# haskoin/haskoin-node

Hardware: AMD Instinct MI355X
Metric: ECDSA verifies/sec (1/8 GPU) + verdict mismatches vs libsecp256k1 (higher is better)
Workload: dtype u32 (256-bit integer limbs)

## Files before the change

haskoin-node_amd/csrc/hkv_api.cpp:

```cpp
#include <hip/hip_runtime.h>

#include <algorithm>
#include <chrono>
#include <cstdio>
#include <cstdlib>
#include <cstring>
#include <memory>
#include <mutex>
#include <new>
#include <random>
#include <string>
#include <vector>

#include "../../include/hkv.h"
#include "hkv_blocktx.h"
#include "hkv_spends.h"
#include "hkv_internal.h"
#include "hkv_launch_plan.h"
#include "hkv_layout.h"
#include "hkv_plan.h"
#include "hkv_tail_plan.h"

namespace {

thread_local std::string g_last_hip;

constexpr size_t CLK_GROUPS = 4096, CLK_WORDS = 16 + 2 * CLK_GROUPS;

int hip_fail(hipError_t e, const char* what) {
  g_last_hip = std::string(what) + ": " + hipGetErrorString(e);
  return HKV_E_HIP;
}
int oom_fail(hipError_t e, const char* what) {
  g_last_hip = std::string(what) + ": " + hipGetErrorString(e);
  return HKV_E_OOM;
}
#define HKV_TRY(expr, what)                       \
  do {                                            \
    hipError_t e_ = (expr);                       \
    if (e_ != hipSuccess) return hip_fail(e_, what); \
  } while (0)
#define HKV_RC(expr)         \
  do {                       \
    const int rc_ = (expr);  \
    if (rc_) return rc_;     \
  } while (0)

struct DeviceMem {
  static hipError_t alloc(void** p, size_t bytes) { return hipMalloc(p, bytes); }
  static void release(void* p) { (void)hipFree(p); }
};
struct PinnedMem {
  static hipError_t alloc(void** p, size_t bytes) { return hipHostMalloc(p, bytes, hipHostMallocPortable); }
  static void release(void* p) { (void)hipHostFree(p); }
};
template <class T, class Mem = DeviceMem>
class DevBuf {
 public:
  DevBuf() = default;
  DevBuf(DevBuf&& o) noexcept : p_(o.p_), n_(o.n_) { o.p_ = nullptr, o.n_ = 0; }
  DevBuf& operator=(DevBuf&& o) noexcept {
    std::swap(p_, o.p_), std::swap(n_, o.n_);
    return *this;
  }
  ~DevBuf() {
    if (p_) Mem::release(p_);
  }
  int reserve(size_t count, const char* what) {
    if (p_ && n_ >= count) return HKV_OK;
    if (p_) Mem::release(p_);
    p_ = nullptr, n_ = 0;
    const hipError_t e = Mem::alloc(reinterpret_cast<void**>(&p_), std::max<size_t>(count * sizeof(T), 16));
    if (e != hipSuccess) {
      p_ = nullptr;
      return oom_fail(e, what);
    }
    n_ = count;
    return HKV_OK;
  }
  T* get() const { return p_; }
  operator T*() const { return p_; }
  size_t size() const { return n_; }

 private:
  T* p_ = nullptr;
  size_t n_ = 0;
};

struct DevCtx {
  int device = -1;
  hkv::Geometry geo;
  hipStream_t stream = nullptr;
  hipStream_t copy_stream = nullptr;
  hipStream_t hash_stream = nullptr;
  hipEvent_t ev_fork = nullptr, ev_join = nullptr;
  DevBuf<uint32_t> gtab, qs;
  DevBuf<uint32_t> im;
  DevBuf<uint32_t> bits;
  DevBuf<uint8_t> recs;
  DevBuf<uint32_t, PinnedMem> hbits;
  DevBuf<uint32_t> pool;
  uint32_t pool_n = 0;
  uint64_t pool_seed = ~0ull;
  DevBuf<uint32_t> txt;
  DevBuf<uint8_t> stage_tx_bytes, stage_scripts, stage_jobs, stage_out, stage_headers, stage_blocks;
  DevBuf<uint32_t> stage_tx_off;
  DevBuf<uint8_t> stage_prev;
  DevBuf<uint32_t> std_first, host_tx_bits;
  DevBuf<hkv_input_job> std_jobs;
  DevBuf<uint8_t> blk_txids;
  DevBuf<uint32_t> blk_table, blk_src;
  uint32_t txid_mask = 0xFFFFFFFFu;
  DevBuf<uint32_t> spd_off, spd_table, spd_spender;
  DevBuf<uint64_t> spd_sums;
  DevBuf<uint8_t> spd_flags;
  uint32_t spend_stages = hkv::SPEND_STAGE_ALL;
  DevBuf<uint32_t> ms_desc, ms_cbits, ms_kbits, host_std_bits;
  DevBuf<uint64_t> ms_off;
  DevBuf<uint8_t> ms_recs;
  uint32_t ms_win_cand = 0, ms_win_keys = 0;
  DevBuf<uint64_t> ms_ctr;
  DevBuf<unsigned int> ms_bar;
  uint32_t tail_epoch = 0;
  bool inject_tail = false;
  uint32_t* call_status = nullptr;
  bool ms_dirty = false;
  DevBuf<uint32_t> rare_ctr;
  bool rare_dirty = false;
  DevBuf<uint32_t> aux;
  bool profile = false;
  std::vector<hipEvent_t> ev;
  DevBuf<unsigned long long> clk;
  int wall_khz = 0;
  hipEvent_t last_use = nullptr;
  uint32_t inject = 0;
};

}

struct hkv_ctx {
  std::vector<DevCtx> devs;
  std::mutex mu;
  std::vector<std::unique_ptr<std::mutex>> tx_mu;
  std::vector<bool> healthy;
  std::vector<uint32_t> failures;
  uint64_t txid_salt = 0;
};
struct hkv_batch {
  hkv_ctx* ctx = nullptr;
  uint8_t* host = nullptr;
  size_t cap = 0;
};

namespace {

size_t round_up(size_t a, size_t b) { return (a + b - 1) / b * b; }

#ifndef HKV_STD_CHUNK
#define HKV_STD_CHUNK (1u << 20)
#endif
constexpr size_t MS_CAND_PER_INPUT = hkv::MS_CAND_PER_INPUT, MS_KEYS_PER_INPUT = hkv::MS_KEYS_PER_INPUT;
constexpr size_t HKV_MAX_STD_INPUTS = 0xFFFFFF00ull;
constexpr size_t MS_BAR_WORDS = 32, MS_FAULT = 16, MS_HOST_STATUS = 17;
#ifndef HKV_HOST_FIRST_DIV
#define HKV_HOST_FIRST_DIV 4
#endif
#ifndef HKV_HOST_MAX_GRIDS
#define HKV_HOST_MAX_GRIDS 8
#endif

int ensure_dev_buffers(DevCtx& d, size_t n_pad) {
  int rc = d.im.reserve(n_pad * hkv::IM_WORDS, "hipMalloc(intermediate)");
  if (!rc) rc = d.bits.reserve(n_pad / 32, "hipMalloc(bits)");
  if (!rc) rc = d.qs.reserve(hkv::plan_records(d.geo, n_pad).qs_quads * 4, "hipMalloc(qtab scratch)");
  return rc;
}

int scratch_acquire(DevCtx& d, hipStream_t st) {
  HKV_TRY(hipStreamWaitEvent(st, d.last_use, 0), "hipStreamWaitEvent(scratch)");
  return HKV_OK;
}
int scratch_release(DevCtx& d, hipStream_t st) {
  HKV_TRY(hipEventRecord(d.last_use, st), "hipEventRecord(scratch)");
  return HKV_OK;
}

int ensure_aux(DevCtx& d, size_t n_pad) { return d.aux.reserve(n_pad * hkv::AUX_WORDS, "hipMalloc(aux)"); }

int profile_mark(DevCtx& d, hipEvent_t (&e)[3], int k, hipStream_t st) {
  if (!d.profile) return HKV_OK;
  if (k == 0)
    for (auto& x : e) HKV_TRY(hipEventCreate(&x), "hipEventCreate");
  HKV_TRY(hipEventRecord(e[k], st), "hipEventRecord");
  if (k == 2) d.ev.insert(d.ev.end(), e, e + 3);
  return HKV_OK;
}

int enqueue_verify(DevCtx& d, const void* d_records, size_t n, uint32_t mode, hipStream_t st,
                   uint32_t* out_bits = nullptr, hipEvent_t late_join = nullptr,
                   const hkv::StdOps* std_pro = nullptr) {
  const hkv::RecPlan plan = hkv::plan_records(d.geo, n);
  HKV_RC(ensure_dev_buffers(d, plan.n_pad));
  hipEvent_t e[3] = {nullptr, nullptr, nullptr};
  HKV_RC(profile_mark(d, e, 0, st));
  if (std_pro != nullptr && plan.shape != hkv::Shape::Mid) return HKV_E_INTERNAL;
  if (plan.aux) HKV_RC(ensure_aux(d, plan.n_pad));
  const hkv::RecOps ops{d.im, (uint32_t)n, d.gtab, d.qs, out_bits ? out_bits : d.bits.get(),
                        (uint32_t)(out_bits ? (n + 31) / 32 : plan.n_pad / 32), d.profile ? d.clk.get() : nullptr,
                        d.aux, d_records, mode};
  if (plan.prologue && std_pro == nullptr) HKV_TRY(hkv::launch_prologue(plan, ops, st), "prologue launch");
  HKV_RC(profile_mark(d, e, 1, st));
  HKV_TRY(hkv::launch_ecmult(plan, ops, std_pro, st), "ecmult launch");
  if (plan.prologue) {
    if (late_join != nullptr) HKV_TRY(hipStreamWaitEvent(st, late_join, 0), "hipStreamWaitEvent(hash join)");
    if (d.rare_dirty) {
      HKV_TRY(hipMemsetAsync(d.rare_ctr, 0, sizeof(uint32_t), st), "hipMemset(rare counter)");
      d.rare_dirty = false;
    }
    const hipError_t e2 = hkv::launch_finish(plan, ops, d.rare_ctr, late_join != nullptr ? d_records : nullptr, st);
    if (e2 != hipSuccess) {
      d.rare_dirty = true;
      return hip_fail(e2, "finish launch");
    }
  }
  return profile_mark(d, e, 2, st);
}

int init_device(DevCtx& d, int device) {
  d.device = device;
  HKV_TRY(hipSetDevice(device), "hipSetDevice");
  hipDeviceProp_t prop;
  HKV_TRY(hipGetDeviceProperties(&prop, device), "hipGetDeviceProperties");
  if (std::strncmp(prop.gcnArchName, "gfx950", 6) != 0) {
    g_last_hip = std::string("device is ") + prop.gcnArchName + ", libhkv is built for gfx950 only";
    return HKV_E_NODEV;
  }
  hkv::Geometry& g = d.geo;
  g.n_cu = (uint32_t)prop.multiProcessorCount;
  HKV_TRY(hipStreamCreateWithFlags(&d.stream, hipStreamNonBlocking), "hipStreamCreate");
  HKV_TRY(hipStreamCreateWithFlags(&d.copy_stream, hipStreamNonBlocking), "hipStreamCreate(copy)");
  HKV_TRY(hipStreamCreateWithFlags(&d.hash_stream, hipStreamNonBlocking), "hipStreamCreate(hash)");
  HKV_TRY(hipEventCreateWithFlags(&d.ev_fork, hipEventDisableTiming), "hipEventCreate(fork)");
  HKV_TRY(hipEventCreateWithFlags(&d.ev_join, hipEventDisableTiming), "hipEventCreate(join)");
  HKV_TRY(hipEventCreateWithFlags(&d.last_use, hipEventDisableTiming), "hipEventCreate(scratch)");
  HKV_TRY(hipEventRecord(d.last_use, d.stream), "hipEventRecord(scratch)");
  HKV_RC(d.ms_ctr.reserve(4, "hipMalloc(multisig counters)"));
  HKV_TRY(hipMemsetAsync(d.ms_ctr, 0, 4 * sizeof(uint64_t), d.stream), "hipMemset(multisig counters)");
  HKV_RC(d.ms_bar.reserve(MS_BAR_WORDS, "hipMalloc(multisig barrier)"));
  HKV_TRY(hipMemsetAsync(d.ms_bar, 0, MS_BAR_WORDS * sizeof(unsigned int), d.stream), "hipMemset(multisig barrier)");
  HKV_RC(d.rare_ctr.reserve(1, "hipMalloc(rare counter)"));
  HKV_TRY(hipMemsetAsync(d.rare_ctr, 0, sizeof(uint32_t), d.stream), "hipMemset(rare counter)");
  HKV_TRY(hipStreamSynchronize(d.stream), "multisig counters sync");
  HKV_TRY(hipDeviceGetAttribute(&d.wall_khz, hipDeviceAttributeWallClockRate, device), "wall clock rate");
  HKV_RC(d.clk.reserve(CLK_WORDS, "hipMalloc(clock probe)"));
  HKV_TRY(hipMemsetAsync(d.clk, 0, CLK_WORDS * sizeof(unsigned long long), d.stream), "hipMemset(clock probe)");
  HKV_RC(d.gtab.reserve(hkv::GTAB_DWORDS, "hipMalloc(gtab)"));
  int per_cu = 0;
  HKV_TRY(hkv::ecmult_max_blocks_per_cu(&per_cu), "occupancy query");
  if (per_cu < 1) per_cu = 1;
  g.grid_max = g.n_cu * (uint32_t)per_cu;
  if (!hkv::host_chunks_ok((size_t)g.grid_max * hkv::WG, HKV_HOST_FIRST_DIV)) {
    g_last_hip = "the host-batch first chunk is not a whole number of verdict words";
    return HKV_E_INTERNAL;
  }
  g.std_chunk = HKV_STD_CHUNK;
  if (const char* e = std::getenv("HKV_STD_CHUNK")) {
    const unsigned long long c = std::strtoull(e, nullptr, 10) / 64 * 64;
    if (c >= 64 && c <= (1ull << 24)) g.std_chunk = (size_t)c;
  }
  g.rec_chunk = HKV_REC_CHUNK;
  if (const char* e = std::getenv("HKV_REC_CHUNK")) {
    const unsigned long long c = std::strtoull(e, nullptr, 10) / hkv::WG * hkv::WG;
    if (c >= (unsigned long long)hkv::WG && c <= HKV_REC_CHUNK) g.rec_chunk = (size_t)c;
  }
  HKV_RC(d.qs.reserve(hkv::plan_records(g, 1).qs_quads * 4, "hipMalloc(qtab scratch)"));
  HKV_TRY(hkv::launch_gtable(d.gtab, d.stream), "gtable launch");
  HKV_TRY(hipStreamSynchronize(d.stream), "gtable sync");
  return HKV_OK;
}

void clear_events(DevCtx& d) {
  for (auto e : d.ev) (void)hipEventDestroy(e);
  d.ev.clear();
}

void free_device(DevCtx& d) {
  if (d.device < 0) return;
  (void)hipSetDevice(d.device);
  if (d.stream) (void)hipStreamSynchronize(d.stream);
  (void)hipDeviceSynchronize();
  clear_events(d);
  for (hipEvent_t e : {d.last_use, d.ev_fork, d.ev_join})
    if (e) (void)hipEventDestroy(e);
  for (hipStream_t s : {d.stream, d.copy_stream, d.hash_stream})
    if (s) (void)hipStreamDestroy(s);
  d = DevCtx();
}

int ensure_pool(DevCtx& d, uint64_t seed, uint32_t pool_n, hipStream_t st) {
  if (d.pool_n == pool_n && d.pool_seed == seed) return HKV_OK;
  d.pool_n = 0;
  HKV_RC(d.pool.reserve((size_t)pool_n * 16, "hipMalloc(pool)"));
  HKV_TRY(hkv::launch_gen_pool(seed, pool_n, d.pool, st), "gen pool launch");
  d.pool_n = pool_n;
  d.pool_seed = seed;
  return HKV_OK;
}

int self_check(DevCtx& d) {
  const size_t n = 256;
  uint8_t* recs = nullptr;
  HKV_TRY(hipMalloc(&recs, n * hkv::REC_SIZE), "hipMalloc(selfcheck)");
  int rc = scratch_acquire(d, d.stream);
  if (!rc) rc = ensure_pool(d, 0x484B5630ull, 16, d.stream);
  if (!rc) {
    hipError_t e = hkv::launch_gen_records(0x484B5630ull, 0, (uint32_t)n, d.pool, d.pool_n, 250, 0, recs, nullptr,
                                           d.stream);
    if (e != hipSuccess) rc = hip_fail(e, "selfcheck gen");
  }
  if (!rc) rc = enqueue_verify(d, recs, n, HKV_MODE_LIBSECP, d.stream);
  uint32_t words[8] = {0};
  if (!rc) {
    hipError_t e = hipMemcpyAsync(words, d.bits, sizeof(words), hipMemcpyDeviceToHost, d.stream);
    if (e == hipSuccess) e = hipStreamSynchronize(d.stream);
    if (e != hipSuccess) rc = hip_fail(e, "selfcheck copy");
  }
  if (!rc) rc = scratch_release(d, d.stream);
  (void)hipFree(recs);
  if (rc) return rc;
  for (uint32_t w : words)
    if (w != 0xFFFFFFFFu) {
      g_last_hip = "self-check: generated valid signatures did not verify";
      return HKV_E_INTERNAL;
    }
  return HKV_OK;
}


bool txs_ok(const hkv_txs* t) {
  return t && (t->n_tx == 0 || (t->bytes && t->offsets)) && (t->scripts || t->scripts_len == 0) &&
         t->n_tx < 0xFFFFFF00u;
}

int reserve_txt(DevCtx& d, const hkv_txs* dt) {
  return d.txt.reserve((size_t)dt->n_tx * hkv::TXT_WORDS, "hipMalloc(txt)");
}
int enqueue_tx_index(DevCtx& d, const hkv_txs* dt, hipStream_t st, uint32_t hashes = hkv::TX_HASHES_ALL) {
  HKV_RC(reserve_txt(d, dt));
  HKV_TRY(hkv::launch_tx_index(dt->bytes, dt->offsets, dt->n_tx, hashes, d.txt, st), "tx index launch");
  return HKV_OK;
}
uint32_t std_tx_hashes(int32_t forkid) { return forkid >= 0 ? hkv::TX_HASHES_ALL : hkv::TX_HASHES_WITNESS; }

hkv::StdOps std_ops(const DevCtx& d, const hkv_txs* dt, const hkv_input_job* jobs, int32_t forkid) {
  return hkv::StdOps{dt->bytes, dt->n_tx, d.txt, dt->scripts, dt->scripts_len, jobs, forkid};
}

int enqueue_std_inputs(DevCtx& d, const hkv_txs* dt, const hkv::StdOps& so, size_t n, void* recs, hipStream_t st) {
  HKV_RC(enqueue_tx_index(d, dt, st, std_tx_hashes(so.forkid)));
  HKV_TRY(hkv::launch_std_inputs(so, (uint32_t)n, static_cast<uint8_t*>(recs), st), "std input launch");
  return HKV_OK;
}

int enqueue_std_verify_split(DevCtx& d, const hkv::StdPlan& plan, const hkv::StdOps& so, size_t n, void* recs,
                             uint32_t* out_bits, const hkv::MsScan* ms, const uint32_t* tx_off, hipStream_t st) {
  HKV_RC(ensure_dev_buffers(d, plan.n_pad));
  HKV_RC(ensure_aux(d, plan.n_pad));
  hipEvent_t e[3] = {nullptr, nullptr, nullptr};
  HKV_RC(profile_mark(d, e, 0, st));
  HKV_RC(profile_mark(d, e, 1, st));
  const hkv::RecOps ops{d.im, (uint32_t)n, d.gtab, d.qs, out_bits, (uint32_t)((n + 31) / 32),
                        d.profile ? d.clk.get() : nullptr, d.aux, recs, HKV_MODE_HASKOIN};
  HKV_TRY(hkv::launch_std_verify_split(plan, so, ops, ms, tx_off, st), "std-input verify launch");
  return profile_mark(d, e, 2, st);
}

hkv::MsTail tail_args(DevCtx& d, const hkv::StdOps& so, const uint32_t* tx_off, size_t n, uint32_t* out_bits,
                      bool hash_txs, const hkv::MsScan& ms, size_t cap_cand, size_t cap_keys) {
  hkv::MsTail t;
  t.win_cand = (uint32_t)cap_cand;
  t.win_keys = (uint32_t)cap_keys;
  t.txs = so.txs;
  t.tx_off = tx_off;
  t.n_tx = so.n_tx;
  t.txt = d.txt;
  t.scripts = so.scripts;
  t.scripts_len = so.scripts_len;
  t.jobs = so.jobs;
  t.n = (uint32_t)n;
  t.forkid = so.forkid;
  t.hash_txs = hash_txs ? std_tx_hashes(so.forkid) : hkv::TX_HASHES_NONE;
  t.desc = ms.desc;
  t.off = ms.off;
  t.total = reinterpret_cast<unsigned long long*>(ms.counters);
  t.total_next = reinterpret_cast<unsigned long long*>(d.ms_ctr + ((d.tail_epoch + 1u) & 1u));
  t.cand = d.ms_recs;
  t.keyrec = d.ms_recs + cap_cand * hkv::REC_SIZE;
  t.cbits = d.ms_cbits;
  t.kbits = d.ms_kbits;
  t.im = d.im;
  t.aux = d.aux;
  t.gtab = d.gtab;
  t.qs = d.qs;
  t.out_bits = out_bits;
  t.bar = d.ms_bar;
  t.epoch = d.tail_epoch;
  t.fault = d.ms_bar + MS_FAULT;
  t.status = d.call_status;
  t.force_fault = d.inject_tail ? 1u : 0u;
  return t;
}
int enqueue_std_chunk(DevCtx& d, const hkv_txs* dt, const hkv_input_job* jobs, size_t n, int32_t forkid, void* recs,
                      uint32_t* out_bits, hipStream_t st) {
  const hkv::StdPlan plan = hkv::plan_std_chunk(d.geo, n);
  const bool small = plan.shape == hkv::Shape::Block || plan.shape == hkv::Shape::Pair;
  const size_t all_cand = n * MS_CAND_PER_INPUT, all_keys = n * MS_KEYS_PER_INPUT;
  const size_t win_c = d.ms_win_cand ? d.ms_win_cand : HKV_MS_WIN_CAND;
  const size_t win_k = d.ms_win_keys ? d.ms_win_keys : HKV_MS_WIN_KEYS;
  const size_t cap_cand = hkv::ms_window_records(all_cand, win_c), cap_keys = hkv::ms_window_records(all_keys, win_k);
  const size_t scratch_pad = std::max<size_t>(plan.n_pad, round_up(hkv::ms_tail_slots(d.geo.n_cu), hkv::WG));
  int rc = d.ms_desc.reserve(n * 2, "hipMalloc(multisig desc)");
  if (!rc) rc = d.ms_off.reserve(n, "hipMalloc(multisig offsets)");
  if (!rc) rc = d.ms_cbits.reserve(hkv::ms_cbits_words(n), "hipMalloc(multisig candidate bits)");
  if (!rc) rc = d.ms_recs.reserve((cap_cand + cap_keys) * hkv::REC_SIZE, "hipMalloc(multisig records)");
  if (!rc) rc = d.ms_kbits.reserve(hkv::ms_kbits_words(n), "hipMalloc(multisig key bits)");
  if (!rc) rc = ensure_dev_buffers(d, scratch_pad);
  if (!rc) rc = ensure_aux(d, scratch_pad);
  if (!rc) rc = reserve_txt(d, dt);
  if (rc) return rc;
  const hkv::StdOps so = std_ops(d, dt, jobs, forkid);
  if (d.ms_dirty) {
    HKV_TRY(hipMemsetAsync(d.ms_ctr, 0, 2 * sizeof(uint64_t), st), "hipMemset(multisig counters)");
    d.ms_dirty = false;
  }
  d.ms_dirty = true;
  const hkv::MsScan ms{d.ms_desc, d.ms_off, d.ms_ctr + (d.tail_epoch & 1u)};
  auto hip_rc = [](hipError_t e, const char* what) { return e == hipSuccess ? (int)HKV_OK : hip_fail(e, what); };
  bool forked = false;
  if (plan.index_first)
    rc = enqueue_tx_index(d, dt, st, plan.index_hashes ? std_tx_hashes(forkid) : (uint32_t)hkv::TX_HASHES_NONE);
  if (rc) return rc;
  if (small) {
    rc = enqueue_std_verify_split(d, plan, so, n, recs, out_bits, plan.scan_in_kernel ? &ms : nullptr,
                                  plan.rows_in_kernel ? dt->offsets : nullptr, st);
  } else if (plan.overlap) {
    HKV_TRY(hipEventRecord(d.ev_fork, st), "hipEventRecord(fork)");
    HKV_TRY(hipStreamWaitEvent(d.hash_stream, d.ev_fork, 0), "hipStreamWaitEvent(fork)");
    forked = true;
    hipError_t e = hkv::launch_tx_hashes_only(dt->bytes, dt->offsets, dt->n_tx, std_tx_hashes(forkid), d.txt,
                                              d.hash_stream);
    if (e == hipSuccess) e = hkv::launch_std_inputs(so, (uint32_t)n, static_cast<uint8_t*>(recs), d.hash_stream);
    if (e == hipSuccess && plan.scan == hkv::ScanOn::HashStream)
      e = hkv::launch_ms_scan(so, (uint32_t)n, ms, d.hash_stream);
    const hipError_t e2 = hipEventRecord(d.ev_join, d.hash_stream);
    rc = e != hipSuccess ? hip_fail(e, "std hash half launch") : hip_rc(e2, "hipEventRecord(join)");
  } else {
    rc = hip_rc(hkv::launch_std_inputs(so, (uint32_t)n, static_cast<uint8_t*>(recs), st), "std input launch");
  }
  if (!rc && plan.scan == hkv::ScanOn::MainStream)
    rc = hip_rc(hkv::launch_ms_scan(so, (uint32_t)n, ms, st), "multisig scan launch");
  if (!rc && !small)
    rc = enqueue_verify(d, recs, n, HKV_MODE_HASKOIN, st, out_bits, plan.overlap ? d.ev_join : nullptr,
                        plan.overlap ? &so : nullptr);
  if (!rc)
    rc = hip_rc(hkv::launch_ms_tail(tail_args(d, so, dt->offsets, n, out_bits, plan.tail_hashes, ms, cap_cand, cap_keys),
                                    d.geo.n_cu, st),
                "multisig tail launch");
  if (!rc) {
    ++d.tail_epoch;
    d.inject_tail = false;
    d.ms_dirty = false;
  }
  if (rc && forked) (void)hipStreamWaitEvent(st, d.ev_join, 0);
  return rc;
}

int enqueue_verify_std_inputs(DevCtx& d, const hkv_txs* dt, const hkv_input_job* jobs, size_t n, int32_t forkid,
                              void* recs, uint32_t* out_bits, hipStream_t st) {
  const size_t chunk = hkv::std_chunk_len(d.geo, n);
  for (size_t lo = 0; lo < n; lo += chunk) {
    const size_t cn = std::min(chunk, n - lo);
    const int rc = enqueue_std_chunk(d, dt, jobs + lo, cn, forkid, static_cast<uint8_t*>(recs) + lo * hkv::REC_SIZE,
                                     out_bits + lo / 32, st);
    if (rc) return rc;
  }
  return HKV_OK;
}

int stage_txs(DevCtx& d, const hkv_txs* h, const void* jobs, size_t job_bytes, hkv_txs* dt, void** djobs) {
  const size_t nbytes = h->n_tx ? h->offsets[h->n_tx] : 0;
  const size_t noff = (size_t)h->n_tx + 1;
  HKV_RC(d.stage_tx_bytes.reserve(nbytes, "hipMalloc(tx bytes)"));
  HKV_RC(d.stage_tx_off.reserve(noff, "hipMalloc(tx offsets)"));
  HKV_RC(d.stage_scripts.reserve(h->scripts_len, "hipMalloc(scripts)"));
  HKV_RC(d.stage_jobs.reserve(job_bytes, "hipMalloc(jobs)"));
  if (nbytes) HKV_TRY(hipMemcpyAsync(d.stage_tx_bytes, h->bytes, nbytes, hipMemcpyHostToDevice, d.stream), "H2D txs");
  if (h->n_tx)
    HKV_TRY(hipMemcpyAsync(d.stage_tx_off, h->offsets, noff * 4, hipMemcpyHostToDevice, d.stream), "H2D offsets");
  if (h->scripts_len)
    HKV_TRY(hipMemcpyAsync(d.stage_scripts, h->scripts, h->scripts_len, hipMemcpyHostToDevice, d.stream),
            "H2D scripts");
  if (job_bytes) HKV_TRY(hipMemcpyAsync(d.stage_jobs, jobs, job_bytes, hipMemcpyHostToDevice, d.stream), "H2D jobs");
  dt->bytes = d.stage_tx_bytes;
  dt->offsets = d.stage_tx_off;
  dt->n_tx = h->n_tx;
  dt->scripts = d.stage_scripts;
  dt->scripts_len = h->scripts_len;
  *djobs = d.stage_jobs.get();
  return HKV_OK;
}

bool dev_ok(const hkv_ctx* ctx, int dev) { return ctx && dev >= 0 && dev < (int)ctx->devs.size(); }

enum class Lock { None, Mu, Tx };
class Call {
 public:
  DevCtx& d;
  const hipStream_t st;
  int rc = HKV_OK;
  Call(hkv_ctx* ctx, int dev, void* hip_stream, Lock kind)
      : d(ctx->devs[(size_t)dev]), st(static_cast<hipStream_t>(hip_stream)) {
    if (kind == Lock::Tx) tx_ = std::unique_lock<std::mutex>(*ctx->tx_mu[(size_t)dev]);
    if (kind != Lock::None) mu_ = std::unique_lock<std::mutex>(ctx->mu);
    const hipError_t e = hipSetDevice(d.device);
    if (e != hipSuccess) rc = hip_fail(e, "hipSetDevice");
  }
  Call(hkv_ctx* ctx, int dev, Lock kind) : Call(ctx, dev, ctx->devs[(size_t)dev].stream, kind) {}
  int acquire(uint32_t* status = nullptr) {
    if (!rc) rc = scratch_acquire(d, st);
    if (!rc) held_ = true, d.call_status = status;
    return rc;
  }
  int done(int r = HKV_OK) {
    if (!held_) return r;
    held_ = false;
    d.call_status = nullptr;
    if (!r) return scratch_release(d, st);
    (void)hipEventRecord(d.last_use, st);
    return r;
  }
  ~Call() { (void)done(HKV_E_HIP); }

 private:
  std::unique_lock<std::mutex> tx_, mu_;
  bool held_ = false;
};

}

extern "C" {

uint32_t hkv_version(void) { return (1u << 16) | 4u; }

const char* hkv_strerror(int err) {
  switch (err) {
    case HKV_OK: return "ok";
    case HKV_E_ARG: return "invalid argument";
    case HKV_E_NODEV: return "no usable gfx950 device";
    case HKV_E_OOM: return "out of memory";
    case HKV_E_HIP: return "HIP runtime error";
    case HKV_E_INTERNAL: return "internal self-check failed";
    default: return "unknown error";
  }
}
const char* hkv_last_hip_error(void) { return g_last_hip.c_str(); }

int hkv_device_count(void) {
  int n = 0;
  if (hipGetDeviceCount(&n) != hipSuccess) return 0;
  return n;
}

int hkv_open_devices(const int* device_ids, int n_ids, uint32_t flags, hkv_ctx** out) {
  if (!out || n_ids <= 0 || !device_ids) return HKV_E_ARG;
  *out = nullptr;
  hkv_ctx* ctx = new (std::nothrow) hkv_ctx();
  if (!ctx) return HKV_E_OOM;
  ctx->devs.resize(n_ids);
  ctx->healthy.assign(n_ids, true);
  ctx->failures.assign(n_ids, 0);
  try {
    std::random_device rd;
    ctx->txid_salt = ((uint64_t)rd() << 32) ^ (uint64_t)rd();
  } catch (...) {
    const uint64_t now = (uint64_t)std::chrono::steady_clock::now().time_since_epoch().count();
    ctx->txid_salt = (now * 0x9E3779B97F4A7C15ull) ^ (uint64_t)reinterpret_cast<uintptr_t>(ctx);
  }
  for (int k = 0; k < n_ids; ++k) ctx->tx_mu.emplace_back(new (std::nothrow) std::mutex());
  for (auto& m : ctx->tx_mu)
    if (!m) {
      delete ctx;
      return HKV_E_OOM;
    }
  for (int k = 0; k < n_ids; ++k) {
    int rc = init_device(ctx->devs[k], device_ids[k]);
    if (!rc && !(flags & HKV_OPEN_NO_SELFCHECK)) rc = self_check(ctx->devs[k]);
    if (rc) {
      for (auto& d : ctx->devs) free_device(d);
      delete ctx;
      return rc;
    }
  }
  *out = ctx;
  return HKV_OK;
}

int hkv_open(int n_gpus, uint32_t flags, hkv_ctx** out) {
  if (!out) return HKV_E_ARG;
  int avail = hkv_device_count();
  if (avail <= 0) return HKV_E_NODEV;
  if (n_gpus <= 0 || n_gpus > avail) n_gpus = avail;
  std::vector<int> ids(n_gpus);
  for (int k = 0; k < n_gpus; ++k) ids[k] = k;
  return hkv_open_devices(ids.data(), n_gpus, flags, out);
}

void hkv_close(hkv_ctx* ctx) {
  if (!ctx) return;
  for (auto& d : ctx->devs) free_device(d);
  delete ctx;
}

int hkv_ctx_num_devices(const hkv_ctx* ctx) { return ctx ? (int)ctx->devs.size() : 0; }

int hkv_device_healthy(hkv_ctx* ctx, int dev) {
  if (!dev_ok(ctx, dev)) return HKV_E_ARG;
  std::lock_guard<std::mutex> lock(ctx->mu);
  return ctx->healthy[(size_t)dev] ? 1 : 0;
}

int hkv_device_reset_health(hkv_ctx* ctx, int dev) {
  if (!dev_ok(ctx, dev)) return HKV_E_ARG;
  std::lock_guard<std::mutex> lock(ctx->mu);
  ctx->healthy[(size_t)dev] = true;
  return HKV_OK;
}

int hkv_device_failures(hkv_ctx* ctx, int dev) {
  if (!dev_ok(ctx, dev)) return HKV_E_ARG;
  std::lock_guard<std::mutex> lock(ctx->mu);
  return (int)ctx->failures[(size_t)dev];
}

int hkv_debug_fail_device(hkv_ctx* ctx, int dev, uint32_t when) {
  if (!dev_ok(ctx, dev) || when > HKV_FAIL_TAIL) return HKV_E_ARG;
  std::lock_guard<std::mutex> lock(ctx->mu);
  if (when == HKV_FAIL_TAIL) ctx->devs[(size_t)dev].inject_tail = true;
  else ctx->devs[(size_t)dev].inject = when;
  return HKV_OK;
}

int hkv_debug_ms_window(hkv_ctx* ctx, int dev, uint32_t cand_records, uint32_t key_records) {
  if (!dev_ok(ctx, dev) || cand_records > HKV_MS_WIN_CAND ||
      key_records > HKV_MS_WIN_KEYS)
    return HKV_E_ARG;
  std::lock_guard<std::mutex> lock(ctx->mu);
  DevCtx& d = ctx->devs[(size_t)dev];
  d.ms_win_cand = (uint32_t)round_up(cand_records, 64);
  d.ms_win_keys = (uint32_t)round_up(key_records, 64);
  return HKV_OK;
}

int hkv_debug_q_scratch(hkv_ctx* ctx, int dev, size_t* bytes, size_t* chunk) {
  if (!dev_ok(ctx, dev) || !bytes || !chunk) return HKV_E_ARG;
  std::lock_guard<std::mutex> lock(ctx->mu);
  *bytes = ctx->devs[(size_t)dev].qs.size() * sizeof(uint32_t);
  *chunk = ctx->devs[(size_t)dev].geo.rec_chunk;
  return HKV_OK;
}

int hkv_debug_launch_shape(hkv_ctx* ctx, int dev, uint32_t kind, size_t n, uint32_t out[4]) {
  if (!dev_ok(ctx, dev) || kind > 1 || n == 0 || n > HKV_MAX_STD_INPUTS || !out) return HKV_E_ARG;
  std::lock_guard<std::mutex> lock(ctx->mu);
  const hkv::Geometry& g = ctx->devs[(size_t)dev].geo;
  if (kind == 0) {
    const hkv::RecPlan p = hkv::plan_records(g, n);
    out[0] = (uint32_t)p.shape, out[1] = 0, out[2] = p.chunk(0).cn, out[3] = p.n_chunks;
  } else {
    const size_t chunk = hkv::std_chunk_len(g, n), first = std::min(chunk, n);
    const hkv::StdPlan p = hkv::plan_std_chunk(g, first);
    out[0] = (uint32_t)p.shape;
    out[1] = (p.scan_in_kernel ? 1u : 0u) | (p.rows_in_kernel ? 2u : 0u) | (p.overlap ? 4u : 0u);
    out[2] = (uint32_t)first, out[3] = (uint32_t)((n + chunk - 1) / chunk);
  }
  return HKV_OK;
}

int hkv_debug_ms_scratch(hkv_ctx* ctx, int dev, size_t* bytes) {
  if (!dev_ok(ctx, dev) || !bytes) return HKV_E_ARG;
  std::lock_guard<std::mutex> lock(ctx->mu);
  *bytes = ctx->devs[(size_t)dev].ms_recs.size();
  return HKV_OK;
}

int hkv_debug_ms_tail_counts(hkv_ctx* ctx, int dev, uint64_t out[3]) {
  if (!dev_ok(ctx, dev) || !out) return HKV_E_ARG;
  Call c(ctx, dev, Lock::Mu);
  DevCtx& d = c.d;
  out[0] = out[1] = out[2] = 0;
  if (d.tail_epoch == 0) return HKV_OK;
  const uint32_t par = (d.tail_epoch - 1u) & 1u;
  uint64_t total = 0;
  unsigned int slot[2] = {0, 0};
  HKV_RC(c.acquire());
  HKV_TRY(hipMemcpyAsync(&total, d.ms_ctr + par, sizeof(total), hipMemcpyDeviceToHost, c.st), "D2H scan total");
  HKV_TRY(hipMemcpyAsync(slot, d.ms_bar + par * 8u, sizeof(slot), hipMemcpyDeviceToHost, c.st), "D2H tail slot");
  HKV_TRY(hipStreamSynchronize(c.st), "tail counts sync");
  out[0] = total;
  out[1] = slot[0];
  out[2] = slot[1];
  return c.done();
}

int hkv_device_fault(hkv_ctx* ctx, int dev, uint32_t* fault) {
  if (!dev_ok(ctx, dev) || !fault) return HKV_E_ARG;
  Call c(ctx, dev, Lock::Mu);
  DevCtx& d = c.d;
  unsigned int w = 0;
  HKV_RC(c.acquire());
  HKV_TRY(hipMemcpyAsync(&w, d.ms_bar + MS_FAULT, sizeof(w), hipMemcpyDeviceToHost, c.st), "D2H fault latch");
  HKV_TRY(hipMemsetAsync(d.ms_bar + MS_FAULT, 0, sizeof(unsigned int), c.st), "hipMemset(fault latch)");
  HKV_TRY(hipStreamSynchronize(c.st), "fault latch sync");
  *fault = w ? HKV_STATUS_TAIL_FAULT : 0u;
  return c.done();
}

int hkv_batch_alloc(hkv_ctx* ctx, size_t max_n, hkv_batch** out) {
  if (!ctx || !out || max_n == 0) return HKV_E_ARG;
  hkv_batch* b = new (std::nothrow) hkv_batch();
  if (!b) return HKV_E_OOM;
  if (hipHostMalloc(reinterpret_cast<void**>(&b->host), max_n * hkv::REC_SIZE, hipHostMallocPortable) !=
      hipSuccess) {
    delete b;
    return HKV_E_OOM;
  }
  std::memset(b->host, 0, max_n * hkv::REC_SIZE);
  b->ctx = ctx;
  b->cap = max_n;
  *out = b;
  return HKV_OK;
}
void hkv_batch_free(hkv_batch* b) {
  if (!b) return;
  if (b->host) (void)hipHostFree(b->host);
  delete b;
}
uint8_t* hkv_batch_records(hkv_batch* b) { return b ? b->host : nullptr; }
size_t hkv_batch_capacity(const hkv_batch* b) { return b ? b->cap : 0; }

static void quiesce(DevCtx& d) {
  (void)hipSetDevice(d.device);
  (void)hipStreamSynchronize(d.copy_stream);
  (void)hipStreamSynchronize(d.stream);
}

static int enqueue_host_shard(DevCtx& d, const uint8_t* host, const hkv::Shard& s, uint32_t mode,
                              std::vector<hipEvent_t>& evs) {
  if (d.inject == HKV_FAIL_ENQUEUE) {
    d.inject = 0;
    g_last_hip = "injected enqueue failure (hkv_debug_fail_device)";
    return HKV_E_HIP;
  }
  if (d.inject == HKV_FAIL_ALLOC) {
    d.inject = 0;
    return oom_fail(hipErrorOutOfMemory, "injected allocation failure (hkv_debug_fail_device)");
  }
  const size_t len = s.hi - s.lo;
  hipError_t e0 = hipSetDevice(d.device);
  int rc = e0 == hipSuccess ? scratch_acquire(d, d.stream) : hip_fail(e0, "hipSetDevice");
  if (!rc) rc = scratch_acquire(d, d.copy_stream);
  if (!rc) rc = d.recs.reserve(len * hkv::REC_SIZE, "hipMalloc(records)");
  if (!rc) rc = d.hbits.reserve((len + 31) / 32, "hipHostMalloc(bits)");
  if (rc) return rc;
  const size_t grid_lanes = (size_t)d.geo.grid_max * hkv::WG;
  const uint8_t* src = host + s.lo * hkv::REC_SIZE;
  const std::vector<size_t> chunks = hkv::host_chunks(len, grid_lanes, HKV_HOST_FIRST_DIV, HKV_HOST_MAX_GRIDS);
  rc = ensure_dev_buffers(d, round_up(*std::max_element(chunks.begin(), chunks.end()), hkv::WG));
  size_t off = 0;
  for (auto it = chunks.begin(); it != chunks.end() && !rc; off += *it++) {
    const size_t cl = *it;
    hipEvent_t ev = nullptr;
    hipError_t e = hipEventCreateWithFlags(&ev, hipEventDisableTiming);
    if (e != hipSuccess) {
      rc = oom_fail(e, "hipEventCreate");
      break;
    }
    evs.push_back(ev);
    if (e == hipSuccess)
      e = hipMemcpyAsync(d.recs + off * hkv::REC_SIZE, src + off * hkv::REC_SIZE, cl * hkv::REC_SIZE,
                         hipMemcpyHostToDevice, d.copy_stream);
    if (e == hipSuccess) e = hipEventRecord(ev, d.copy_stream);
    if (e == hipSuccess) e = hipStreamWaitEvent(d.stream, ev, 0);
    if (e != hipSuccess) {
      rc = hip_fail(e, "H2D records");
      break;
    }
    rc = enqueue_verify(d, d.recs + off * hkv::REC_SIZE, cl, mode, d.stream);
    if (!rc) {
      e = hipMemcpyAsync(d.hbits + off / 32, d.bits, (cl + 31) / 32 * 4, hipMemcpyDeviceToHost, d.stream);
      if (e != hipSuccess) rc = hip_fail(e, "D2H bits");
    }
  }
  if (!rc) rc = scratch_release(d, d.stream);
  if (!rc) rc = scratch_acquire(d, d.copy_stream);
  return rc;
}

static int join_host_shard(DevCtx& d, const hkv::Shard& s, uint32_t* out, size_t out_words) {
  HKV_TRY(hipSetDevice(d.device), "hipSetDevice");
  HKV_TRY(hipStreamSynchronize(d.stream), "verify sync");
  if (d.inject == HKV_FAIL_JOIN) {
    d.inject = 0;
    g_last_hip = "injected join failure (hkv_debug_fail_device)";
    return HKV_E_HIP;
  }
  if (!hkv::merge_shard_words(out, out_words, d.hbits, s)) {
    g_last_hip = "shard does not fit the verdict bitmap";
    return HKV_E_INTERNAL;
  }
  return HKV_OK;
}

static int verify_from_host(hkv_ctx* ctx, const uint8_t* host, size_t n, uint32_t mode, uint32_t* out) {
  if (!ctx || !host || !out || mode > HKV_MODE_HASKOIN) return HKV_E_ARG;
  if (n == 0) return HKV_OK;
  std::lock_guard<std::mutex> lock(ctx->mu);
  std::vector<std::vector<hipEvent_t>> evs(ctx->devs.size());
  struct EventGuard {
    std::vector<std::vector<hipEvent_t>>& e;
    ~EventGuard() {
      for (auto& v : e)
        for (auto ev : v) (void)hipEventDestroy(ev);
    }
  } guard{evs};
  const size_t out_words = (n + 31) / 32;
  return hkv::run_with_failover(
      n, ctx->healthy,
      [&](const hkv::Shard& s) { return enqueue_host_shard(ctx->devs[(size_t)s.dev], host, s, mode, evs[(size_t)s.dev]); },
      [&](const hkv::Shard& s) { return join_host_shard(ctx->devs[(size_t)s.dev], s, out, out_words); },
      [&](int dev, int) {
        quiesce(ctx->devs[(size_t)dev]);
        ++ctx->failures[(size_t)dev];
      });
}

int hkv_verify(hkv_ctx* ctx, hkv_batch* b, size_t n, uint32_t mode, uint32_t* verdict_bits) {
  if (!b || n > b->cap) return HKV_E_ARG;
  return verify_from_host(ctx, b->host, n, mode, verdict_bits);
}

int hkv_verify_host(hkv_ctx* ctx, const uint8_t* records, size_t n, uint32_t mode, uint32_t* verdict_bits) {
  return verify_from_host(ctx, records, n, mode, verdict_bits);
}

int hkv_verify_device(hkv_ctx* ctx, int dev, const void* d_records, size_t n, uint32_t mode, uint32_t* d_bits,
                      void* hip_stream) {
  if (!dev_ok(ctx, dev) || !d_records || !d_bits || mode > HKV_MODE_HASKOIN) return HKV_E_ARG;
  if (n == 0) return HKV_OK;
  if (n > 0xFFFFFF00ull) return HKV_E_ARG;
  Call c(ctx, dev, hip_stream, Lock::Mu);
  int rc = c.acquire();
  if (!rc) rc = enqueue_verify(c.d, d_records, n, mode, c.st, d_bits);
  return c.done(rc);
}

int hkv_gen_batch_device(hkv_ctx* ctx, int dev, uint64_t seed, uint64_t index0, size_t n, uint32_t pool_size,
                         uint32_t uncompressed_permille, uint32_t invalid_permille, void* d_records,
                         uint32_t* d_labels, void* hip_stream) {
  if (!dev_ok(ctx, dev) || !d_records || pool_size == 0 || uncompressed_permille > 1000 ||
      invalid_permille > 1000 || n > 0xFFFFFF00ull || index0 > ~0ull - n)
    return HKV_E_ARG;
  if (n == 0) return HKV_OK;
  Call c(ctx, dev, hip_stream, Lock::Mu);
  DevCtx& d = c.d;
  HKV_RC(c.acquire());
  HKV_RC(ensure_pool(d, seed ^ 0x706F6F6Cull, pool_size, c.st));
  HKV_TRY(hkv::launch_gen_records(seed, index0, (uint32_t)n, d.pool, d.pool_n, uncompressed_permille,
                                  invalid_permille, d_records, d_labels, c.st),
          "gen records launch");
  return c.done();
}

int hkv_gen_records_device(hkv_ctx* ctx, int dev, uint64_t seed, size_t n, uint32_t pool_size,
                           uint32_t uncompressed_permille, void* d_records, void* hip_stream) {
  return hkv_gen_batch_device(ctx, dev, seed, 0, n, pool_size, uncompressed_permille, 0, d_records, nullptr,
                              hip_stream);
}

int hkv_debug_op(hkv_ctx* ctx, int dev, uint32_t op, size_t n, const uint32_t* d_a, const uint32_t* d_b,
                 uint32_t* d_out, void* hip_stream) {
  if (!dev_ok(ctx, dev) || !d_a || !d_b || !d_out) return HKV_E_ARG;
  if (n == 0) return HKV_OK;
  Call c(ctx, dev, hip_stream, Lock::None);
  HKV_RC(c.rc);
  HKV_TRY(hkv::launch_debug(op, (uint32_t)n, d_a, d_b, d_out, c.st), "debug launch");
  return HKV_OK;
}

int hkv_profile_enable(hkv_ctx* ctx, int on) {
  if (!ctx) return HKV_E_ARG;
  std::lock_guard<std::mutex> lock(ctx->mu);
  for (auto& d : ctx->devs) {
    (void)hipSetDevice(d.device);
    (void)hipDeviceSynchronize();
    clear_events(d);
    d.profile = on != 0;
  }
  return HKV_OK;
}

int hkv_profile_read(hkv_ctx* ctx, int dev, double* prologue_ms, double* ecmult_ms, uint64_t* launches) {
  if (!dev_ok(ctx, dev) || !prologue_ms || !ecmult_ms || !launches)
    return HKV_E_ARG;
  Call call(ctx, dev, Lock::Mu);
  HKV_RC(call.rc);
  DevCtx& d = call.d;
  double p = 0, m = 0;
  for (size_t k = 0; k + 2 < d.ev.size(); k += 3) {
    HKV_TRY(hipEventSynchronize(d.ev[k + 2]), "hipEventSynchronize");
    float a = 0, b = 0;
    HKV_TRY(hipEventElapsedTime(&a, d.ev[k], d.ev[k + 1]), "hipEventElapsedTime");
    HKV_TRY(hipEventElapsedTime(&b, d.ev[k + 1], d.ev[k + 2]), "hipEventElapsedTime");
    p += a;
    m += b;
  }
  *prologue_ms = p;
  *ecmult_ms = m;
  *launches = d.ev.size() / 3;
  clear_events(d);
  return HKV_OK;
}

int hkv_profile_clock(hkv_ctx* ctx, int dev, double* sclk_mhz) {
  if (!dev_ok(ctx, dev) || !sclk_mhz) return HKV_E_ARG;
  Call call(ctx, dev, Lock::Mu);
  HKV_RC(call.rc);
  DevCtx& d = call.d;
  HKV_TRY(hipDeviceSynchronize(), "hipDeviceSynchronize");
  unsigned long long c[4] = {0, 0, 0, 0};
  HKV_TRY(hipMemcpy(c, d.clk, sizeof(c), hipMemcpyDeviceToHost), "D2H clock probe");
  *sclk_mhz = 0;
  if (c[3] > c[1] && d.wall_khz > 0) *sclk_mhz = (double)(c[2] - c[0]) / ((double)(c[3] - c[1]) / (d.wall_khz * 1e-3));
  return HKV_OK;
}

int hkv_profile_phases(hkv_ctx* ctx, int dev, uint64_t* stamps, size_t n, double* tick_ns) {
  if (!dev_ok(ctx, dev) || !stamps || !tick_ns || n > 12) return HKV_E_ARG;
  Call call(ctx, dev, Lock::Mu);
  HKV_RC(call.rc);
  DevCtx& d = call.d;
  HKV_TRY(hipDeviceSynchronize(), "hipDeviceSynchronize");
  if (n) HKV_TRY(hipMemcpy(stamps, d.clk + 4, n * sizeof(uint64_t), hipMemcpyDeviceToHost), "D2H phase stamps");
  *tick_ns = d.wall_khz > 0 ? 1e6 / d.wall_khz : 0.0;
  return HKV_OK;
}

int hkv_profile_group_stamps(hkv_ctx* ctx, int dev, uint64_t* stamps, size_t n_groups, double* tick_ns) {
  if (!dev_ok(ctx, dev) || !stamps || !tick_ns || n_groups > CLK_GROUPS)
    return HKV_E_ARG;
  Call call(ctx, dev, Lock::Mu);
  HKV_RC(call.rc);
  DevCtx& d = call.d;
  HKV_TRY(hipDeviceSynchronize(), "hipDeviceSynchronize");
  if (n_groups)
    HKV_TRY(hipMemcpy(stamps, d.clk + 16, 2 * n_groups * sizeof(uint64_t), hipMemcpyDeviceToHost), "D2H group stamps");
  *tick_ns = d.wall_khz > 0 ? 1e6 / d.wall_khz : 0.0;
  return HKV_OK;
}

int hkv_sighash_device(hkv_ctx* ctx, int dev, const hkv_txs* d_txs, const hkv_sighash_job* d_jobs, size_t n,
                       int32_t forkid, uint8_t* d_out, size_t out_stride, uint8_t* d_status, void* hip_stream) {
  if (!dev_ok(ctx, dev) || !txs_ok(d_txs) || out_stride < 32 || out_stride % 4 ||
      out_stride > 0xFFFFFFFFu || n > 0xFFFFFF00ull)
    return HKV_E_ARG;
  if (n == 0) return HKV_OK;
  if (!d_jobs || !d_out) return HKV_E_ARG;
  Call c(ctx, dev, hip_stream, Lock::Tx);
  HKV_RC(c.acquire());
  HKV_RC(enqueue_tx_index(c.d, d_txs, c.st));
  HKV_TRY(hkv::launch_sighash(d_txs->bytes, d_txs->n_tx, c.d.txt, d_txs->scripts, d_txs->scripts_len, d_jobs,
                              (uint32_t)n, forkid, d_out, (uint32_t)out_stride, d_status, c.st),
          "sighash launch");
  return c.done();
}

int hkv_sighash(hkv_ctx* ctx, const hkv_txs* txs, const hkv_sighash_job* jobs, size_t n, int32_t forkid,
                uint8_t* out32, uint8_t* status) {
// ... 725 lines not shown
```

haskoin-node_amd/csrc/hkv_internal.h:

```cpp
#pragma once
#include <hip/hip_runtime.h>
#include <stdint.h>

#include "../../include/hkv.h"
#include "hkv_launch_plan.h"

#define HKV_MODE_LIBSECP 0u
#define HKV_MODE_HASKOIN 1u

enum {
  HKV_DBG_FE_MUL = 1,
  HKV_DBG_FE_SQR = 2,
  HKV_DBG_FE_ADD = 3,
  HKV_DBG_FE_SUB = 4,
  HKV_DBG_FE_INV = 5,
  HKV_DBG_FE_SQRT = 6,
  HKV_DBG_SC_MUL = 7,
  HKV_DBG_SC_INV = 8,
  HKV_DBG_GLV = 9,
  HKV_DBG_ECMULT_G = 10,
  HKV_DBG_MUL512 = 11,
  HKV_DBG_SQR512 = 12,
  HKV_DBG_FE_CNEG = 13,
  HKV_DBG_FE_CNEG_MASK = 14,
  HKV_DBG_FE_NEG = 15,
  HKV_DBG_FE_HALF = 16,
  HKV_DBG_FE_SHL = 17,
  HKV_DBG_FE_SHL_VAR = 18,
  HKV_DBG_FE_MUL_SMALL = 19,
  HKV_DBG_FE_MUL_SMALL2 = 20,
  HKV_DBG_FE_LIN2 = 21,
  HKV_DBG_FE_MUL_ADD = 22,
  HKV_DBG_FE_MUL2 = 23,
  HKV_DBG_FE_SQR2 = 24,
  HKV_DBG_FE_SQRMUL = 25,
  HKV_DBG_FE_MUL_REF = 26,
  HKV_DBG_FE_SQR_REF = 27,
  HKV_DBG_FE_NORMALIZE = 28,
  HKV_DBG_FE_IS_ZERO = 29,
  HKV_DBG_FE_EQUAL = 30,
  HKV_DBG_U256_LT_P = 31,
  HKV_DBG_SC_ADD = 32,
  HKV_DBG_SC_SUB = 33,
  HKV_DBG_SC_NEG = 34,
  HKV_DBG_SC_SQR = 35,
  HKV_DBG_SC_IS_HIGH = 36,
  HKV_DBG_INV_MOD_P = 37,
  HKV_DBG_FE_MUL_SUM = 38,
  HKV_DBG_FE_SQRMUL_SUM = 39,
  HKV_DBG_FE_NEG_COMPL = 40,
  HKV_DBG_FE_MUL_SUM_RA = 41,
  HKV_DBG_FE_MUL_SUM_RD = 42,
  HKV_DBG_FE_SQRMUL_SUM_RA = 43,
  HKV_DBG_FE_SQRMUL_SUM_RD = 44,
  HKV_DBG_FE_MUL_SUM_RB = 45,
  HKV_DBG_GEJ_DOUBLE = 64,
  HKV_DBG_GEJ_DOUBLE_ILP = 65,
  HKV_DBG_GEJ_ACCUMULATE = 66,
  HKV_DBG_GEJ_ACCUMULATE_ILP = 67,
  HKV_DBG_GEJ_ADD_VAR = 68,
  HKV_DBG_GEJ_ADD_AFFINE_COMPLETE = 69,
  HKV_DBG_X_MATCHES_R = 70,
  HKV_DBG_ECMULT = 71,
};

namespace hkv {
struct RecOps {
  uint32_t* im;
  uint32_t n;
  const uint32_t* gtab;
  uint32_t* qs;
  uint32_t* bits;
  uint32_t n_words;
  unsigned long long* clk;
  uint32_t* aux;
  const void* recs;
  uint32_t mode;
};
struct StdOps;
hipError_t launch_prologue(const RecPlan& p, const RecOps& r, hipStream_t st);
hipError_t launch_ecmult(const RecPlan& p, const RecOps& r, const StdOps* std_pro, hipStream_t st);
hipError_t launch_gtable(uint32_t* gtab, hipStream_t st);
struct MsScan {
  uint32_t* desc;
  uint64_t* off;
  uint64_t* counters;
};
struct MsTail {
  const uint8_t* txs;
  const uint32_t* tx_off;
  uint32_t n_tx;
  uint32_t* txt;
  const uint8_t* scripts;
  uint32_t scripts_len;
  const hkv_input_job* jobs;
  uint32_t n;
  int32_t forkid;
  uint32_t hash_txs;
  const uint32_t* desc;
  const uint64_t* off;
  unsigned long long* total;
  unsigned long long* total_next;
  uint8_t* cand;
  uint8_t* keyrec;
  uint32_t win_cand, win_keys;
  uint32_t* cbits;
  uint32_t* kbits;
  uint32_t* im;
  uint32_t* aux;
  const uint32_t* gtab;
  uint32_t* qs;
  uint32_t* out_bits;
  unsigned int* bar;
  uint32_t epoch;
  unsigned int* fault;
  uint32_t* status;
  uint32_t force_fault;
};
hipError_t launch_ms_tail(const MsTail& a, uint32_t grid, hipStream_t st);
uint32_t ms_tail_slots(uint32_t n_cu);
struct StdOps {
  const uint8_t* txs;
  uint32_t n_tx;
  const uint32_t* txt;
  const uint8_t* scripts;
  uint32_t scripts_len;
  const hkv_input_job* jobs;
  int32_t forkid;
};
hipError_t launch_std_verify_split(const StdPlan& p, const StdOps& o, const RecOps& r, const MsScan* ms,
                                   const uint32_t* tx_off, hipStream_t st);
hipError_t launch_finish(const RecPlan& p, const RecOps& r, uint32_t* rare_ctr, const void* late_recs,
                         hipStream_t st);
hipError_t launch_gen_pool(uint64_t seed, uint32_t npool, uint32_t* pool, hipStream_t st);
hipError_t launch_gen_records(uint64_t seed, uint64_t index0, uint32_t n, const uint32_t* pool, uint32_t npool,
                              uint32_t unc_permille, uint32_t invalid_permille, void* recs, uint32_t* labels,
                              hipStream_t st);
hipError_t launch_debug(uint32_t op, uint32_t n, const uint32_t* a, const uint32_t* b, uint32_t* out,
                        hipStream_t st);
hipError_t ecmult_max_blocks_per_cu(int* out);
hipError_t launch_gen_keys(uint64_t seed, uint32_t n, uint8_t* priv, uint8_t* pub, uint8_t* h160, hipStream_t st);
hipError_t launch_gen_sign(uint64_t seed, uint32_t n, const uint8_t* priv, const uint32_t* key_idx,
                           const uint8_t* msg, uint32_t msg_stride, uint8_t* sig, hipStream_t st);
hipError_t launch_tx_index(const uint8_t* txs, const uint32_t* tx_off, uint32_t n_tx, uint32_t hashes,
                           uint32_t* txt, hipStream_t st);
hipError_t launch_sighash(const uint8_t* txs, uint32_t n_tx, const uint32_t* txt, const uint8_t* scripts,
                          uint32_t scripts_len, const hkv_sighash_job* jobs, uint32_t n, int32_t forkid, uint8_t* out,
                          uint32_t stride, uint8_t* status, hipStream_t st);
hipError_t launch_std_inputs(const StdOps& o, uint32_t n, uint8_t* recs, hipStream_t st);
hipError_t launch_txids(const uint8_t* txs, const uint32_t* tx_off, uint32_t n_tx, uint8_t* txids, uint8_t* status,
                        hipStream_t st);
hipError_t launch_tx_hashes_only(const uint8_t* txs, const uint32_t* tx_off, uint32_t n_tx, uint32_t hashes,
                                 uint32_t* txt, hipStream_t st);
hipError_t launch_ms_scan(const StdOps& o, uint32_t n, const MsScan& ms, hipStream_t st);
struct StdPrevouts {
  const uint32_t* offsets;
  const uint8_t* outpoints;
  const uint32_t* scripts;
  const uint64_t* values;
};
hipError_t launch_stdtx_counts(const uint8_t* txs, const uint32_t* tx_off, uint32_t n_tx, uint32_t n_inputs,
                               uint32_t* input_first, uint32_t* status, hipStream_t st);
hipError_t launch_stdtx_jobs(const uint8_t* txs, const uint32_t* tx_off, uint32_t n_tx, const uint32_t* input_first,
                             const StdPrevouts& p, uint32_t n_inputs, hkv_input_job* jobs, hipStream_t st);
hipError_t launch_tx_verdicts(const uint32_t* input_first, uint32_t n_tx, const uint32_t* input_bits,
                              const uint32_t* status, uint32_t* tx_bits, hipStream_t st);
struct TxidTable;
hipError_t launch_txid_table(const TxidTable& tb, hipStream_t st);
hipError_t launch_txid_lookup(const TxidTable& tb, const uint8_t* queries, uint32_t n_q, uint32_t* found,
                              hipStream_t st);
hipError_t launch_blocktx_jobs(const uint8_t* txs, const uint32_t* tx_off, uint32_t n_tx, const uint32_t* input_first,
                               const StdPrevouts& p, uint32_t pool_base, uint32_t pool_len, const TxidTable& tb,
                               uint32_t n_inputs, hkv_input_job* jobs, uint32_t* input_src, hipStream_t st);
struct SpendStage {
  const uint8_t* txs;
  const uint32_t* tx_off;
  uint32_t n_tx;
  const uint32_t* input_first;
  const hkv_input_job* jobs;
  const uint32_t* input_src;
  uint32_t n_inputs;
  uint64_t max_money;
  uint32_t* input_off;
  uint32_t* slots;
  uint32_t n_slots;
  uint64_t salt;
  uint32_t mask;
  uint32_t* spender;
  uint64_t* tx_sums;
  uint8_t* tx_flags;
  uint32_t* status;
};
constexpr uint32_t SPEND_STAGE_WALK = 1u, SPEND_STAGE_TABLE = 2u, SPEND_STAGE_SPENDER = 4u, SPEND_STAGE_FOLD = 8u,
                   SPEND_STAGE_ALL = 15u;
hipError_t launch_block_spends(const SpendStage& s, uint32_t stages, hipStream_t st);
hipError_t launch_headers(const uint8_t* hdrs, uint32_t n, const uint8_t* pow_limit, const uint8_t* prev0,
                          uint8_t* hashes, uint8_t* status, hipStream_t st);
hipError_t launch_merkle(const uint8_t* leaves, const uint32_t* offsets, uint32_t n_blocks, uint8_t* scratch,
                         uint8_t* roots, uint8_t* mutated, uint32_t n_cu, hipStream_t st);
hipError_t launch_block_verdicts(const uint8_t* txids, const uint32_t* offsets, uint32_t n_blocks, const uint8_t* hdrs,
                                 const uint8_t* roots, const uint8_t* mutated, uint8_t* status, hipStream_t st);
}
```

haskoin-node_amd/csrc/hkv_kernels.hip:

```cpp
#include "hkv_group.h"
#include "hkv_hash.h"
#include "hkv_layout.h"
#include "hkv_internal.h"
#include "hkv_sighash_dev.h"
#include "hkv_tail_plan.h"

namespace hkv {

HKV_DEV uint32_t rec_word_at(const uint32_t* w, int off) {
  const int k = off >> 2, s = off & 3;
  if (s == 0) return w[k];
  return __builtin_amdgcn_alignbyte(w[k + 1], w[k], s);
}
HKV_DEV void rec_be256(uint32_t out[8], const uint32_t* w, int off) {
#pragma unroll
  for (int j = 0; j < 8; ++j) out[7 - j] = __builtin_bswap32(rec_word_at(w, off + 4 * j));
}

__constant__ static const uint32_t PMN[8] = {0x2FC9BAEEu, 0x402DA172u, 0x50B75FC4u, 0x45512319u, 1u, 0, 0, 0};

template <class W>
struct SoA {
  W* p;
  uint32_t n_pad;
// ... 1225 lines not shown
    fe Pb;
    fe_sel(Pb, b.x, b.y, odd);
    pair_add_var(P, Zs, inf, Pb, b.z, binf, odd);
  }
}
HKV_DEV void add_segment(fe& Pacc, fe& Zacc, bool& ainf, const fe& P, const fe& Zs, bool sinf, const fe& zs,
                         const fe& y0, uint32_t odd) {
  fe zt, zb;
  fe_mul(zt, Zs, zs);
  fe_mul(zb, zt, y0);
  pair_add_var(Pacc, Zacc, ainf, P, zb, sinf, odd);
}
HKV_DEV void pair_from_xch(const uint32_t* xk, uint32_t c, uint32_t odd, fe& P, fe& Z, bool& inf) {
  gej b;
  xch_read(xk, BLK_SIGS, c, b, inf);
  fe_sel(P, b.x, b.y, odd);
  Z = b.z;
}
HKV_DEV void pair_to_xch(uint32_t* xk, uint32_t c, uint32_t odd, const fe& P, const fe& Z, bool inf) {
  pair_publish(xk, BLK_SIGS, c, P, Z, inf, odd);
}

template <bool STD>
__global__ void __launch_bounds__(BLK_TPB, 1) hkv_block_kernel(uint32_t* __restrict__ im, uint32_t n, uint32_t n_pad,
                                                               const uint32_t* __restrict__ gtab,
                                                               uint32_t* __restrict__ qs,
                                                               uint32_t* __restrict__ bits, uint32_t n_words,
                                                               uint32_t* __restrict__ aux,
                                                               uint32_t* __restrict__ recs, uint32_t mode,
                                                               unsigned long long* __restrict__ clk, StdArgs sa) {
  __shared__ QLane qlds[3];
  __shared__ HLane hlds[3];
  __shared__ uint32_t xch[5][25 * BLK_SIGS];
  __shared__ uint32_t qpub[3][8][BLK_SIGS];
  __shared__ uint32_t shabuf[STD ? 16 * WG : 1];
  __shared__ uint32_t bflag[BF_COUNT];
  __shared__ typename TxCacheOf<STD>::type tcache;
  const int wv = __builtin_amdgcn_readfirstlane(threadIdx.x >> 6);
  const uint32_t ln = threadIdx.x & 63;
  const uint32_t odd = (ln & 1u) ? 0xFFFFFFFFu : 0u;
  const bool stamp = clk != nullptr && blockIdx.x == 0 && ln == 0;
  auto mark = [&](int slot) {
    if (stamp) clk[4 + slot] = wall_clock64();
  };
  const SoAView iv = {im, n_pad}, av = {aux, n_pad};
  if (threadIdx.x < BF_COUNT) bflag[threadIdx.x] = 0;
  if (clk != nullptr && threadIdx.x == 0 && blockIdx.x < 4096) clk[16 + 2 * blockIdx.x] = wall_clock64();
  __syncthreads();
  if (wv == 0) mark(STAMP_START);

  uint32_t seq = 0;
  for (uint32_t base = blockIdx.x * BLK_SIGS; base < n_pad; base += gridDim.x * BLK_SIGS) {
    ++seq;
    if constexpr (STD) {
      txc_fill(tcache, sa, base, n);
      __syncthreads();
    }
    if (wv == 2) {
      const uint32_t i = base + ln;
      const bool on = ln < BLK_SIGS;
      uint32_t flags;
      bool use;
      sc sinv, m;
      StdIn x = {};
      sig_wave_parse<STD>(i, on, n, mode, iv, recs, sa, x, m, sinv, use, flags,
                          blk_view<STD>(tcache, ln & (BLK_SIGS - 1)));
      blk_post(&bflag[BF_SIG], seq);
      mark(STAMP_SIG);
      if constexpr (STD) blk_wait(&bflag[BF_H], seq);
      sig_wave_gsum<STD, (STD ? -1 : BLK_SIGS)>(i, on, n, iv, gtab, av, recs, sa, shabuf, x, m, sinv, use, flags);
      blk_post(&bflag[BF_A], seq);
      mark(STAMP_GSUM);
      if constexpr (STD) {
        if (sa.ms_desc != nullptr)
          ms_scan_lane(sa.txs, sa.n_tx, sa.txt, sa.scripts, sa.scripts_len, sa.jobs, i, on && i < n, sa.forkid,
                       sa.ms_desc, sa.ms_off, sa.ms_ctr, shabuf);
      }
      __syncthreads();
      continue;
    }
#if HKV_CHAIN_PRIO
    __builtin_amdgcn_s_setprio(HKV_CHAIN_PRIO);
#endif
    int k1 = BLK_K1;
#if HKV_BLK_K1_HASHED
    if constexpr (STD) {
      const uint32_t* row_;
      if (__any(blk_needs_tx_hashes(sa, base + (ln & (BLK_SIGS - 1)), n, row_))) k1 = HKV_BLK_K1_HASHED;
    }
#endif
    const int half = (int)(ln >> 5);
    const uint32_t c = (ln & 31u) >> 1;
    const uint32_t i = base + c;
    const int slot = wv == 3 ? 2 : wv;
    fe Zg, zb, P, Z;
    if (wv == 0) {
      ge q;
      key_point<STD>(i, n, recs, sa, q, blk_view<STD>(tcache, c));
      fe_sel(P, q.x, q.y, odd);
      fe_set_u32(zb, 1);
      pair_table(P, half, odd, qlds[0], hlds[0], ln, Zg);
      mark(STAMP_TABLE0);
      if constexpr (STD) {
        blk_tx_hashes(sa, tcache, base, n, recs, shabuf);
        blk_post(&bflag[BF_H], seq);
      }
    } else if (wv == 1) {
      const uint32_t cq = ln >> 2, qd = ln & 3u;
      const uint32_t m0 = qd == 0 ? ~0u : 0u, m1 = qd == 1 ? ~0u : 0u, m2 = qd == 2 ? ~0u : 0u;
      ge q;
      key_point<STD>(base + cq, n, recs, sa, q, blk_view<STD>(tcache, cq));
      fe V;
      fe_set_u32(V, 1);
      fe_sel(V, V, q.y, m1);
      fe_sel(V, V, q.x, m0);
#pragma unroll 1
      for (int d = 0; d < QW * k1; ++d) quad_double(V, m0, m1, m2);
      if (qd < 3) {
#pragma unroll
        for (int k = 0; k < 8; ++k) qpub[qd][k][cq] = V.v[k];
      }
      blk_post(&bflag[BF_Q], seq);
#pragma unroll 1
      for (int d = QW * k1; d < QW * BLK_K2; ++d) quad_double(V, m0, m1, m2);
      const int src_p = (int)(4 * c + (odd ? 1u : 0u)), src_z = (int)(4 * c + 2);
#pragma unroll
      for (int k = 0; k < 8; ++k) {
        P.v[k] = (uint32_t)__shfl((int)V.v[k], src_p);
        zb.v[k] = (uint32_t)__shfl((int)V.v[k], src_z);
      }
      pair_table(P, half, odd, qlds[1], hlds[1], ln, Zg);
      mark(STAMP_TABLE1);
    } else {
      if (ln < BLK_SIGS) sqrt_lane<STD>(base + ln, n, recs, sa, av, blk_view<STD>(tcache, ln));
      blk_post(&bflag[BF_Y], seq);
      mark(STAMP_SQRT);
      blk_wait(&bflag[BF_Q], seq);
#pragma unroll
      for (int k = 0; k < 8; ++k) {
        P.v[k] = qpub[odd ? 1 : 0][k][c];
        zb.v[k] = qpub[2][k][c];
      }
      pair_table(P, half, odd, qlds[2], hlds[2], ln, Zg);
    }
    blk_wait(&bflag[BF_SIG], seq);
    if (wv == 0) mark(STAMP_P);
    const uint32_t flags = iv.get(IM_FLAGS, i);
    const bool valid = (i < n) && (flags & FLAG_VALID);
    const bool negh = (flags & (half ? FLAG_NEG2 : FLAG_NEG1)) != 0;
    const int w_hi = wv == 0 ? k1 - 1 : (wv == 1 ? NWIN - 1 : BLK_K2 - 1);
    const int w_lo = wv == 0 ? 0 : (wv == 1 ? BLK_K2 : k1);
    fe zs;
    fe_mul(zs, Zg, zb);
    bool inf;
    pair_chain(P, Z, inf, qlds[slot], iv, i, valid, negh, half, odd, ln, w_hi, w_lo);
    mark(wv == 0 ? STAMP_CHAIN0 : (wv == 1 ? STAMP_CHAIN1 : STAMP_CHAIN_MID));
    fe Zs;
    halves_sum(xch[slot], c, half, odd, P, Z, inf, Zs);
    if (wv == 0) {
      blk_wait(&bflag[BF_A], seq);
      blk_wait(&bflag[BF_Y], seq);
      mark(STAMP_A);
      if (half == 0) {
        gej A;
        fe y0, PA;
        uint32_t r[8], af;
        bool is_sq;
        join_inputs(iv, av, i, A, y0, r, af, is_sq);
        bool tinf = (af & AUXF_AINF) != 0;
        fe_sel(PA, A.x, A.y, odd);
        add_segment(PA, A.z, tinf, P, Zs, inf, zs, y0, odd);
        pair_to_xch(xch[3], c, odd, PA, A.z, tinf);
      }
      blk_post(&bflag[BF_T], seq);
    } else if (wv == 3) {
      fe zbs;
      if (half == 0) {
        fe y0, zt;
#pragma unroll
        for (int k = 0; k < 8; ++k) y0.v[k] = av.get(AUX_Y0, k, i);
        fe_mul(zt, Zs, zs);
        fe_mul(zbs, zt, y0);
      }
      blk_wait(&bflag[BF_T], seq);
      if (half == 0) {
        fe PT, ZT;
        bool tinf;
        pair_from_xch(xch[3], c, odd, PT, ZT, tinf);
        pair_add_var(PT, ZT, tinf, P, zbs, inf, odd);
        pair_to_xch(xch[4], c, odd, PT, ZT, tinf);
      }
      blk_post(&bflag[BF_U], seq);
    } else {
      blk_wait(&bflag[BF_A], seq);
      blk_wait(&bflag[BF_Y], seq);
      bool accept = false;
      gej A;
      fe y0, zb;
      uint32_t r[8], af;
      bool is_sq;
      if (half == 0) {
        join_inputs(iv, av, i, A, y0, r, af, is_sq);
        fe zt;
        fe_mul(zt, Zs, zs);
        fe_mul(zb, zt, y0);
      }
      blk_wait(&bflag[BF_U], seq);
      if (half == 0) {
        fe PR, ZR;
        bool rinf;
        pair_from_xch(xch[4], c, odd, PR, ZR, rinf);
        pair_add_var(PR, ZR, rinf, P, zb, inf, odd);
        accept = valid && is_sq && !rinf && x_matches_r(PR, ZR, r) && (!STD || (af & AUXF_STDOK));
      }
      const uint64_t ball = __ballot(accept && !odd);
      mark(STAMP_JOIN);
      if (ln == 0) {
        const uint32_t wi = base / 32;
        if (wi < n_words) reinterpret_cast<uint16_t*>(bits)[base / BLK_SIGS] = (uint16_t)(even_bits(ball) & 0xFFFFu);
      }
    }
    __syncthreads();
  }
  if (clk != nullptr && threadIdx.x == 0 && blockIdx.x < 4096) clk[16 + 2 * blockIdx.x + 1] = wall_clock64();
}

HKV_DEV void gej_add_var(gej& acc, bool& inf, const gej& b, bool binf) {
  gej a2;
  fe z2, z3;
  fe_sqr(z2, b.z);
  fe_mul(z3, z2, b.z);
  fe_mul(a2.x, acc.x, z2);
  fe_mul(a2.y, acc.y, z3);
  fe_mul(a2.z, acc.z, b.z);
  bool ainf = inf;
  gej_accumulate(a2, ainf, acc.z, b.x, b.y, !binf && !inf);
  const bool take_b = inf && !binf, keep_a = binf;
  gej_cmov(a2, b, take_b);
  gej_cmov(a2, acc, keep_a);
  acc = a2;
  inf = keep_a ? inf : (take_b ? false : ainf);
}

HKV_DEV bool x_matches_r(const fe& Xin, const fe& Z, const uint32_t r[8]) {
  fe zz, X = Xin, t, rf;
  fe_sqr(zz, Z);
  fe_normalize(X);
#pragma unroll
  for (int k = 0; k < 8; ++k) rf.v[k] = r[k];
  fe_mul(t, rf, zz);
  fe_normalize(t);
  bool eq = fe_eq_norm(t, X);
  const bool small_r = u256_lt(r, PMN);
  uint32_t c = 0;
#pragma unroll
  for (int k = 0; k < 8; ++k) rf.v[k] = addc(r[k], SC_N[k], c);
  fe_mul(t, rf, zz);
  fe_normalize(t);
  return eq || (small_r && fe_eq_norm(t, X));
}

#ifndef HKV_FINISH_WAVES
#define HKV_FINISH_WAVES 3
#endif
HKV_DEV void gtab_entry(const uint32_t* __restrict__ gtab, int t, uint32_t gd, fe& tx, fe& ty) {
  const uint32_t mag = gd & GD_MAG;
  const uint4* e = reinterpret_cast<const uint4*>(gtab) + ((size_t)t * GTAB_ENTRIES + (mag ? mag - 1 : 0)) * 4;
  const uint4 a0 = e[0], a1 = e[1], a2 = e[2], a3 = e[3];
  tx.v[0] = a0.x; tx.v[1] = a0.y; tx.v[2] = a0.z; tx.v[3] = a0.w;
  tx.v[4] = a1.x; tx.v[5] = a1.y; tx.v[6] = a1.z; tx.v[7] = a1.w;
  ty.v[0] = a2.x; ty.v[1] = a2.y; ty.v[2] = a2.z; ty.v[3] = a2.w;
  ty.v[4] = a3.x; ty.v[5] = a3.y; ty.v[6] = a3.z; ty.v[7] = a3.w;
}

template <bool ILP>
HKV_DEV void gsum_lane(SoACView iv, const uint32_t* __restrict__ gtab, uint32_t i, bool valid, gej& A, bool& ainf) {
  uint32_t gd = valid ? iv.get(IM_GDIG, i) : 0u;
  fe tx, ty;
  gtab_entry(gtab, 0, gd, tx, ty);
  fe_cneg(A.y, ty, (gd & GD_NEG) != 0);
  A.x = tx;
  fe_set_u32(A.z, 1);
  ainf = (gd & GD_MAG) == 0;
  gd = valid ? iv.get(IM_GDIG, 1, i) : 0u;
  gtab_entry(gtab, 1, gd, tx, ty);
#pragma unroll 1
  for (int t = 1; t < 2 * GWIN; ++t) {
    const uint32_t gdn = (t + 1 < 2 * GWIN && valid) ? iv.get(IM_GDIG, t + 1, i) : 0u;
    fe nx, nyy;
    if (t + 1 < 2 * GWIN) gtab_entry(gtab, t + 1, gdn, nx, nyy);
    const bool take = (gd & GD_MAG) != 0;
    fe_cneg(ty, ty, (gd & GD_NEG) != 0);
    const bool was_inf = ainf;
    ec_accumulate<ILP>(A, ainf, A.z, tx, ty, take);
    if (__any(take && was_inf)) gej_accumulate_from_inf(A, ainf, tx, ty, take && was_inf);
    gd = gdn;
    tx = nx;
    ty = nyy;
  }
}

template <bool ILP, bool LATE>
HKV_DEV void finish_lane(uint32_t* __restrict__ im, uint32_t n, uint32_t n_pad, const uint32_t* __restrict__ gtab,
                         uint32_t* __restrict__ rare_ctr, uint32_t i, uint32_t flags,
                         const uint32_t* __restrict__ recs) {
  if constexpr (LATE) {
    if (i < n) flags = late_u1_lane(recs, i, SoAView{im, n_pad}, flags);
  }
  const bool valid = (i < n) && (flags & FLAG_VALID);

  gej A;
  bool ainf;
  gsum_lane<ILP>(SoAView{im, n_pad}, gtab, i, valid, A, ainf);

  asm volatile("" ::: "memory");
  gej B;
  fe w;
  uint32_t r[8];
#pragma unroll
  for (int k = 0; k < 8; ++k) {
    B.x.v[k] = SoAView{im, n_pad}.get(IM_BX, k, i);
    B.y.v[k] = SoAView{im, n_pad}.get(IM_BY, k, i);
    B.z.v[k] = SoAView{im, n_pad}.get(IM_BZ, k, i);
    w.v[k] = SoAView{im, n_pad}.get(IM_W, k, i);
    r[k] = SoAView{im, n_pad}.get(IM_R, k, i);
  }
  const bool binf = (flags & FLAG_BINF) != 0;

  fe ZA2, ZA3, Z2, Z3, U1, H, T, S1, HH, t, num, numn, den;
  fe rf, nf;
#pragma unroll
  for (int k = 0; k < 8; ++k) {
    rf.v[k] = r[k];
    nf.v[k] = SC_N[k];
  }
  bool hz;
  if constexpr (ILP) {
    fe a, b, t2, t3;
    fe_sqr2(ZA2, A.z, Z2, B.z);
    fe_mul2(ZA3, ZA2, A.z, Z3, Z2, B.z);
    fe_mul2(Z2, Z2, w, U1, B.x, ZA2);
    fe_mul2(t, A.x, Z2, T, Z2, ZA2);
    fe_sub(H, U1, t);
    hz = fe_is_zero(H);
    fe_add(S1, t, U1);
    fe_sqrmul(HH, H, t, rf, T);
    fe_add(S1, S1, t);
    fe_mul2(a, B.y, ZA3, b, A.y, Z3);
    fe_sqrmul(num, a, den, a, b);
    fe_sqrmul(t, w, den, den, w);
    fe_add(den, den, den);
    fe_sqrmul(b, b, t, t, w);
    fe_mul2(t, t, b, t2, HH, S1);
    fe_add(num, num, t);
    fe_sub(num, num, t2);
    fe_mul(t3, T, nf);
    fe_mul(t3, HH, t3);
    fe_sub(numn, num, t3);
  } else {
    fe_sqr(ZA2, A.z);
    fe_mul(ZA3, ZA2, A.z);
    fe_sqr(Z2, B.z);
    fe_mul(Z3, Z2, B.z);
    fe_mul(Z2, Z2, w);
    fe_mul(U1, B.x, ZA2);
    fe_mul(t, A.x, Z2);
    fe_sub(H, U1, t);
    hz = fe_is_zero(H);
    fe_add(S1, t, U1);
    fe_mul(T, Z2, ZA2);
    fe_mul(t, rf, T);
    fe_add(S1, S1, t);
    fe_sqr(HH, H);
    fe a, b;
    fe_mul(a, B.y, ZA3);
    fe_mul(b, A.y, Z3);
    fe_mul(den, a, b);
    fe_mul(den, den, w);
    fe_add(den, den, den);
    fe_sqr(num, a);
    fe_sqr(t, w);
    fe_mul(t, t, w);
    fe_sqr(b, b);
    fe_mul(t, t, b);
    fe_add(num, num, t);
    fe_mul(t, HH, S1);
    fe_sub(num, num, t);
    fe_mul(t, T, nf);
    fe_mul(t, HH, t);
    fe_sub(numn, num, t);
  }

  uint32_t fo = flags;
  if (!valid) fo |= FLAG_DECIDED;
  const bool rare = valid && (ainf || binf || hz);
  const uint64_t rmask = __ballot(rare);
  if (rmask) {
    uint32_t base = 0;
    const int lead = __builtin_ctzll(rmask);
    if ((int)(threadIdx.x & 63) == lead) base = atomicAdd(rare_ctr, (uint32_t)__popcll(rmask));
    base = __shfl(base, lead);
    const uint32_t rank = __builtin_amdgcn_mbcnt_hi((uint32_t)(rmask >> 32),
                                                    __builtin_amdgcn_mbcnt_lo((uint32_t)rmask, 0u));
    if (rare && base + rank < n_pad) SoAView{im, n_pad}.put(IM_RARE_LIST, (size_t)base + rank, i);
  }
  if (rare) {
    fo |= FLAG_RARE | (ainf ? FLAG_AINF : 0u);
#pragma unroll
    for (int k = 0; k < 8; ++k) {
      SoAView{im, n_pad}.put(IM_AX, k, i, A.x.v[k]);
      SoAView{im, n_pad}.put(IM_AY, k, i, A.y.v[k]);
      SoAView{im, n_pad}.put(IM_AZ, k, i, A.z.v[k]);
    }
  } else {
#pragma unroll
    for (int k = 0; k < 8; ++k) {
      SoAView{im, n_pad}.put(IM_NUM, k, i, num.v[k]);
      SoAView{im, n_pad}.put(IM_NUMN, k, i, numn.v[k]);
      SoAView{im, n_pad}.put(IM_DEN, k, i, den.v[k]);
    }
  }
  SoAView{im, n_pad}.put(IM_FLAGS, i, fo);
}

template <bool ILP, bool LATE>
__global__ void __launch_bounds__(WG, ILP ? 2 : HKV_FINISH_WAVES) hkv_finish_kernel(uint32_t* __restrict__ im, uint32_t n,
                                                                                 uint32_t n_pad,
                                                                                 const uint32_t* __restrict__ gtab,
                                                                                 uint32_t* __restrict__ rare_ctr,
                                                                                 const uint32_t* __restrict__ recs) {
  const uint32_t i = blockIdx.x * WG + threadIdx.x;
  if (i >= n_pad) return;
  finish_lane<ILP, LATE>(im, n, n_pad, gtab, rare_ctr, i, SoAView{im, n_pad}.get(IM_FLAGS, i), recs);
}

__global__ void __launch_bounds__(WG) hkv_rare_kernel(uint32_t* __restrict__ im, uint32_t n_pad,
                                                      const uint32_t* __restrict__ rare_ctr) {
  const uint32_t k = blockIdx.x * WG + threadIdx.x;
  if (k >= min(*rare_ctr, n_pad)) return;
  const SoAView iv = {im, n_pad};
  const uint32_t i = iv.get(IM_RARE_LIST, k);
  const uint32_t flags = iv.get(IM_FLAGS, i);
  const bool rare = true;
  gej A, B;
  fe w;
  uint32_t r[8];
#pragma unroll
  for (int k = 0; k < 8; ++k) {
    A.x.v[k] = iv.get(IM_AX, k, i);
    A.y.v[k] = iv.get(IM_AY, k, i);
    A.z.v[k] = iv.get(IM_AZ, k, i);
    B.x.v[k] = iv.get(IM_BX, k, i);
    B.y.v[k] = iv.get(IM_BY, k, i);
    B.z.v[k] = iv.get(IM_BZ, k, i);
    w.v[k] = iv.get(IM_W, k, i);
    r[k] = iv.get(IM_R, k, i);
  }
  fe y0, y2, ny;
  fe_sqrt_cand(y0, w);
  fe_sqr(y2, y0);
  const bool is_sq = fe_equal(y2, w);
  fe_normalize(y0);
  fe_neg(ny, y0);
  fe_normalize(ny);
  if ((y0.v[0] & 1u) != ((flags & FLAG_YODD) ? 1u : 0u)) y0 = ny;
  gej b = B;
  fe_mul(b.z, B.z, y0);
  bool rinf = (flags & FLAG_AINF) != 0;
  gej_add_var(A, rinf, b, (flags & FLAG_BINF) != 0);
  const bool acc_ok = is_sq && !rinf && x_matches_r(A.x, A.z, r);
  if (rare) iv.put(IM_FLAGS, i, flags | FLAG_DECIDED | (acc_ok ? FLAG_ACCEPT : 0u));
}

__global__ void __launch_bounds__(WG) hkv_yverdict_kernel(uint32_t* __restrict__ im, uint32_t n_pad, uint32_t stride,
                                                          uint32_t* __restrict__ bits, uint32_t n_words,
                                                          uint32_t* __restrict__ rare_ctr) {
  const uint32_t t = blockIdx.x * WG + threadIdx.x;
  if (t == 0) *rare_ctr = 0;
  fe c;
  fe_set_u32(c, 1);
  int kn = 0;
  {
    fe d;
    SoACView::ld8(im, n_pad, IM_DEN.off, t, d.v);
    uint32_t fl = im[(size_t)IM_FLAGS.off * n_pad + t];
#pragma unroll 1
    for (int k = 0; k < VERDICT_BATCH; ++k) {
      const uint32_t i = t + (uint32_t)k * stride;
      if (i >= n_pad) break;
      kn = k + 1;
      const uint32_t inext = i + stride;
      fe dn;
      uint32_t fn = 0;
      if (k + 1 < VERDICT_BATCH && inext < n_pad) {
        SoACView::ld8(im, n_pad, IM_DEN.off, inext, dn.v);
        fn = im[(size_t)IM_FLAGS.off * n_pad + inext];
      }
      if (fl & FLAG_DECIDED) fe_set_u32(d, 1);
      fe_mul(c, c, d);
      SoAView::st8(im, n_pad, IM_C.off, i, c.v);
      d = dn;
      fl = fn;
    }
  }
  fe inv;
  fe_normalize(c);
  sgcd::inv_mod_p(inv.v, c.v);
  struct Ops {
    uint32_t f;
    fe prev, d, num, w;
    uint32_t r[8];
  };
  auto load_ops = [&](Ops& o, int k) {
    const uint32_t i = t + (uint32_t)k * stride;
    o.f = im[(size_t)IM_FLAGS.off * n_pad + i];
    if (k > 0) SoACView::ld8(im, n_pad, IM_C.off, i - stride, o.prev.v);
    SoACView::ld8(im, n_pad, IM_DEN.off, i, o.d.v);
    SoACView::ld8(im, n_pad, IM_NUM.off, i, o.num.v);
    SoACView::ld8(im, n_pad, IM_W.off, i, o.w.v);
    SoACView::ld8(im, n_pad, IM_R.off, i, o.r);
  };
  Ops cur;
  if (kn > 0) load_ops(cur, kn - 1);
#pragma unroll 1
  for (int k = kn - 1; k >= 0; --k) {
    const uint32_t i = t + (uint32_t)k * stride;
    Ops nxt;
    if (k > 0) load_ops(nxt, k - 1);
    const uint32_t f = cur.f;
    const bool decided = (f & FLAG_DECIDED) != 0;
    fe dinv;
    if (k == 0) fe_set_u32(cur.prev, 1);
    fe_mul(dinv, inv, cur.prev);
    if (decided) fe_set_u32(cur.d, 1);
    fe_mul(inv, inv, cur.d);
    bool accept = (f & FLAG_ACCEPT) != 0;
    if (!decided) {
      fe yc, y2;
      const uint32_t want = (f & FLAG_YODD) ? 1u : 0u;
      fe_mul(yc, cur.num, dinv);
      fe_normalize(yc);
      fe_sqr(y2, yc);
      bool ok = fe_equal(y2, cur.w) && (yc.v[0] & 1u) == want;
      const bool small_r = u256_lt(cur.r, PMN);
      if (__any(!ok && small_r)) {
        fe numn;
        SoACView::ld8(im, n_pad, IM_NUMN.off, i, numn.v);
        fe_mul(yc, numn, dinv);
        fe_normalize(yc);
        fe_sqr(y2, yc);
        ok = ok || (small_r && fe_equal(y2, cur.w) && (yc.v[0] & 1u) == want);
      }
      accept = ok;
    }
    cur = nxt;
    const uint64_t ball = __ballot(accept);
    if ((threadIdx.x & 63) == 0) {
      const uint32_t wi = i / 32;
      if (wi < n_words) bits[wi] = (uint32_t)ball;
      if (wi + 1 < n_words) bits[wi + 1] = (uint32_t)(ball >> 32);
    }
  }
}
HKV_DEV void gej_add_affine_complete(gej& acc, bool& inf, const ge& b, bool take) {
  const bool was_inf = inf;
  gej_accumulate(acc, inf, acc.z, b.x, b.y, take);
  gej_accumulate_from_inf(acc, inf, b.x, b.y, take && was_inf);
}
HKV_DEV bool ecmult_simple(ge& out, const sc& a, const sc& b, const ge& p) {
  ge g;
  ge_set_g(g);
  gej acc;
  bool inf = true;
  fe_set_zero(acc.x);
  fe_set_zero(acc.y);
  fe_set_zero(acc.z);
  for (int bit = 255; bit >= 0; --bit) {
    if (__any(!inf)) {
      gej d;
      gej_double(d, acc);
      gej_cmov(acc, d, !inf);
    }
    const bool ba = (a.v[bit >> 5] >> (bit & 31)) & 1u;
    const bool bb = (b.v[bit >> 5] >> (bit & 31)) & 1u;
    gej_add_affine_complete(acc, inf, g, ba);
    gej_add_affine_complete(acc, inf, p, bb);
  }
  if (inf) return false;
  fe zi, zi2, zi3;
  fe_inv(zi, acc.z);
  fe_sqr(zi2, zi);
  fe_mul(zi3, zi2, zi);
  fe_mul(out.x, acc.x, zi2);
  fe_mul(out.y, acc.y, zi3);
  fe_normalize(out.x);
  fe_normalize(out.y);
  return true;
}

__global__ void __launch_bounds__(WG) hkv_gtable_kernel(uint32_t* __restrict__ gtab) {
  const int tid = blockIdx.x * WG + threadIdx.x;
  if (tid >= GTAB_TABLES * GTAB_ENTRIES) return;
  const int t = tid / GTAB_ENTRIES, j = tid % GTAB_ENTRIES + 1;
  sc a, zero;
#pragma unroll
  for (int k = 0; k < 8; ++k) { a.v[k] = 0; zero.v[k] = 0; }
  {
    const int off = GTAB_W * (t / 2) + 128 * (t % 2);
    sc p2, jj;
#pragma unroll
    for (int k = 0; k < 8; ++k) { p2.v[k] = 0; jj.v[k] = 0; }
    p2.v[off >> 5] = 1u << (off & 31);
    jj.v[0] = (uint32_t)j;
    sc_mul(a, jj, p2);
  }
  ge g, out;
  ge_set_g(g);
  ecmult_simple(out, a, zero, g);
#pragma unroll
  for (int k = 0; k < 8; ++k) {
    gtab[tid * 16 + k] = out.x.v[k];
    gtab[tid * 16 + 8 + k] = out.y.v[k];
  }
}

HKV_DEV uint64_t splitmix64(uint64_t& s) {
  uint64_t z = (s += 0x9E3779B97F4A7C15ull);
  z = (z ^ (z >> 30)) * 0xBF58476D1CE4E5B9ull;
  z = (z ^ (z >> 27)) * 0x94D049BB133111EBull;
  return z ^ (z >> 31);
}
HKV_DEV void rand_scalar(sc& r, uint64_t& st) {
#pragma unroll
  for (int k = 0; k < 4; ++k) {
    const uint64_t v = splitmix64(st);
    r.v[2 * k] = (uint32_t)v;
    r.v[2 * k + 1] = (uint32_t)(v >> 32);
  }
  sc_cond_sub_n(r.v);
  if (u256_is_zero(r.v)) r.v[0] = 1;
}

__global__ void __launch_bounds__(WG) hkv_gen_pool_kernel(uint64_t seed, uint32_t npool,
                                                          uint32_t* __restrict__ pool) {
  const uint32_t j = blockIdx.x * WG + threadIdx.x;
  if (j >= npool) return;
  uint64_t st = seed * 0x2545F4914F6CDD1Dull + j * 0x9E3779B97F4A7C15ull + 0x5851F42D4C957F2Dull;
  sc d, zero;
  rand_scalar(d, st);
#pragma unroll
  for (int k = 0; k < 8; ++k) zero.v[k] = 0;
  ge g, q;
  ge_set_g(g);
  ecmult_simple(q, d, zero, g);
#pragma unroll
  for (int k = 0; k < 8; ++k) {
    pool[(size_t)j * 16 + k] = q.x.v[k];
    pool[(size_t)j * 16 + 8 + k] = q.y.v[k];
  }
}

HKV_DEV void put_be256(uint8_t* dst, const uint32_t v[8]) {
#pragma unroll
  for (int j = 0; j < 8; ++j) {
    const uint32_t x = v[7 - j];
    dst[4 * j + 0] = (uint8_t)(x >> 24);
    dst[4 * j + 1] = (uint8_t)(x >> 16);
    dst[4 * j + 2] = (uint8_t)(x >> 8);
    dst[4 * j + 3] = (uint8_t)x;
  }
}

enum : uint32_t { GEN_CLS_MSG = 0, GEN_CLS_R = 1, GEN_CLS_S = 2, GEN_CLS_KEY = 3, GEN_CLS_NEGKEY = 4, GEN_NCLS = 5 };
__global__ void __launch_bounds__(WG) hkv_gen_records_kernel(uint64_t seed, uint64_t index0, uint32_t n,
                                                             const uint32_t* __restrict__ pool,
                                                             uint32_t npool, uint32_t unc_permille,
                                                             uint32_t invalid_permille,
                                                             uint8_t* __restrict__ recs,
                                                             uint32_t* __restrict__ labels) {
  const uint32_t i = blockIdx.x * WG + threadIdx.x;
  bool label = false;
  if (i < n) {
    const uint64_t g = index0 + i;
    uint64_t st = seed * 0xD1B54A32D192ED03ull + g * 0x9E3779B97F4A7C15ull + 0x8CB92BA72F3D8DD7ull;
    sc a, b;
    rand_scalar(a, st);
    rand_scalar(b, st);
    const uint64_t pick = splitmix64(st);
    const uint32_t j = (uint32_t)(pick % npool);
    const bool unc = ((pick >> 40) % 1000u) < unc_permille;
    ge q, R;
#pragma unroll
    for (int k = 0; k < 8; ++k) {
      q.x.v[k] = pool[(size_t)j * 16 + k];
      q.y.v[k] = pool[(size_t)j * 16 + 8 + k];
    }
    ecmult_simple(R, a, b, q);
    sc r, s, bi, m;
#pragma unroll
    for (int k = 0; k < 8; ++k) r.v[k] = R.x.v[k];
    sc_cond_sub_n(r.v);
    sc_inv(bi, b);
    sc_mul(s, r, bi);
    sc_mul(m, a, s);
    if (sc_is_high(s)) sc_neg(s, s);
    uint64_t mut = 0;
    bool bad = false;
    uint32_t cls = 0, bit = 0;
    if (invalid_permille) {
      mut = splitmix64(st);
      bad = (mut % 1000u) < invalid_permille;
      cls = (uint32_t)((mut >> 16) % GEN_NCLS);
      bit = (uint32_t)(mut >> 32) & 255u;
      if (bad && cls == GEN_CLS_KEY && npool > 1) {
        const uint32_t j2 = (j + 1u + (uint32_t)((mut >> 40) % (npool - 1u))) % npool;
#pragma unroll
        for (int k = 0; k < 8; ++k) {
          q.x.v[k] = pool[(size_t)j2 * 16 + k];
          q.y.v[k] = pool[(size_t)j2 * 16 + 8 + k];
        }
      }
      if (bad && cls == GEN_CLS_KEY && npool <= 1) cls = GEN_CLS_MSG;
      if (bad && cls == GEN_CLS_NEGKEY) {
        fe ny;
        fe_neg(ny, q.y);
        fe_normalize(ny);
        q.y = ny;
      }
    }
    label = !bad;
    uint8_t* o = recs + (size_t)i * REC_SIZE;
    put_be256(o, m.v);
    put_be256(o + 32, r.v);
    put_be256(o + 64, s.v);
    o[96] = unc ? 65 : 33;
    if (unc) {
      o[97] = 4;
      put_be256(o + 98, q.x.v);
      put_be256(o + 130, q.y.v);
    } else {
      o[97] = (uint8_t)(2u | (q.y.v[0] & 1u));
      put_be256(o + 98, q.x.v);
      for (int k = 130; k < 162; ++k) o[k] = 0;
    }
    for (int k = 162; k < REC_SIZE; ++k) o[k] = 0;
    if (bad && cls <= GEN_CLS_S) o[32u * cls + (bit >> 3)] ^= (uint8_t)(1u << (bit & 7u));
  }
  if (labels != nullptr) {
    const uint64_t ball = __ballot(label);
    if ((threadIdx.x & 63) == 0 && i < n) {
      const uint32_t wi = i / 32;
      labels[wi] = (uint32_t)ball;
      labels[wi + 1] = (uint32_t)(ball >> 32);
    }
  }
}

__global__ void __launch_bounds__(WG) hkv_gen_keys_kernel(uint64_t seed, uint32_t n, uint8_t* __restrict__ priv,
                                                          uint8_t* __restrict__ pub, uint8_t* __restrict__ h160) {
  const uint32_t i = blockIdx.x * WG + threadIdx.x;
  if (i >= n) return;
  uint64_t st = seed * 0x9FB21C651E98DF25ull + (uint64_t)i * 0x9E3779B97F4A7C15ull + 0x2545F4914F6CDD1Dull;
  sc d, zero;
  rand_scalar(d, st);
#pragma unroll
  for (int k = 0; k < 8; ++k) zero.v[k] = 0;
  ge g, q;
  ge_set_g(g);
  ecmult_simple(q, d, zero, g);
  put_be256(priv + (size_t)i * 32, d.v);
  uint8_t* pk = pub + (size_t)i * 33;
  pk[0] = (uint8_t)(2u | (q.y.v[0] & 1u));
  put_be256(pk + 1, q.x.v);
  uint32_t w[16], h[8], rip[5];
  w[0] = ((uint32_t)pk[0] << 24) | (q.x.v[7] >> 8);
#pragma unroll
  for (int k = 1; k < 8; ++k) w[k] = (q.x.v[8 - k] << 24) | (q.x.v[7 - k] >> 8);
  w[8] = (q.x.v[0] << 24) | 0x800000u;
#pragma unroll
  for (int k = 9; k < 15; ++k) w[k] = 0;
  w[15] = 33 * 8;
  sha256_init(h);
  sha256_compress(h, w);
  ripemd160_of_digest(rip, h);
  uint8_t* o = h160 + (size_t)i * 20;
#pragma unroll
  for (int k = 0; k < 20; ++k) o[k] = (uint8_t)(rip[k >> 2] >> (8 * (k & 3)));
}

__global__ void __launch_bounds__(WG) hkv_gen_sign_kernel(uint64_t seed, uint32_t n, const uint8_t* __restrict__ priv,
                                                          const uint32_t* __restrict__ key_idx,
                                                          const uint8_t* __restrict__ msg, uint32_t msg_stride,
                                                          uint8_t* __restrict__ sig) {
  const uint32_t i = blockIdx.x * WG + threadIdx.x;
  if (i >= n) return;
  uint64_t st = seed * 0xC2B2AE3D27D4EB4Full + (uint64_t)i * 0x9E3779B97F4A7C15ull + 0x165667B19E3779F9ull;
  const uint32_t kidx = key_idx ? key_idx[i] : i;
  sc d, m, k, zero, r, s, t, ki;
  const uint8_t* dp = priv + (size_t)kidx * 32;
  const uint8_t* mp = msg + (size_t)i * msg_stride;
#pragma unroll
  for (int q = 0; q < 8; ++q) {
    d.v[7 - q] = ((uint32_t)dp[4 * q] << 24) | ((uint32_t)dp[4 * q + 1] << 16) | ((uint32_t)dp[4 * q + 2] << 8) |
                 dp[4 * q + 3];
    m.v[7 - q] = ((uint32_t)mp[4 * q] << 24) | ((uint32_t)mp[4 * q + 1] << 16) | ((uint32_t)mp[4 * q + 2] << 8) |
                 mp[4 * q + 3];
    zero.v[q] = 0;
  }
  sc_cond_sub_n(m.v);
  rand_scalar(k, st);
  ge g, R;
  ge_set_g(g);
  ecmult_simple(R, k, zero, g);
#pragma unroll
  for (int q = 0; q < 8; ++q) r.v[q] = R.x.v[q];
  sc_cond_sub_n(r.v);
  sc_mul(t, r, d);
  sc_add(t, t, m);
  sc_inv(ki, k);
  sc_mul(s, ki, t);
  if (sc_is_high(s)) sc_neg(s, s);
  put_be256(sig + (size_t)i * 64, r.v);
  put_be256(sig + (size_t)i * 64 + 32, s.v);
}

__global__ void __launch_bounds__(WG) hkv_debug_kernel(uint32_t op, uint32_t n, const uint32_t* __restrict__ a,
                                                       const uint32_t* __restrict__ b,
                                                       uint32_t* __restrict__ out) {
  const uint32_t i = blockIdx.x * WG + threadIdx.x;
// ... 73 lines not shown
      if (s == 1u) fe_shl(z, x, 1);
      else fe_shl(z, x, (int)s);
      raw_norm(z);
      break;
    }
    case HKV_DBG_FE_SHL_VAR: fe_shl_var(z, x, y.v[0]); raw_norm(z); break;
    case HKV_DBG_FE_MUL_SMALL: fe_mul_small(z, x, y.v[0]); raw_norm(z); break;
    case HKV_DBG_FE_MUL_SMALL2: {
      fe xn, z2;
      load_next(xn, a);
      fe_mul_small2(z, x, y.v[0], z2, xn, y.v[1]);
      norm_pair(z, z2);
      break;
    }
    case HKV_DBG_FE_LIN2: {
      const uint32_t kk = b[inext * 8];
      fe_lin2(z, x, kk & 0xFFu, y, (kk >> 8) & 0xFFu);
      raw_norm(z);
      break;
    }
    case HKV_DBG_FE_MUL_ADD: {
      fe xn;
      load_next(xn, a);
      fe_mul_add(z, x, y, xn);
      raw_norm(z);
      break;
    }
    case HKV_DBG_FE_MUL2: {
      fe xn, yn, z2;
      load_next(xn, a);
      load_next(yn, b);
      fe_mul2(z, x, y, z2, xn, yn);
      norm_pair(z, z2);
      break;
    }
    case HKV_DBG_FE_SQR2: {
      fe z2;
      fe_sqr2(z, x, z2, y);
      norm_pair(z, z2);
      break;
    }
    case HKV_DBG_FE_SQRMUL: {
      fe xn, z2;
      load_next(xn, a);
      fe_sqrmul(z, x, z2, y, xn);
      norm_pair(z, z2);
      break;
    }
    case HKV_DBG_FE_MUL_REF: fe_mul_ref(z, x, y); raw_norm(z); break;
    case HKV_DBG_FE_SQR_REF: fe_sqr_ref(z, x); raw_norm(z); break;
    case HKV_DBG_FE_NORMALIZE: z = x; fe_normalize(z); for (int k = 0; k < 8; ++k) res[k] = z.v[k]; break;
    case HKV_DBG_FE_IS_ZERO: res[0] = fe_is_zero(x) ? 1u : 0u; break;
    case HKV_DBG_FE_EQUAL: res[0] = fe_equal(x, y) ? 1u : 0u; break;
    case HKV_DBG_U256_LT_P: res[0] = u256_lt_p(x.v) ? 1u : 0u; break;
    case HKV_DBG_SC_ADD: sc_add(wres, u, v); for (int k = 0; k < 8; ++k) res[k] = wres.v[k]; break;
    case HKV_DBG_SC_SUB: sc_sub(wres, u, v); for (int k = 0; k < 8; ++k) res[k] = wres.v[k]; break;
    case HKV_DBG_SC_NEG: sc_neg(wres, u); for (int k = 0; k < 8; ++k) res[k] = wres.v[k]; break;
    case HKV_DBG_SC_SQR: sc_sqr(wres, u); for (int k = 0; k < 8; ++k) res[k] = wres.v[k]; break;
    case HKV_DBG_SC_IS_HIGH: res[0] = sc_is_high(u) ? 1u : 0u; break;
    case HKV_DBG_INV_MOD_P: sgcd::inv_mod_p(res, x.v); break;
    case HKV_DBG_FE_MUL_SUM:
    case HKV_DBG_FE_MUL_SUM_RA:
    case HKV_DBG_FE_MUL_SUM_RB:
    case HKV_DBG_FE_MUL_SUM_RD: {
      fe xn, yn;
      load_next(xn, a);
      load_next(yn, b);
      if (op == HKV_DBG_FE_MUL_SUM_RA) { fe_mul_sum(x, x, y, xn, yn); z = x; }
      else if (op == HKV_DBG_FE_MUL_SUM_RB) { fe_mul_sum(y, x, y, xn, yn); z = y; }
      else if (op == HKV_DBG_FE_MUL_SUM_RD) { fe_mul_sum(yn, x, y, xn, yn); z = yn; }
      else fe_mul_sum(z, x, y, xn, yn);
      raw_norm(z);
      break;
    }
    case HKV_DBG_FE_SQRMUL_SUM:
    case HKV_DBG_FE_SQRMUL_SUM_RA:
    case HKV_DBG_FE_SQRMUL_SUM_RD: {
      fe xn;
      load_next(xn, a);
      if (op == HKV_DBG_FE_SQRMUL_SUM_RA) { fe_sqrmul_sum(x, x, y, xn); z = x; }
      else if (op == HKV_DBG_FE_SQRMUL_SUM_RD) { fe_sqrmul_sum(xn, x, y, xn); z = xn; }
      else fe_sqrmul_sum(z, x, y, xn);
      raw_norm(z);
      break;
    }
    case HKV_DBG_FE_NEG_COMPL: fe_neg_compl(z, x); raw_norm(z); break;
    default: break;
  }
#pragma unroll
  for (int k = 0; k < 16; ++k) out[i * 16 + k] = res[k];
}

__global__ void __launch_bounds__(WG) hkv_debug_group_kernel(uint32_t op, uint32_t lanes,
                                                             const uint32_t* __restrict__ a,
                                                             const uint32_t* __restrict__ b,
                                                             uint32_t* __restrict__ out) {
  const uint32_t i = blockIdx.x * WG + threadIdx.x;
  if (i >= lanes) return;
  sc k1, k2, zero;
  fe z1, w;
#pragma unroll
  for (int k = 0; k < 8; ++k) {
    k1.v[k] = a[(2 * i) * 8 + k];
    z1.v[k] = a[(2 * i + 1) * 8 + k];
    k2.v[k] = b[(2 * i) * 8 + k];
    w.v[k] = b[(2 * i + 1) * 8 + k];
    zero.v[k] = 0;
  }
  const uint32_t sel = w.v[0];
  const bool take = (sel & 1u) != 0;
  ge g, p1, p2, o;
  ge_set_g(g);
  fe_set_zero(o.x);
  fe_set_zero(o.y);
  bool oinf = false;
  uint32_t flag = 0;
  if (op == HKV_DBG_X_MATCHES_R) {
    fe X, zz, xin;
#pragma unroll
    for (int k = 0; k < 8; ++k) xin.v[k] = k1.v[k];
    fe_sqr(zz, z1);
    fe_mul(X, xin, zz);
    o.x.v[0] = x_matches_r(X, z1, k2.v) ? 1u : 0u;
  } else if (op == HKV_DBG_ECMULT) {
    sc kp;
#pragma unroll
    for (int k = 0; k < 8; ++k) kp.v[k] = z1.v[k];
    p1 = g;
    const bool pok = ecmult_simple(p2, kp, zero, g);
    if (!pok) p2 = g;
    oinf = !ecmult_simple(p1, k1, k2, p2);
    if (!oinf) o = p1;
  } else {
    p1 = g;
    p2 = g;
    ge t;
    const bool ok1 = ecmult_simple(t, k1, zero, g);
    if (ok1) p1 = t;
    const bool ok2 = ecmult_simple(t, k2, zero, g);
    if (ok2) p2 = t;
    gej acc;
    fe zz, zzz;
    fe_sqr(zz, z1);
    fe_mul(zzz, zz, z1);
    fe_mul(acc.x, p1.x, zz);
    fe_mul(acc.y, p1.y, zzz);
    acc.z = z1;
    bool inf = !ok1 || (sel & 2u) != 0;
    switch (op) {
      case HKV_DBG_GEJ_DOUBLE: gej_double(acc, acc); break;
      case HKV_DBG_GEJ_DOUBLE_ILP: gej_double_ilp(acc, acc); break;
      case HKV_DBG_GEJ_ACCUMULATE: gej_accumulate(acc, inf, acc.z, p2.x, p2.y, take); break;
      case HKV_DBG_GEJ_ACCUMULATE_ILP: gej_accumulate_ilp(acc, inf, acc.z, p2.x, p2.y, take); break;
      case HKV_DBG_GEJ_ADD_AFFINE_COMPLETE: gej_add_affine_complete(acc, inf, p2, take); break;
      case HKV_DBG_GEJ_ADD_VAR: {
        gej bj;
        fe_sqr(zz, w);
        fe_mul(zzz, zz, w);
        fe_mul(bj.x, p2.x, zz);
        fe_mul(bj.y, p2.y, zzz);
        bj.z = w;
        gej_add_var(acc, inf, bj, !ok2 || (sel & 4u) != 0);
        break;
      }
      default: break;
    }
    oinf = inf;
    if (!inf) {
      fe zi, zi2, zi3;
      fe_inv(zi, acc.z);
      fe_sqr(zi2, zi);
      fe_mul(zi3, zi2, zi);
      fe_mul(o.x, acc.x, zi2);
      fe_mul(o.y, acc.y, zi3);
      fe_normalize(o.x);
      fe_normalize(o.y);
    }
  }
  flag = oinf ? 1u : 0u;
#pragma unroll
  for (int k = 0; k < 8; ++k) {
    out[(2 * i) * 16 + k] = oinf ? 0u : o.x.v[k];
    out[(2 * i) * 16 + 8 + k] = oinf ? 0u : o.y.v[k];
  }
  out[(2 * i + 1) * 16] = flag;
#pragma unroll
  for (int k = 1; k < 16; ++k) out[(2 * i + 1) * 16 + k] = 0;
}

}

namespace hkv {

enum : uint32_t { TQ_CLAIM = 0, TQ_DONE = 1, TQ_SLOT = 8 };
HKV_DEV bool tail_wait(const MsTail& a, unsigned int* done, uint32_t want) {
  uint32_t spins = 0;
  while (a.force_fault || __hip_atomic_load(done, __ATOMIC_ACQUIRE, __HIP_MEMORY_SCOPE_AGENT) < want) {
    if (a.force_fault || spins++ >= (1u << 24)) {
      atomicOr(a.fault, 1u);
      if (a.status) atomicOr(a.status, (uint32_t)HKV_STATUS_TAIL_FAULT);
      return false;
    }
    __builtin_amdgcn_s_sleep(8);
  }
  return true;
}
HKV_DEV void publish_count(unsigned int* ctr) {
  __builtin_amdgcn_s_waitcnt(0);
  __syncthreads();
  if (threadIdx.x == 0) __hip_atomic_fetch_add(ctr, 1u, __ATOMIC_RELEASE, __HIP_MEMORY_SCOPE_AGENT);
}

__global__ void __launch_bounds__(PAIR_TPB, 1) hkv_ms_tail_kernel(MsTail a) {
  __shared__ QLane qlds[2];
  __shared__ HLane hlds[2];
  __shared__ uint32_t xch[25 * PAIR_SIGS];
  __shared__ uint32_t buf[16 * PAIR_TPB];
  __shared__ TailItem item_s;
  __shared__ uint32_t go_s;
  unsigned int* q = a.bar + (a.epoch & 1u) * TQ_SLOT;
  if (blockIdx.x == 0 && threadIdx.x == 0) {
    unsigned int* nx = a.bar + ((a.epoch + 1u) & 1u) * TQ_SLOT;
#pragma unroll
    for (int k = 0; k < (int)TQ_SLOT; ++k) __hip_atomic_store(&nx[k], 0u, __ATOMIC_RELAXED, __HIP_MEMORY_SCOPE_AGENT);
    __hip_atomic_store(a.total_next, 0ull, __ATOMIC_RELAXED, __HIP_MEMORY_SCOPE_AGENT);
  }
  const unsigned long long total = __hip_atomic_load(a.total, __ATOMIC_RELAXED, __HIP_MEMORY_SCOPE_AGENT);
  const uint32_t n_cand = (uint32_t)total, n_keys = (uint32_t)(total >> 32);
  if (n_keys == 0) return;
  const uint32_t T = PAIR_TPB;
  const uint32_t n1 = (a.hash_txs != TX_HASHES_NONE) ? (3 * a.n_tx + T - 1) / T : 0;
  const TailPlan plan = tail_plan(a.n, n1, n_cand, n_keys, a.win_cand, a.win_keys, T, PAIR_SIGS);
  const uint32_t slots = gridDim.x * PAIR_SIGS, sbase = blockIdx.x * PAIR_SIGS;
  const StdArgs none{};
  uint32_t seen = 0;
  for (;;) {
    if (threadIdx.x == 0) {
      const uint32_t it = atomicAdd(&q[TQ_CLAIM], 1u);
      uint32_t ok = it < plan.e4 ? 1u : 0u;
      if (ok) {
        const TailItem x = tail_item(plan, it);
        if (x.start > seen) {
          ok = tail_wait(a, &q[TQ_DONE], x.start) ? 1u : 0u;
          if (ok) seen = x.start;
        }
        item_s = x;
      }
      go_s = ok;
    }
    __syncthreads();
    const TailItem x = item_s;
    const uint32_t go = go_s;
    __syncthreads();
    if (!go) return;
    if (x.kind == TAIL_HASH) {
      const uint32_t t_ = x.idx * T + threadIdx.x;
      bool go1 = t_ < 3 * a.n_tx;
      const uint32_t t = go1 ? t_ % a.n_tx : 0, which = go1 ? t_ / a.n_tx : 0;
      uint32_t row[8] = {0, 0, 0, 0, 0, 0, 0, 0};
      if (go1) tx_index_row(a.txs, a.tx_off, t, row);
      if (go1 && a.hash_txs == TX_HASHES_WITNESS) go1 = (row[TXT_FLAGS] & TXF_WITNESS) != 0;
      tx_hash_word_lane(a.txs, row, a.txt + (size_t)t * TXT_WORDS, which, go1, buf);
    } else if (x.kind == TAIL_EMIT) {
      const uint32_t jx = x.idx * T + threadIdx.x;
      ms_emit_lane(a.txs, a.n_tx, a.txt, a.scripts, a.scripts_len, a.jobs, jx, jx < a.n, a.forkid, a.desc, a.off,
                   a.cand, a.keyrec, x.cw0, plan.Wc, x.kw0, plan.Wk, buf);
    } else if (x.kind == TAIL_KEYS) {
      key_check_lane(reinterpret_cast<const uint32_t*>(a.keyrec), x.first + threadIdx.x, x.end, a.kbits, x.kw0);
    } else if (x.kind == TAIL_CAND) {
      const int64_t shift = (int64_t)x.base - (int64_t)sbase;
      const int64_t rshift = shift - (int64_t)x.cw0;
      uint32_t* recs = reinterpret_cast<uint32_t*>(reinterpret_cast<uintptr_t>(a.cand) +
                                                   (uintptr_t)(rshift * (int64_t)(REC_WORDS * 4)));
      uint32_t* bits = reinterpret_cast<uint32_t*>(reinterpret_cast<uintptr_t>(a.cbits) +
                                                   (uintptr_t)(shift / 32 * 4));
      pair_group<false>(sbase, a.im, sbase + x.valid, slots, a.gtab, bits, 0xFFFFFFFFu, a.aux, recs,
                        HKV_MODE_HASKOIN, nullptr, none, qlds, hlds, xch, buf);
    } else {
      const uint32_t jx = x.idx * T + threadIdx.x;
      ms_resolve_lane(a.desc, a.off, jx, jx < a.n, a.cbits, a.kbits, a.out_bits);
    }
    publish_count(&q[TQ_DONE]);
  }
}


}

namespace hkv {

static inline uint32_t ceil_div(size_t a, uint32_t b) { return (uint32_t)((a + b - 1) / b); }

hipError_t launch_prologue(const RecPlan& p, const RecOps& r, hipStream_t st) {
  hipLaunchKernelGGL(hkv_prologue_kernel, dim3(ceil_div(p.n_pad, WG)), dim3(WG), 0, st, (const uint32_t*)r.recs, r.n,
                     p.n_pad, r.mode, r.im);
  hipError_t e = hipGetLastError();
  if (e != hipSuccess) return e;
  hipLaunchKernelGGL(hkv_inv_kernel, dim3(ceil_div(p.inv_stride, WG)), dim3(WG), 0, st, p.n_pad, p.inv_stride, r.im);
  e = hipGetLastError();
  if (e != hipSuccess) return e;
  hipLaunchKernelGGL(hkv_glv_kernel, dim3(ceil_div(p.n_pad, WG)), dim3(WG), 0, st, p.n_pad, r.im);
  return hipGetLastError();
}
static hipError_t launch_table_chain(const RecPlan& p, const RecOps& r, hipStream_t st) {
  if (p.chunk_len < (uint32_t)WG || p.chunk_len % WG != 0) return hipErrorInvalidValue;
  for (uint32_t k = 0; k < p.n_chunks; ++k) {
    const uint32_t i0 = p.chunk(k).i0, cn = p.chunk(k).cn;
    hipLaunchKernelGGL(hkv_qtable_kernel, dim3(cn / WG), dim3(WG), 0, st, (const uint32_t*)r.im, r.n, p.n_pad, i0, cn,
                       r.qs);
    hipError_t e = hipGetLastError();
    if (e != hipSuccess) return e;
    hipLaunchKernelGGL(hkv_chain_kernel, dim3(cn / WG), dim3(WG), 0, st, r.im, r.n, p.n_pad, i0, cn,
                       (const uint32_t*)r.qs, i0 == 0 ? r.clk : nullptr);
    e = hipGetLastError();
    if (e != hipSuccess) return e;
  }
  return hipSuccess;
}
static StdArgs std_args(const StdOps& o) {
  return StdArgs{o.txs, o.n_tx, o.txt, o.scripts, o.scripts_len, o.jobs, o.forkid, nullptr, nullptr, nullptr, nullptr};
}
static hipError_t launch_mid_std(const RecPlan& p, const RecOps& r, const StdOps& o, hipStream_t st);
hipError_t launch_ecmult(const RecPlan& p, const RecOps& r, const StdOps* std_pro, hipStream_t st) {
  if (std_pro != nullptr && p.shape != Shape::Mid) return hipErrorInvalidValue;
  uint32_t* rw = const_cast<uint32_t*>((const uint32_t*)r.recs);
  switch (p.shape) {
    case Shape::Block:
      hipLaunchKernelGGL(hkv_block_kernel<false>, dim3(p.grid), dim3(BLK_TPB), 0, st, r.im, r.n, p.n_pad, r.gtab, r.qs,
                         r.bits, r.n_words, r.aux, rw, r.mode, r.clk, StdArgs{});
      break;
    case Shape::Pair:
      hipLaunchKernelGGL(hkv_pair_split_kernel<false>, dim3(p.grid), dim3(PAIR_TPB), 0, st, r.im, r.n, p.n_pad, r.gtab,
                         r.bits, r.n_words, r.aux, rw, r.mode, r.clk, StdArgs{});
      break;
    case Shape::Mid:
      if (std_pro != nullptr) return launch_mid_std(p, r, *std_pro, st);
      hipLaunchKernelGGL((hkv_ecmult_kernel<true, false>), dim3(p.grid), dim3(WG), 0, st, r.im, r.n, p.n_pad, r.qs,
                         r.clk, StdArgs{});
      break;
    case Shape::TableChain: return launch_table_chain(p, r, st);
    default: return hipErrorInvalidValue;
  }
  return hipGetLastError();
}
hipError_t launch_std_verify_split(const StdPlan& p, const StdOps& o, const RecOps& r, const MsScan* ms,
                                   const uint32_t* tx_off, hipStream_t st) {
  StdArgs sa = std_args(o);
  uint32_t* rw = const_cast<uint32_t*>((const uint32_t*)r.recs);
  switch (p.shape) {
    case Shape::Block:
      if (ms != nullptr) {
        sa.ms_desc = ms->desc;
        sa.ms_off = ms->off;
        sa.ms_ctr = reinterpret_cast<unsigned long long*>(ms->counters);
      }
      sa.tx_off = tx_off;
      hipLaunchKernelGGL(hkv_block_kernel<true>, dim3(p.n_pad / BLK_SIGS), dim3(BLK_TPB), 0, st, r.im, r.n, p.n_pad,
                         r.gtab, r.qs, r.bits, r.n_words, r.aux, rw, (uint32_t)HKV_MODE_HASKOIN, r.clk, sa);
      break;
    case Shape::Pair:
      if (tx_off != nullptr) return hipErrorInvalidValue;
      hipLaunchKernelGGL(hkv_pair_split_kernel<true>, dim3(p.n_pad / PAIR_SIGS), dim3(PAIR_TPB), 0, st, r.im, r.n,
                         p.n_pad, r.gtab, r.bits, r.n_words, r.aux, rw, (uint32_t)HKV_MODE_HASKOIN, r.clk, sa);
      break;
    default: return hipErrorInvalidValue;
  }
  return hipGetLastError();
}
uint32_t ms_tail_slots(uint32_t n_cu) { return n_cu * PAIR_SIGS; }
hipError_t launch_ms_tail(const MsTail& a, uint32_t grid, hipStream_t st) {
  hipLaunchKernelGGL(hkv_ms_tail_kernel, dim3(grid), dim3(PAIR_TPB), 0, st, a);
  return hipGetLastError();
}
hipError_t launch_gtable(uint32_t* gtab, hipStream_t st) {
  hipLaunchKernelGGL(hkv_gtable_kernel, dim3(ceil_div((size_t)GTAB_TABLES * GTAB_ENTRIES, WG)), dim3(WG), 0, st,
                     gtab);
  return hipGetLastError();
}
static hipError_t launch_mid_std(const RecPlan& p, const RecOps& r, const StdOps& o, hipStream_t st) {
  hipLaunchKernelGGL((hkv_ecmult_kernel<true, true>), dim3(p.grid), dim3(WG), 0, st, r.im, r.n, p.n_pad, r.qs, r.clk,
                     std_args(o));
  return hipGetLastError();
}
hipError_t launch_finish(const RecPlan& p, const RecOps& r, uint32_t* rare_ctr, const void* late_recs,
                         hipStream_t st) {
  if (p.shape != Shape::Mid && p.shape != Shape::TableChain) return hipErrorInvalidValue;
  const bool paired = p.shape == Shape::Mid;
  const uint32_t* lr = static_cast<const uint32_t*>(late_recs);
  const dim3 g(p.n_pad / WG), b(WG);
  if (paired && lr)
    hipLaunchKernelGGL((hkv_finish_kernel<true, true>), g, b, 0, st, r.im, r.n, p.n_pad, r.gtab, rare_ctr, lr);
  else if (paired)
    hipLaunchKernelGGL((hkv_finish_kernel<true, false>), g, b, 0, st, r.im, r.n, p.n_pad, r.gtab, rare_ctr, lr);
  else if (lr)
    hipLaunchKernelGGL((hkv_finish_kernel<false, true>), g, b, 0, st, r.im, r.n, p.n_pad, r.gtab, rare_ctr, lr);
  else
    hipLaunchKernelGGL((hkv_finish_kernel<false, false>), g, b, 0, st, r.im, r.n, p.n_pad, r.gtab, rare_ctr, lr);
  hipError_t e = hipGetLastError();
  if (e != hipSuccess) return e;
  hipLaunchKernelGGL(hkv_rare_kernel, dim3(p.n_pad / WG), dim3(WG), 0, st, r.im, p.n_pad, (const uint32_t*)rare_ctr);
  e = hipGetLastError();
  if (e != hipSuccess) return e;
  hipLaunchKernelGGL(hkv_yverdict_kernel, dim3(p.verdict_stride / WG), dim3(WG), 0, st, r.im, p.n_pad,
                     p.verdict_stride, r.bits, r.n_words, rare_ctr);
  return hipGetLastError();
}
hipError_t launch_gen_pool(uint64_t seed, uint32_t npool, uint32_t* pool, hipStream_t st) {
  hipLaunchKernelGGL(hkv_gen_pool_kernel, dim3(ceil_div(npool, WG)), dim3(WG), 0, st, seed, npool, pool);
  return hipGetLastError();
}
hipError_t launch_gen_records(uint64_t seed, uint64_t index0, uint32_t n, const uint32_t* pool, uint32_t npool,
                              uint32_t unc_permille, uint32_t invalid_permille, void* recs, uint32_t* labels,
                              hipStream_t st) {
  hipLaunchKernelGGL(hkv_gen_records_kernel, dim3(ceil_div(n, WG)), dim3(WG), 0, st, seed, index0, n, pool, npool,
                     unc_permille, invalid_permille, (uint8_t*)recs, labels);
  return hipGetLastError();
}
hipError_t launch_debug(uint32_t op, uint32_t n, const uint32_t* a, const uint32_t* b, uint32_t* out,
                        hipStream_t st) {
  if (op >= HKV_DBG_GEJ_DOUBLE) {
    if (n < 2) return hipErrorInvalidValue;
    hipLaunchKernelGGL(hkv_debug_group_kernel, dim3(ceil_div(n / 2, WG)), dim3(WG), 0, st, op, n / 2, a, b, out);
    return hipGetLastError();
  }
  hipLaunchKernelGGL(hkv_debug_kernel, dim3(ceil_div(n, WG)), dim3(WG), 0, st, op, n, a, b, out);
  return hipGetLastError();
}
hipError_t launch_gen_keys(uint64_t seed, uint32_t n, uint8_t* priv, uint8_t* pub, uint8_t* h160, hipStream_t st) {
  hipLaunchKernelGGL(hkv_gen_keys_kernel, dim3(ceil_div(n, WG)), dim3(WG), 0, st, seed, n, priv, pub, h160);
  return hipGetLastError();
}
hipError_t launch_gen_sign(uint64_t seed, uint32_t n, const uint8_t* priv, const uint32_t* key_idx,
                           const uint8_t* msg, uint32_t msg_stride, uint8_t* sig, hipStream_t st) {
  hipLaunchKernelGGL(hkv_gen_sign_kernel, dim3(ceil_div(n, WG)), dim3(WG), 0, st, seed, n, priv, key_idx, msg,
                     msg_stride, sig);
  return hipGetLastError();
}
hipError_t ecmult_max_blocks_per_cu(int* out) {
  const hipError_t e = hipOccupancyMaxActiveBlocksPerMultiprocessor(out, hkv_chain_kernel, WG, 0);
  if (e == hipSuccess && *out > HKV_ECMULT_WAVES) *out = HKV_ECMULT_WAVES;
  return e;
}

}
```

haskoin-node_amd/csrc/hkv_launch_plan.h:

```cpp
#pragma once
#include <stddef.h>
#include <stdint.h>

#include "hkv_layout.h"

namespace hkv {

struct Geometry {
  uint32_t n_cu = 0;
  uint32_t grid_max = 0;
  size_t rec_chunk = 0;
  size_t std_chunk = 0;
};

constexpr size_t SPLIT_DIV = 8;
constexpr uint32_t MIN_INV_LANES = 65536;

enum class Shape : uint32_t {
  Block = 1,
  Pair = 2,
  Mid = 3,
  TableChain = 4,
};

struct RecChunk {
  uint32_t i0, cn;
};

struct RecPlan {
  Shape shape;
  uint32_t n_pad;
  uint32_t grid;
  bool prologue;
  bool aux;
  uint32_t inv_stride, verdict_stride;
  size_t qs_quads;
  uint32_t chunk_len, n_chunks;
  RecChunk chunk(uint32_t k) const {
    const uint64_t i0 = (uint64_t)k * chunk_len;
    const uint64_t left = n_pad - i0;
    return RecChunk{(uint32_t)i0, (uint32_t)(left < chunk_len ? left : chunk_len)};
  }
};

namespace plan_detail {
inline size_t round_up(size_t a, size_t b) { return (a + b - 1) / b * b; }
inline size_t grid_lanes(const Geometry& g) { return (size_t)g.grid_max * WG; }
inline Shape shape_of(const Geometry& g, size_t n_pad) {
  if (n_pad > grid_lanes(g) / 2) return Shape::TableChain;
  if (n_pad > grid_lanes(g) / SPLIT_DIV) return Shape::Mid;
  return n_pad <= (size_t)BLK_SIGS * g.n_cu ? Shape::Block : Shape::Pair;
}
}

inline RecPlan plan_records(const Geometry& g, size_t n) {
  using namespace plan_detail;
  const size_t n_pad = round_up(n, WG);
  RecPlan p{};
  p.shape = shape_of(g, n_pad);
  p.n_pad = (uint32_t)n_pad;
  const bool small = p.shape == Shape::Block || p.shape == Shape::Pair;
  p.prologue = !small;
  p.aux = small;
  const size_t blocks = n_pad / WG;
  switch (p.shape) {
    case Shape::Block: p.grid = (uint32_t)(n_pad / BLK_SIGS); break;
    case Shape::Pair: p.grid = (uint32_t)(n_pad / PAIR_SIGS); break;
    case Shape::Mid: p.grid = (uint32_t)(blocks < g.grid_max / 2 ? blocks : g.grid_max / 2); break;
    case Shape::TableChain: p.grid = 0; break;
  }
  const size_t min_lanes = n_pad < MIN_INV_LANES ? n_pad : MIN_INV_LANES;
  const size_t inv = (n_pad + BATCH_INV - 1) / BATCH_INV;
  p.inv_stride = (uint32_t)(inv > MIN_INV_LANES ? inv : min_lanes);
  const size_t ver = round_up((n_pad + VERDICT_BATCH - 1) / VERDICT_BATCH, WG);
  p.verdict_stride = (uint32_t)(ver < min_lanes ? min_lanes : ver);
  p.qs_quads = grid_lanes(g) * QTAB_QUADS;
  p.chunk_len = p.n_pad;
  p.n_chunks = 1;
  if (p.shape == Shape::TableChain) {
    const size_t chunk = n_pad < g.rec_chunk ? n_pad : g.rec_chunk;
    const size_t quads = chunk * (QTAB_QUADS + QTAB_ZG_QUADS);
    if (quads > p.qs_quads) p.qs_quads = quads;
    p.chunk_len = (uint32_t)chunk;
    p.n_chunks = (uint32_t)((n_pad + chunk - 1) / chunk);
  }
  return p;
}

enum class ScanOn : uint32_t {
  Kernel = 0,
  MainStream = 1,
  HashStream = 2,
};

struct StdPlan {
  Shape shape;
  uint32_t n_pad;
  bool scan_in_kernel, rows_in_kernel;
  bool overlap;
  bool index_first;
  bool index_hashes, tail_hashes;
  ScanOn scan;
};

inline StdPlan plan_std_chunk(const Geometry& g, size_t n) {
  using namespace plan_detail;
  const size_t n_pad = round_up(n, WG);
  StdPlan p{};
  p.shape = shape_of(g, n_pad);
  p.n_pad = (uint32_t)n_pad;
  p.scan_in_kernel = p.rows_in_kernel = p.shape == Shape::Block;
  p.overlap = p.shape == Shape::Mid;
  p.index_first = !p.rows_in_kernel;
  p.index_hashes = p.shape == Shape::TableChain;
  p.tail_hashes = p.shape == Shape::Block || p.shape == Shape::Pair;
  p.scan = p.scan_in_kernel ? ScanOn::Kernel : p.overlap ? ScanOn::HashStream : ScanOn::MainStream;
  return p;
}

inline size_t std_chunk_len(const Geometry& g, size_t n) {
  return n > plan_detail::grid_lanes(g) ? g.std_chunk : plan_detail::grid_lanes(g) / 2;
}

}
```

haskoin-node_amd/csrc/hkv_layout.h:

```cpp
#pragma once
#include <stdint.h>

namespace hkv {

constexpr int REC_SIZE = 168;
constexpr int REC_WORDS = REC_SIZE / 4;

#ifndef HKV_QW
#define HKV_QW 4
#endif
#ifndef HKV_GTAB_W
#define HKV_GTAB_W 20
#endif
constexpr int QW = HKV_QW;
static_assert(QW == 4 || QW == 5, "radix-16 or radix-32 Q windows");
constexpr int GTAB_W = HKV_GTAB_W;
static_assert(GTAB_W % QW == 0 && GTAB_W >= 8 && GTAB_W <= 28, "G windows sit on Q window boundaries");
constexpr int NWIN = (130 + QW - 1) / QW;
constexpr int QBIAS = 1 << (QW - 1);
constexpr int QDIG_BITS = QW + 1;
constexpr uint32_t QDIG_MASK = (1u << QDIG_BITS) - 1u;
constexpr int GWIN = (128 + GTAB_W) / GTAB_W;
constexpr int GSTEP = GTAB_W / QW;
constexpr uint32_t GD_MAG = (1u << GTAB_W) - 1u, GD_NEG = 1u << GTAB_W;
constexpr uint32_t DIG_ZERO = (uint32_t)QBIAS | ((uint32_t)QBIAS << QDIG_BITS);

#ifndef HKV_BATCH_INV
#define HKV_BATCH_INV 16
#endif
constexpr int BATCH_INV = HKV_BATCH_INV;
#ifndef HKV_VERDICT_BATCH
#define HKV_VERDICT_BATCH 16
#endif
constexpr int VERDICT_BATCH = HKV_VERDICT_BATCH;
constexpr int PAIR_SIGS = 32;
constexpr int BLK_SIGS = 16;


constexpr uint32_t FLAG_VALID = 1u;
constexpr uint32_t FLAG_NEG1 = 2u;
constexpr uint32_t FLAG_NEG2 = 4u;
constexpr uint32_t FLAG_GLV_OVF = 8u;
constexpr uint32_t FLAG_YODD = 16u;
constexpr uint32_t FLAG_COMP = 32u;
constexpr uint32_t FLAG_BINF = 64u;
constexpr uint32_t FLAG_DECIDED = 128u;
constexpr uint32_t FLAG_ACCEPT = 256u;
constexpr uint32_t FLAG_RARE = 512u;
constexpr uint32_t FLAG_AINF = 1024u;
constexpr uint32_t AUXF_AINF = 1u, AUXF_SQ = 2u;
constexpr uint32_t AUXF_STDOK = 4u;

struct Field {
  int off, len;
};

constexpr Field IM_FLAGS = {0, 1};
constexpr Field IM_QX = {1, 8};
constexpr Field IM_W = {9, 8};
constexpr Field IM_S = {17, 8};
constexpr Field IM_M = {27, 8};
constexpr Field IM_R = {35, 8};
constexpr Field IM_C = {43, 8};
constexpr Field IM_DIG = {51, NWIN};
constexpr Field IM_GDIG = {84, 2 * GWIN};
constexpr int IM_WORDS = IM_GDIG.off + IM_GDIG.len;
constexpr Field IM_BX = {IM_DIG.off, 8};
constexpr Field IM_BY = {IM_DIG.off + 8, 8};
constexpr Field IM_BZ = {IM_DIG.off + 16, 8};
constexpr Field IM_NUM = {IM_DIG.off, 8};
constexpr Field IM_NUMN = {IM_DIG.off + 8, 8};
constexpr Field IM_DEN = {IM_DIG.off + 16, 8};
constexpr Field IM_AX = {IM_QX.off, 8};
constexpr Field IM_AY = {IM_S.off, 8};
constexpr Field IM_AZ = {IM_S.off + 8, 8};
constexpr Field IM_RARE_LIST = {IM_AZ.off + 8, 1};

constexpr Field AUX_AX = {0, 8};
constexpr Field AUX_AY = {8, 8};
constexpr Field AUX_AZ = {16, 8};
constexpr Field AUX_Y0 = {24, 8};
constexpr Field AUX_FLAGS = {32, 1};
constexpr Field AUX_SQ = {33, 1};
constexpr int AUX_WORDS = 34;

constexpr Field LIVE_PROLOGUE_INV[] = {IM_FLAGS, IM_QX, IM_W, IM_R, IM_S, IM_M};
constexpr Field LIVE_INV_GLV[] = {IM_FLAGS, IM_QX, IM_W, IM_R, IM_S, IM_M, IM_C};
constexpr Field LIVE_GLV_ECMULT[] = {IM_FLAGS, IM_QX, IM_W, IM_R, IM_C, IM_DIG, IM_GDIG};
constexpr Field LIVE_CHAIN_FINISH[] = {IM_FLAGS, IM_W, IM_R, IM_C, IM_BX, IM_BY, IM_BZ, IM_GDIG};
constexpr Field LIVE_FINISH_RARE[] = {IM_FLAGS, IM_W, IM_R, IM_RARE_LIST, IM_AX, IM_AY, IM_AZ, IM_BX, IM_BY, IM_BZ};
constexpr Field LIVE_FINISH_VERDICT[] = {IM_FLAGS, IM_W, IM_R, IM_RARE_LIST, IM_NUM, IM_NUMN, IM_DEN, IM_C};
constexpr Field LIVE_SMALL_IM[] = {IM_FLAGS, IM_R, IM_DIG, IM_GDIG};
constexpr Field LIVE_SMALL_AUX[] = {AUX_AX, AUX_AY, AUX_AZ, AUX_Y0, AUX_FLAGS, AUX_SQ};

constexpr bool fields_overlap(Field a, Field b) { return a.off < b.off + b.len && b.off < a.off + a.len; }
template <int N>
constexpr bool live_set_ok(const Field (&f)[N], int words) {
  for (int a = 0; a < N; ++a) {
    if (f[a].off < 0 || f[a].len < 1 || f[a].off + f[a].len > words) return false;
    for (int b = a + 1; b < N; ++b)
      if (fields_overlap(f[a], f[b])) return false;
  }
  return true;
}
static_assert(live_set_ok(LIVE_PROLOGUE_INV, IM_WORDS), "prologue -> inv");
static_assert(live_set_ok(LIVE_INV_GLV, IM_WORDS), "inv -> glv");
static_assert(live_set_ok(LIVE_GLV_ECMULT, IM_WORDS), "glv -> table / chain / mid-size");
static_assert(live_set_ok(LIVE_CHAIN_FINISH, IM_WORDS), "chain -> finish");
static_assert(live_set_ok(LIVE_FINISH_RARE, IM_WORDS), "finish -> rare");
static_assert(live_set_ok(LIVE_FINISH_VERDICT, IM_WORDS), "finish -> verdict");
static_assert(live_set_ok(LIVE_SMALL_IM, IM_WORDS), "small-batch im");
static_assert(live_set_ok(LIVE_SMALL_AUX, AUX_WORDS), "small-batch aux");

constexpr int GTAB_ENTRIES = 1 << (GTAB_W - 1);
constexpr int GTAB_TABLES = 2 * GWIN;
constexpr size_t GTAB_DWORDS = (size_t)GTAB_TABLES * GTAB_ENTRIES * 16;

constexpr int QTAB_ENTRIES = QBIAS;
constexpr int QTAB_QUADS_PER_ENTRY = 6;
constexpr int QTAB_QUADS = QTAB_ENTRIES * QTAB_QUADS_PER_ENTRY;

#ifndef HKV_REC_CHUNK
#define HKV_REC_CHUNK (1u << 20)
#endif
constexpr int QTAB_ZG_QUADS = 2;

constexpr int WG = 256;

enum : int {
  TXT_FLAGS = 0,
  TXT_INS = 1,
  TXT_NIN = 2,
  TXT_NOUT = 3,
  TXT_OUTS_FIRST = 4,
  TXT_OUTS_END = 5,
  TXT_LOCK = 6,
  TXT_START = 7,
  TXT_HP = 8,
  TXT_HS = 16,
  TXT_HO = 24,
  TXT_WORDS = 32,
};
constexpr uint32_t TXF_OK = 1u, TXF_WITNESS = 2u;
enum : uint32_t { TX_HASHES_NONE = 0, TX_HASHES_ALL = 1, TX_HASHES_WITNESS = 2 };

#ifndef HKV_ECMULT_WAVES
#define HKV_ECMULT_WAVES 4
#endif

}
```

haskoin-node_amd/hkv/lib.py:

```python
from __future__ import annotations

import ctypes
import os
from ctypes import POINTER, c_char_p, c_int, c_size_t, c_uint8, c_uint32, c_uint64, c_void_p

HKV_RECORD_SIZE = 168
HKV_LIBSECP = 0
HKV_HASKOIN = 1

HKV_SIGHASH_LEGACY = 0
HKV_SIGHASH_FORKID = 1
HKV_NO_FORKID = -1
HKV_SH_OK, HKV_SH_BAD_TX, HKV_SH_BAD_INPUT, HKV_SH_BAD_REF = 0, 1, 2, 3

HKV_HDR_POW_OK, HKV_HDR_LINK_OK, HKV_HDR_NEGATIVE, HKV_HDR_OVERFLOW = 0x01, 0x02, 0x04, 0x08
HKV_HDR_ZERO_TARGET, HKV_HDR_ABOVE_LIMIT, HKV_HDR_HASH_ABOVE = 0x10, 0x20, 0x40

HKV_TXID_OK, HKV_TXID_BAD_TX = 0, 1
HKV_BLK_MERKLE_OK, HKV_BLK_MUTATED, HKV_BLK_BAD_TX, HKV_BLK_EMPTY = 0x01, 0x02, 0x04, 0x08

HKV_OK = 0
HKV_FAIL_NONE, HKV_FAIL_ENQUEUE, HKV_FAIL_JOIN, HKV_FAIL_ALLOC, HKV_FAIL_TAIL = 0, 1, 2, 3, 4
HKV_STATUS_TAIL_FAULT = 1
HKV_STATUS_INPUT_COUNT = 2
HKV_SRC_NONE, HKV_SRC_LIST = 0xFFFFFFFF, 0xFFFFFFFE
HKV_SPEND_RESOLVED, HKV_SPEND_FIRST, HKV_SPEND_IN_RANGE, HKV_SPEND_OUT_RANGE = 0x01, 0x02, 0x04, 0x08
HKV_SPEND_BALANCED, HKV_SPEND_COINBASE, HKV_SPEND_OK = 0x10, 0x20, 0x1F
_ERRS = {-1: "HKV_E_ARG", -2: "HKV_E_NODEV", -3: "HKV_E_OOM", -4: "HKV_E_HIP", -5: "HKV_E_INTERNAL"}

_PKG_DIR = os.path.dirname(os.path.dirname(os.path.abspath(__file__)))


def lib_path() -> str:
    return os.environ.get("HKV_LIB", os.path.join(_PKG_DIR, "lib", "libhkv.so"))


class HkvError(RuntimeError):
    def __init__(self, rc: int, what: str, lib=None):
        detail = ""
        if lib is not None:
            try:
                detail = lib.hkv_last_hip_error().decode()
            except Exception:
                detail = ""
        super().__init__(f"{what}: {_ERRS.get(rc, rc)} {detail}".strip())
        self.rc = rc


class HkvTxs(ctypes.Structure):
    _fields_ = [("bytes", c_void_p), ("offsets", c_void_p), ("n_tx", c_uint32), ("scripts", c_void_p),
                ("scripts_len", c_uint32)]


class HkvSighashJob(ctypes.Structure):
    _fields_ = [("tx", c_uint32), ("input", c_uint32), ("script_off", c_uint32), ("script_len", c_uint32),
                ("value", c_uint64), ("sighash", c_uint32), ("kind", c_uint32)]


class HkvInputJob(ctypes.Structure):
    _fields_ = [("tx", c_uint32), ("input", c_uint32), ("script_off", c_uint32), ("script_len", c_uint32),
                ("value", c_uint64)]


assert ctypes.sizeof(HkvSighashJob) == 32 and ctypes.sizeof(HkvInputJob) == 24

EXPORTS = {
    "hkv_open": (c_int, [c_int, c_uint32, POINTER(c_void_p)]),
    "hkv_open_devices": (c_int, [POINTER(c_int), c_int, c_uint32, POINTER(c_void_p)]),
    "hkv_close": (None, [c_void_p]),
    "hkv_ctx_num_devices": (c_int, [c_void_p]),
    "hkv_device_healthy": (c_int, [c_void_p, c_int]),
    "hkv_device_failures": (c_int, [c_void_p, c_int]),
    "hkv_device_reset_health": (c_int, [c_void_p, c_int]),
    "hkv_debug_fail_device": (c_int, [c_void_p, c_int, c_uint32]),
    "hkv_debug_ms_window": (c_int, [c_void_p, c_int, c_uint32, c_uint32]),
    "hkv_debug_ms_scratch": (c_int, [c_void_p, c_int, POINTER(c_size_t)]),
    "hkv_debug_q_scratch": (c_int, [c_void_p, c_int, POINTER(c_size_t), POINTER(c_size_t)]),
    "hkv_debug_launch_shape": (c_int, [c_void_p, c_int, c_uint32, c_size_t, POINTER(c_uint32)]),
    "hkv_debug_ms_tail_counts": (c_int, [c_void_p, c_int, POINTER(c_uint64)]),
    "hkv_batch_alloc": (c_int, [c_void_p, c_size_t, POINTER(c_void_p)]),
    "hkv_batch_free": (None, [c_void_p]),
    "hkv_batch_records": (POINTER(c_uint8), [c_void_p]),
    "hkv_batch_capacity": (c_size_t, [c_void_p]),
    "hkv_verify": (c_int, [c_void_p, c_void_p, c_size_t, c_uint32, POINTER(c_uint32)]),
    "hkv_verify_host": (c_int, [c_void_p, c_void_p, c_size_t, c_uint32, POINTER(c_uint32)]),
    "hkv_verify_device": (c_int, [c_void_p, c_int, c_void_p, c_size_t, c_uint32, c_void_p, c_void_p]),
    "hkv_gen_records_device": (c_int, [c_void_p, c_int, c_uint64, c_size_t, c_uint32, c_uint32, c_void_p,
                                       c_void_p]),
    "hkv_gen_batch_device": (c_int, [c_void_p, c_int, c_uint64, c_uint64, c_size_t, c_uint32, c_uint32, c_uint32,
                                     c_void_p, c_void_p, c_void_p]),
    "hkv_sighash": (c_int, [c_void_p, POINTER(HkvTxs), c_void_p, c_size_t, ctypes.c_int32, c_void_p, c_void_p]),
    "hkv_sighash_device": (c_int, [c_void_p, c_int, POINTER(HkvTxs), c_void_p, c_size_t, ctypes.c_int32, c_void_p,
                                   c_size_t, c_void_p, c_void_p]),
    "hkv_std_inputs_device": (c_int, [c_void_p, c_int, POINTER(HkvTxs), c_void_p, c_size_t, ctypes.c_int32,
                                      c_void_p, c_void_p]),
    "hkv_verify_std_inputs_device": (c_int, [c_void_p, c_int, POINTER(HkvTxs), c_void_p, c_size_t, ctypes.c_int32,
                                             c_void_p, c_void_p, c_void_p]),
    "hkv_verify_std_inputs_device_status": (c_int, [c_void_p, c_int, POINTER(HkvTxs), c_void_p, c_size_t,
                                                    ctypes.c_int32, c_void_p, c_void_p, c_void_p, c_void_p]),
    "hkv_device_fault": (c_int, [c_void_p, c_int, POINTER(c_uint32)]),
    "hkv_verify_std_inputs": (c_int, [c_void_p, POINTER(HkvTxs), c_void_p, c_size_t, ctypes.c_int32,
                                      POINTER(c_uint32)]),
    "hkv_std_tx_jobs_device": (c_int, [c_void_p, c_int, POINTER(HkvTxs), c_void_p, c_void_p, c_void_p, c_void_p,
                                       c_size_t, c_void_p, c_void_p, c_void_p, c_void_p]),
    "hkv_tx_verdicts_device": (c_int, [c_void_p, c_int, c_void_p, c_size_t, c_void_p, c_void_p, c_void_p]),
    "hkv_verify_std_txs_device": (c_int, [c_void_p, c_int, POINTER(HkvTxs), c_void_p, c_void_p, c_void_p, c_void_p,
                                          ctypes.c_int32, c_size_t, c_void_p, c_void_p, c_void_p, c_void_p, c_void_p,
                                          c_void_p, c_void_p]),
    "hkv_verify_std_txs": (c_int, [c_void_p, POINTER(HkvTxs), c_void_p, c_void_p, c_void_p, c_void_p, ctypes.c_int32,
                                   POINTER(c_uint32)]),
    "hkv_txid_table_slots": (c_size_t, [c_size_t]),
    "hkv_txid_index_device": (c_int, [c_void_p, c_int, c_void_p, c_size_t, c_void_p, c_size_t, c_void_p]),
    "hkv_txid_lookup_device": (c_int, [c_void_p, c_int, c_void_p, c_size_t, c_void_p, c_size_t, c_void_p, c_size_t,
                                       c_void_p, c_void_p]),
    "hkv_block_tx_jobs_device": (c_int, [c_void_p, c_int, POINTER(HkvTxs), c_void_p, c_void_p, c_void_p, c_void_p,
                                         c_size_t, c_void_p, c_void_p, c_size_t, c_void_p, c_void_p, c_void_p,
                                         c_void_p, c_void_p]),
    "hkv_verify_block_txs_device": (c_int, [c_void_p, c_int, POINTER(HkvTxs), c_void_p, c_void_p, c_void_p, c_void_p,
                                            ctypes.c_int32, c_size_t, c_void_p, c_void_p, c_size_t, c_void_p,
                                            c_void_p, c_void_p, c_void_p, c_void_p, c_void_p, c_void_p, c_void_p]),
    "hkv_verify_block_txs": (c_int, [c_void_p, POINTER(HkvTxs), c_void_p, c_void_p, c_void_p, c_void_p,
                                     ctypes.c_int32, POINTER(c_uint32), c_void_p, c_void_p, c_size_t]),
    "hkv_debug_txid_hash_mask": (c_int, [c_void_p, c_int, c_uint32]),
    "hkv_spend_table_slots": (c_size_t, [c_size_t]),
    "hkv_block_spends_device": (c_int, [c_void_p, c_int, POINTER(HkvTxs), c_void_p, c_void_p, c_void_p, c_size_t,
                                        c_uint64, c_void_p, c_void_p, c_size_t, c_void_p, c_void_p, c_void_p,
                                        c_void_p, c_void_p]),
    "hkv_verify_block_txs_spends": (c_int, [c_void_p, POINTER(HkvTxs), c_void_p, c_void_p, c_void_p, c_void_p,
                                            ctypes.c_int32, c_uint64, POINTER(c_uint32), c_void_p, c_void_p,
                                            c_void_p, c_size_t, c_void_p, c_void_p]),
    "hkv_debug_spend_stages": (c_int, [c_void_p, c_int, c_uint32]),
    "hkv_merkle_roots": (c_int, [c_void_p, c_void_p, c_void_p, c_size_t, c_void_p, c_void_p]),
    "hkv_merkle_roots_device": (c_int, [c_void_p, c_int, c_void_p, c_void_p, c_size_t, c_void_p, c_void_p, c_void_p,
                                        c_void_p]),
    "hkv_tx_ids": (c_int, [c_void_p, POINTER(HkvTxs), c_void_p, c_void_p]),
    "hkv_tx_ids_device": (c_int, [c_void_p, c_int, POINTER(HkvTxs), c_void_p, c_void_p, c_void_p]),
    "hkv_check_blocks": (c_int, [c_void_p, POINTER(HkvTxs), c_void_p, c_size_t, c_void_p, c_void_p, c_void_p,
                                 c_void_p]),
    "hkv_check_blocks_device": (c_int, [c_void_p, c_int, POINTER(HkvTxs), c_void_p, c_size_t, c_void_p, c_void_p,
                                        c_void_p, c_void_p, c_void_p, c_void_p, c_void_p]),
    "hkv_check_headers": (c_int, [c_void_p, c_void_p, c_size_t, c_void_p, c_void_p, c_void_p, c_void_p]),
    "hkv_check_headers_device": (c_int, [c_void_p, c_int, c_void_p, c_size_t, c_void_p, c_void_p, c_void_p, c_void_p,
                                         c_void_p]),
    "hkv_gen_keys_device": (c_int, [c_void_p, c_int, c_uint64, c_size_t, c_void_p, c_void_p, c_void_p, c_void_p]),
    "hkv_gen_sign_device": (c_int, [c_void_p, c_int, c_uint64, c_size_t, c_void_p, c_void_p, c_void_p, c_size_t,
                                    c_void_p, c_void_p]),
    "hkv_debug_op": (c_int, [c_void_p, c_int, c_uint32, c_size_t, c_void_p, c_void_p, c_void_p, c_void_p]),
    "hkv_profile_enable": (c_int, [c_void_p, c_int]),
    "hkv_profile_read": (c_int, [c_void_p, c_int, POINTER(ctypes.c_double), POINTER(ctypes.c_double),
                                 POINTER(c_uint64)]),
    "hkv_profile_clock": (c_int, [c_void_p, c_int, POINTER(ctypes.c_double)]),
    "hkv_profile_phases": (c_int, [c_void_p, c_int, POINTER(c_uint64), c_size_t, POINTER(ctypes.c_double)]),
    "hkv_profile_group_stamps": (c_int, [c_void_p, c_int, POINTER(c_uint64), c_size_t, POINTER(ctypes.c_double)]),
    "hkv_strerror": (c_char_p, [c_int]),
    "hkv_last_hip_error": (c_char_p, []),
    "hkv_device_count": (c_int, []),
    "hkv_version": (c_uint32, []),
}

MEASUREMENT_ONLY = {"hkv_profile_group_stamps", "hkv_debug_q_scratch", "hkv_debug_launch_shape"}

_LIB = None


def load_library(path: str | None = None):
    global _LIB
    if _LIB is not None and path is None:
        return _LIB
    p = path or lib_path()
    if not os.path.exists(p):
        raise ImportError(f"libhkv.so not built at {p}; run __graft_entry__.build()")
    lib = ctypes.CDLL(p)
    for name, (res, args) in EXPORTS.items():
        if name in MEASUREMENT_ONLY and not hasattr(lib, name):
            continue
        fn = getattr(lib, name)
        fn.restype = res
        fn.argtypes = args
    if path is None:
        _LIB = lib
    return lib


def check(rc: int, what: str, lib=None) -> None:
    if rc != HKV_OK:
        raise HkvError(rc, what, lib)
```

include/hkv.h:

```cpp
#ifndef HKV_H
#define HKV_H

#include <stddef.h>
#include <stdint.h>

#ifdef __cplusplus
extern "C" {
#endif

#define HKV_RECORD_SIZE 168

#define HKV_LIBSECP 0u
#define HKV_HASKOIN 1u

enum hkv_err {
  HKV_OK = 0,
  HKV_E_ARG = -1,
  HKV_E_NODEV = -2,
  HKV_E_OOM = -3,
  HKV_E_HIP = -4,
  HKV_E_INTERNAL = -5,
};

typedef struct hkv_ctx hkv_ctx;
typedef struct hkv_batch hkv_batch;

#define HKV_OPEN_NO_SELFCHECK 1u

int hkv_open(int n_gpus, uint32_t flags, hkv_ctx** out);
int hkv_open_devices(const int* device_ids, int n_ids, uint32_t flags, hkv_ctx** out);
void hkv_close(hkv_ctx* ctx);
int hkv_ctx_num_devices(const hkv_ctx* ctx);
int hkv_device_healthy(hkv_ctx* ctx, int dev);
int hkv_device_reset_health(hkv_ctx* ctx, int dev);
int hkv_device_failures(hkv_ctx* ctx, int dev);
#define HKV_FAIL_NONE 0u
#define HKV_FAIL_ENQUEUE 1u
#define HKV_FAIL_JOIN 2u
#define HKV_FAIL_ALLOC 3u
#define HKV_FAIL_TAIL 4u
int hkv_debug_fail_device(hkv_ctx* ctx, int dev, uint32_t when);
int hkv_debug_ms_window(hkv_ctx* ctx, int dev, uint32_t cand_records, uint32_t key_records);
int hkv_debug_ms_scratch(hkv_ctx* ctx, int dev, size_t* bytes);
int hkv_debug_q_scratch(hkv_ctx* ctx, int dev, size_t* bytes, size_t* chunk);
int hkv_debug_launch_shape(hkv_ctx* ctx, int dev, uint32_t kind, size_t n, uint32_t out[4]);
int hkv_debug_ms_tail_counts(hkv_ctx* ctx, int dev, uint64_t out[3]);

int hkv_batch_alloc(hkv_ctx* ctx, size_t max_n, hkv_batch** out);
void hkv_batch_free(hkv_batch* b);
uint8_t* hkv_batch_records(hkv_batch* b);
size_t hkv_batch_capacity(const hkv_batch* b);

int hkv_verify(hkv_ctx* ctx, hkv_batch* b, size_t n, uint32_t mode, uint32_t* verdict_bits);

int hkv_verify_host(hkv_ctx* ctx, const uint8_t* records, size_t n, uint32_t mode, uint32_t* verdict_bits);

int hkv_verify_device(hkv_ctx* ctx, int dev, const void* d_records, size_t n, uint32_t mode,
                      uint32_t* d_bits, void* hip_stream);

int hkv_gen_records_device(hkv_ctx* ctx, int dev, uint64_t seed, size_t n, uint32_t pool_size,
                           uint32_t uncompressed_permille, void* d_records, void* hip_stream);
int hkv_gen_batch_device(hkv_ctx* ctx, int dev, uint64_t seed, uint64_t index0, size_t n, uint32_t pool_size,
                         uint32_t uncompressed_permille, uint32_t invalid_permille, void* d_records,
                         uint32_t* d_labels, void* hip_stream);

typedef struct hkv_txs {
  const uint8_t* bytes;
  const uint32_t* offsets;
  uint32_t n_tx;
  const uint8_t* scripts;
  uint32_t scripts_len;
} hkv_txs;

#define HKV_SIGHASH_LEGACY 0u
#define HKV_SIGHASH_FORKID 1u
#define HKV_NO_FORKID (-1)

typedef struct hkv_sighash_job {
  uint32_t tx;
  uint32_t input;
  uint32_t script_off;
  uint32_t script_len;
  uint64_t value;
  uint32_t sighash;
  uint32_t kind;
} hkv_sighash_job;

#define HKV_SH_OK 0u
#define HKV_SH_BAD_TX 1u
#define HKV_SH_BAD_INPUT 2u
#define HKV_SH_BAD_REF 3u

typedef struct hkv_input_job {
  uint32_t tx;
  uint32_t input;
  uint32_t script_off;
  uint32_t script_len;
  uint64_t value;
} hkv_input_job;

int hkv_sighash(hkv_ctx* ctx, const hkv_txs* txs, const hkv_sighash_job* jobs, size_t n, int32_t forkid,
                uint8_t* out32, uint8_t* status);
int hkv_sighash_device(hkv_ctx* ctx, int dev, const hkv_txs* d_txs, const hkv_sighash_job* d_jobs, size_t n,
                       int32_t forkid, uint8_t* d_out, size_t out_stride, uint8_t* d_status, void* hip_stream);
int hkv_std_inputs_device(hkv_ctx* ctx, int dev, const hkv_txs* d_txs, const hkv_input_job* d_jobs, size_t n,
                          int32_t forkid, void* d_records, void* hip_stream);
int hkv_verify_std_inputs_device(hkv_ctx* ctx, int dev, const hkv_txs* d_txs, const hkv_input_job* d_jobs, size_t n,
                                 int32_t forkid, void* d_records, uint32_t* d_bits, void* hip_stream);
#define HKV_STATUS_TAIL_FAULT 1u
int hkv_verify_std_inputs_device_status(hkv_ctx* ctx, int dev, const hkv_txs* d_txs, const hkv_input_job* d_jobs,
                                        size_t n, int32_t forkid, void* d_records, uint32_t* d_bits,
                                        uint32_t* d_status, void* hip_stream);
int hkv_device_fault(hkv_ctx* ctx, int dev, uint32_t* fault);
int hkv_verify_std_inputs(hkv_ctx* ctx, const hkv_txs* txs, const hkv_input_job* jobs, size_t n, int32_t forkid,
                          uint32_t* verdict_bits);

#define HKV_STATUS_INPUT_COUNT 2u
int hkv_std_tx_jobs_device(hkv_ctx* ctx, int dev, const hkv_txs* d_txs, const uint32_t* d_prev_offsets,
                           const uint8_t* d_prev_outpoints, const uint32_t* d_prev_scripts,
                           const uint64_t* d_prev_values, size_t n_inputs, uint32_t* d_input_first,
                           hkv_input_job* d_jobs, uint32_t* d_status, void* hip_stream);
int hkv_tx_verdicts_device(hkv_ctx* ctx, int dev, const uint32_t* d_input_first, size_t n_tx,
                           const uint32_t* d_input_bits, uint32_t* d_tx_bits, void* hip_stream);
int hkv_verify_std_txs_device(hkv_ctx* ctx, int dev, const hkv_txs* d_txs, const uint32_t* d_prev_offsets,
                              const uint8_t* d_prev_outpoints, const uint32_t* d_prev_scripts,
                              const uint64_t* d_prev_values, int32_t forkid, size_t n_inputs,
                              uint32_t* d_input_first, hkv_input_job* d_jobs, void* d_records,
                              uint32_t* d_input_bits, uint32_t* d_tx_bits, uint32_t* d_status, void* hip_stream);
int hkv_verify_std_txs(hkv_ctx* ctx, const hkv_txs* txs, const uint32_t* prev_offsets,
                       const uint8_t* prev_outpoints, const uint32_t* prev_scripts, const uint64_t* prev_values,
                       int32_t forkid, uint32_t* tx_verdict_bits);

#define HKV_HDR_POW_OK 0x01u
#define HKV_HDR_LINK_OK 0x02u
#define HKV_HDR_NEGATIVE 0x04u
#define HKV_HDR_OVERFLOW 0x08u
#define HKV_HDR_ZERO_TARGET 0x10u
#define HKV_HDR_ABOVE_LIMIT 0x20u
#define HKV_HDR_HASH_ABOVE 0x40u

int hkv_check_headers(hkv_ctx* ctx, const uint8_t* headers, size_t n, const uint8_t* pow_limit,
                      const uint8_t* prev_hash, uint8_t* hashes_out, uint8_t* status);
int hkv_check_headers_device(hkv_ctx* ctx, int dev, const uint8_t* d_headers, size_t n, const uint8_t* d_pow_limit,
                             const uint8_t* d_prev_hash, uint8_t* d_hashes, uint8_t* d_status, void* hip_stream);

int hkv_merkle_roots(hkv_ctx* ctx, const uint8_t* txids, const uint32_t* offsets, size_t n_blocks,
                     uint8_t* roots_out, uint8_t* mutated);
int hkv_merkle_roots_device(hkv_ctx* ctx, int dev, const uint8_t* d_txids, const uint32_t* d_offsets,
                            size_t n_blocks, uint8_t* d_scratch, uint8_t* d_roots, uint8_t* d_mutated,
                            void* hip_stream);

#define HKV_TXID_OK 0u
#define HKV_TXID_BAD_TX 1u
int hkv_tx_ids(hkv_ctx* ctx, const hkv_txs* txs, uint8_t* txids_out, uint8_t* status);
int hkv_tx_ids_device(hkv_ctx* ctx, int dev, const hkv_txs* d_txs, uint8_t* d_txids, uint8_t* d_status,
                      void* hip_stream);

#define HKV_BLK_MERKLE_OK 0x01u
#define HKV_BLK_MUTATED 0x02u
#define HKV_BLK_BAD_TX 0x04u
#define HKV_BLK_EMPTY 0x08u
int hkv_check_blocks(hkv_ctx* ctx, const hkv_txs* txs, const uint32_t* block_offsets, size_t n_blocks,
                     const uint8_t* headers, uint8_t* txids_out, uint8_t* roots_out, uint8_t* status);
int hkv_check_blocks_device(hkv_ctx* ctx, int dev, const hkv_txs* d_txs, const uint32_t* d_block_offsets,
                            size_t n_blocks, const uint8_t* d_headers, uint8_t* d_txids, uint8_t* d_scratch,
                            uint8_t* d_roots, uint8_t* d_mutated, uint8_t* d_status, void* hip_stream);

#define HKV_SRC_NONE 0xFFFFFFFFu
#define HKV_SRC_LIST 0xFFFFFFFEu
size_t hkv_txid_table_slots(size_t n_tx);
int hkv_txid_index_device(hkv_ctx* ctx, int dev, const uint8_t* d_txids, size_t n_tx, uint32_t* d_table,
                          size_t n_slots, void* hip_stream);
int hkv_txid_lookup_device(hkv_ctx* ctx, int dev, const uint8_t* d_txids, size_t n_tx, const uint32_t* d_table,
                           size_t n_slots, const uint8_t* d_queries32, size_t n_q, uint32_t* d_found,
                           void* hip_stream);
int hkv_block_tx_jobs_device(hkv_ctx* ctx, int dev, const hkv_txs* d_txs, const uint32_t* d_prev_offsets,
                             const uint8_t* d_prev_outpoints, const uint32_t* d_prev_scripts,
                             const uint64_t* d_prev_values, size_t n_inputs, uint8_t* d_txids, uint32_t* d_table,
                             size_t n_slots, uint32_t* d_input_first, hkv_input_job* d_jobs, uint32_t* d_input_src,
                             uint32_t* d_status, void* hip_stream);
int hkv_verify_block_txs_device(hkv_ctx* ctx, int dev, const hkv_txs* d_txs, const uint32_t* d_prev_offsets,
                                const uint8_t* d_prev_outpoints, const uint32_t* d_prev_scripts,
                                const uint64_t* d_prev_values, int32_t forkid, size_t n_inputs, uint8_t* d_txids,
                                uint32_t* d_table, size_t n_slots, uint32_t* d_input_first, hkv_input_job* d_jobs,
                                uint32_t* d_input_src, void* d_records, uint32_t* d_input_bits, uint32_t* d_tx_bits,
                                uint32_t* d_status, void* hip_stream);
int hkv_verify_block_txs(hkv_ctx* ctx, const hkv_txs* txs, const uint32_t* prev_offsets,
                         const uint8_t* prev_outpoints, const uint32_t* prev_scripts, const uint64_t* prev_values,
                         int32_t forkid, uint32_t* tx_verdict_bits, uint32_t* input_first, uint32_t* input_src,
                         size_t input_src_cap);
int hkv_debug_txid_hash_mask(hkv_ctx* ctx, int dev, uint32_t mask);

#define HKV_SPEND_RESOLVED 0x01u
#define HKV_SPEND_FIRST 0x02u
#define HKV_SPEND_IN_RANGE 0x04u
#define HKV_SPEND_OUT_RANGE 0x08u
#define HKV_SPEND_BALANCED 0x10u
#define HKV_SPEND_COINBASE 0x20u
#define HKV_SPEND_OK 0x1Fu
size_t hkv_spend_table_slots(size_t n_inputs);
int hkv_block_spends_device(hkv_ctx* ctx, int dev, const hkv_txs* d_txs, const uint32_t* d_input_first,
                            const hkv_input_job* d_jobs, const uint32_t* d_input_src, size_t n_inputs,
                            uint64_t max_money, uint32_t* d_input_off, uint32_t* d_table, size_t n_slots,
                            uint32_t* d_input_spender, uint64_t* d_tx_sums, uint8_t* d_tx_flags, uint32_t* d_status,
                            void* hip_stream);
int hkv_verify_block_txs_spends(hkv_ctx* ctx, const hkv_txs* txs, const uint32_t* prev_offsets,
                                const uint8_t* prev_outpoints, const uint32_t* prev_scripts,
                                const uint64_t* prev_values, int32_t forkid, uint64_t max_money,
                                uint32_t* tx_verdict_bits, uint32_t* input_first, uint32_t* input_src,
                                uint32_t* input_spender, size_t input_cap, uint64_t* tx_sums, uint8_t* tx_flags);
int hkv_debug_spend_stages(hkv_ctx* ctx, int dev, uint32_t stages);

int hkv_gen_keys_device(hkv_ctx* ctx, int dev, uint64_t seed, size_t n, uint8_t* d_priv, uint8_t* d_pub,
                        uint8_t* d_h160, void* hip_stream);
int hkv_gen_sign_device(hkv_ctx* ctx, int dev, uint64_t seed, size_t n, const uint8_t* d_priv,
                        const uint32_t* d_key_idx, const uint8_t* d_msg, size_t msg_stride, uint8_t* d_sig,
                        void* hip_stream);

int hkv_debug_op(hkv_ctx* ctx, int dev, uint32_t op, size_t n, const uint32_t* d_a, const uint32_t* d_b,
                 uint32_t* d_out, void* hip_stream);

int hkv_profile_enable(hkv_ctx* ctx, int on);
int hkv_profile_read(hkv_ctx* ctx, int dev, double* prologue_ms, double* ecmult_ms, uint64_t* launches);
int hkv_profile_clock(hkv_ctx* ctx, int dev, double* sclk_mhz);

int hkv_profile_phases(hkv_ctx* ctx, int dev, uint64_t* stamps, size_t n, double* tick_ns);

int hkv_profile_group_stamps(hkv_ctx* ctx, int dev, uint64_t* stamps, size_t n_groups, double* tick_ns);

const char* hkv_strerror(int err);
const char* hkv_last_hip_error(void);
int hkv_device_count(void);
uint32_t hkv_version(void);

#ifdef __cplusplus
}
#endif
#endif
```

Baseline: 124.8 million.

## Pipeline table-chain parts across two streams with per-part finish kernels

Splits the TableChain shape into parts, set to half a chunk by default. Consecutive parts alternate between the main stream and a new high-priority pipe stream, each with its own q-table scratch slot. The finish, rare and verdict kernels now run per part right after that part's chain, so the finish work of one part can overlap the table and chain work of the next. Rare counters become per-part arrays. The change adds stream fork and join overhead, and it risks scratch-slot reuse ordering bugs and smaller kernel launches with lower occupancy.

```diff
diff --git a/haskoin-node_amd/csrc/hkv_api.cpp b/haskoin-node_amd/csrc/hkv_api.cpp
--- a/haskoin-node_amd/csrc/hkv_api.cpp
+++ b/haskoin-node_amd/csrc/hkv_api.cpp
@@ -94,6 +94,8 @@
   hipStream_t copy_stream = nullptr;
   hipStream_t hash_stream = nullptr;
   hipEvent_t ev_fork = nullptr, ev_join = nullptr;
+  hipStream_t pipe_stream = nullptr;
+  hipEvent_t ev_pipe_fork = nullptr, ev_pipe_join = nullptr;
   DevBuf<uint32_t> gtab, qs;
   DevBuf<uint32_t> im;
   DevBuf<uint32_t> bits;
@@ -162,6 +164,7 @@
 constexpr size_t MS_CAND_PER_INPUT = hkv::MS_CAND_PER_INPUT, MS_KEYS_PER_INPUT = hkv::MS_KEYS_PER_INPUT;
 constexpr size_t HKV_MAX_STD_INPUTS = 0xFFFFFF00ull;
 constexpr size_t MS_BAR_WORDS = 32, MS_FAULT = 16, MS_HOST_STATUS = 17;
+constexpr size_t RARE_CTR_WORDS = HKV_MAX_STD_INPUTS / ((HKV_REC_PART) != 0 ? (HKV_REC_PART) : HKV_MAX_STD_INPUTS) + 1;
 #ifndef HKV_HOST_FIRST_DIV
 #define HKV_HOST_FIRST_DIV 4
 #endif
@@ -193,6 +196,75 @@
     for (auto& x : e) HKV_TRY(hipEventCreate(&x), "hipEventCreate");
   HKV_TRY(hipEventRecord(e[k], st), "hipEventRecord");
   if (k == 2) d.ev.insert(d.ev.end(), e, e + 3);
+  return HKV_OK;
+}
+
+int ensure_rare(DevCtx& d, size_t count) {
+  if (d.rare_ctr.get() != nullptr && d.rare_ctr.size() >= count) return HKV_OK;
+  d.rare_dirty = true;
+  return d.rare_ctr.reserve(count, "hipMalloc(rare counters)");
+}
+int rearm_rare(DevCtx& d, hipStream_t st) {
+  if (!d.rare_dirty) return HKV_OK;
+  HKV_TRY(hipMemsetAsync(d.rare_ctr, 0, d.rare_ctr.size() * sizeof(uint32_t), st), "hipMemset(rare counters)");
+  d.rare_dirty = false;
+  return HKV_OK;
+}
+
+int enqueue_table_chain(DevCtx& d, const hkv::RecPlan& plan, const hkv::RecOps& ops, hipEvent_t late_join,
+                        const void* late_recs, hipStream_t st) {
+  const bool piped = plan.qs_slots == 2;
+  const hipStream_t streams[2] = {st, d.pipe_stream};
+  HKV_RC(rearm_rare(d, st));
+  if (piped) {
+    HKV_TRY(hipEventRecord(d.ev_pipe_fork, st), "hipEventRecord(pipe fork)");
+    HKV_TRY(hipStreamWaitEvent(d.pipe_stream, d.ev_pipe_fork, 0), "hipStreamWaitEvent(pipe fork)");
+  }
+  hipError_t err = hipSuccess;
+  const char* what = nullptr;
+  bool slot_order = true;
+  uint32_t slot_user[2] = {0, 0};
+  bool late_joined[2] = {late_join == nullptr, late_join == nullptr};
+  for (uint32_t k = 0; k < plan.n_parts; ++k) {
+    const uint32_t lane = piped ? hkv::RecPlan::part_stream(k) : 0u, slot = piped ? hkv::RecPlan::part_slot(k) : 0u;
+    const hipStream_t s = streams[lane];
+    if (k >= 2 && slot_user[slot] != lane) {
+      slot_order = false;
+      break;
+    }
+    slot_user[slot] = lane;
+    err = hkv::launch_table_chain(plan, ops, k, s);
+    if (err != hipSuccess) {
+      what = "ecmult launch";
+      break;
+    }
+    if (!piped) continue;
+    if (!late_joined[lane]) err = hipStreamWaitEvent(s, late_join, 0);
+    late_joined[lane] = true;
+    if (err == hipSuccess) err = hkv::launch_finish(plan, ops, plan.part(k), d.rare_ctr + k, late_recs, s);
+    if (err != hipSuccess) {
+      what = "finish launch";
+      break;
+    }
+  }
+  if (piped) {
+    hipError_t e = hipEventRecord(d.ev_pipe_join, d.pipe_stream);
+    if (e == hipSuccess) e = hipStreamWaitEvent(st, d.ev_pipe_join, 0);
+    if (err == hipSuccess && e != hipSuccess) err = e, what = "pipe join";
+  } else if (err == hipSuccess && slot_order) {
+    if (late_join != nullptr) err = hipStreamWaitEvent(st, late_join, 0);
+    if (err == hipSuccess) err = hkv::launch_finish(plan, ops, hkv::RecChunk{0, plan.n_pad}, d.rare_ctr, late_recs, st);
+    what = "finish launch";
+  }
+  if (!slot_order) {
+    d.rare_dirty = true;
+    g_last_hip = "a part's table launch is not ordered after its slot's last chain launch";
+    return HKV_E_INTERNAL;
+  }
+  if (err != hipSuccess) {
+    d.rare_dirty = true;
+    return hip_fail(err, what);
+  }
   return HKV_OK;
 }
 
@@ -205,19 +277,22 @@
   HKV_RC(profile_mark(d, e, 0, st));
   if (std_pro != nullptr && plan.shape != hkv::Shape::Mid) return HKV_E_INTERNAL;
   if (plan.aux) HKV_RC(ensure_aux(d, plan.n_pad));
+  if (plan.prologue) HKV_RC(ensure_rare(d, plan.qs_slots == 2 ? plan.n_parts : 1));
   const hkv::RecOps ops{d.im, (uint32_t)n, d.gtab, d.qs, out_bits ? out_bits : d.bits.get(),
                         (uint32_t)(out_bits ? (n + 31) / 32 : plan.n_pad / 32), d.profile ? d.clk.get() : nullptr,
                         d.aux, d_records, mode};
   if (plan.prologue && std_pro == nullptr) HKV_TRY(hkv::launch_prologue(plan, ops, st), "prologue launch");
   HKV_RC(profile_mark(d, e, 1, st));
+  const void* late_recs = late_join != nullptr ? d_records : nullptr;
+  if (plan.shape == hkv::Shape::TableChain) {
+    HKV_RC(enqueue_table_chain(d, plan, ops, late_join, late_recs, st));
+    return profile_mark(d, e, 2, st);
+  }
   HKV_TRY(hkv::launch_ecmult(plan, ops, std_pro, st), "ecmult launch");
   if (plan.prologue) {
     if (late_join != nullptr) HKV_TRY(hipStreamWaitEvent(st, late_join, 0), "hipStreamWaitEvent(hash join)");
-    if (d.rare_dirty) {
-      HKV_TRY(hipMemsetAsync(d.rare_ctr, 0, sizeof(uint32_t), st), "hipMemset(rare counter)");
-      d.rare_dirty = false;
-    }
-    const hipError_t e2 = hkv::launch_finish(plan, ops, d.rare_ctr, late_join != nullptr ? d_records : nullptr, st);
+    HKV_RC(rearm_rare(d, st));
+    const hipError_t e2 = hkv::launch_finish(plan, ops, hkv::RecChunk{0, plan.n_pad}, d.rare_ctr, late_recs, st);
     if (e2 != hipSuccess) {
       d.rare_dirty = true;
       return hip_fail(e2, "finish launch");
@@ -242,14 +317,19 @@
   HKV_TRY(hipStreamCreateWithFlags(&d.hash_stream, hipStreamNonBlocking), "hipStreamCreate(hash)");
   HKV_TRY(hipEventCreateWithFlags(&d.ev_fork, hipEventDisableTiming), "hipEventCreate(fork)");
   HKV_TRY(hipEventCreateWithFlags(&d.ev_join, hipEventDisableTiming), "hipEventCreate(join)");
+  int prio_least = 0, prio_greatest = 0;
+  HKV_TRY(hipDeviceGetStreamPriorityRange(&prio_least, &prio_greatest), "stream priority range");
+  HKV_TRY(hipStreamCreateWithPriority(&d.pipe_stream, hipStreamNonBlocking, prio_greatest), "hipStreamCreate(pipe)");
+  HKV_TRY(hipEventCreateWithFlags(&d.ev_pipe_fork, hipEventDisableTiming), "hipEventCreate(pipe fork)");
+  HKV_TRY(hipEventCreateWithFlags(&d.ev_pipe_join, hipEventDisableTiming), "hipEventCreate(pipe join)");
   HKV_TRY(hipEventCreateWithFlags(&d.last_use, hipEventDisableTiming), "hipEventCreate(scratch)");
   HKV_TRY(hipEventRecord(d.last_use, d.stream), "hipEventRecord(scratch)");
   HKV_RC(d.ms_ctr.reserve(4, "hipMalloc(multisig counters)"));
   HKV_TRY(hipMemsetAsync(d.ms_ctr, 0, 4 * sizeof(uint64_t), d.stream), "hipMemset(multisig counters)");
   HKV_RC(d.ms_bar.reserve(MS_BAR_WORDS, "hipMalloc(multisig barrier)"));
   HKV_TRY(hipMemsetAsync(d.ms_bar, 0, MS_BAR_WORDS * sizeof(unsigned int), d.stream), "hipMemset(multisig barrier)");
-  HKV_RC(d.rare_ctr.reserve(1, "hipMalloc(rare counter)"));
-  HKV_TRY(hipMemsetAsync(d.rare_ctr, 0, sizeof(uint32_t), d.stream), "hipMemset(rare counter)");
+  HKV_RC(d.rare_ctr.reserve(RARE_CTR_WORDS, "hipMalloc(rare counters)"));
+  HKV_TRY(hipMemsetAsync(d.rare_ctr, 0, RARE_CTR_WORDS * sizeof(uint32_t), d.stream), "hipMemset(rare counters)");
   HKV_TRY(hipStreamSynchronize(d.stream), "multisig counters sync");
   HKV_TRY(hipDeviceGetAttribute(&d.wall_khz, hipDeviceAttributeWallClockRate, device), "wall clock rate");
   HKV_RC(d.clk.reserve(CLK_WORDS, "hipMalloc(clock probe)"));
@@ -273,6 +353,11 @@
     const unsigned long long c = std::strtoull(e, nullptr, 10) / hkv::WG * hkv::WG;
     if (c >= (unsigned long long)hkv::WG && c <= HKV_REC_CHUNK) g.rec_chunk = (size_t)c;
   }
+  g.rec_part = HKV_REC_PART;
+  if (const char* e = std::getenv("HKV_REC_PART")) {
+    const unsigned long long c = std::strtoull(e, nullptr, 10);
+    if (c <= HKV_REC_CHUNK) g.rec_part = (size_t)c;
+  }
   HKV_RC(d.qs.reserve(hkv::plan_records(g, 1).qs_quads * 4, "hipMalloc(qtab scratch)"));
   HKV_TRY(hkv::launch_gtable(d.gtab, d.stream), "gtable launch");
   HKV_TRY(hipStreamSynchronize(d.stream), "gtable sync");
@@ -290,9 +375,9 @@
   if (d.stream) (void)hipStreamSynchronize(d.stream);
   (void)hipDeviceSynchronize();
   clear_events(d);
-  for (hipEvent_t e : {d.last_use, d.ev_fork, d.ev_join})
+  for (hipEvent_t e : {d.last_use, d.ev_fork, d.ev_join, d.ev_pipe_fork, d.ev_pipe_join})
     if (e) (void)hipEventDestroy(e);
-  for (hipStream_t s : {d.stream, d.copy_stream, d.hash_stream})
+  for (hipStream_t s : {d.stream, d.copy_stream, d.hash_stream, d.pipe_stream})
     if (s) (void)hipStreamDestroy(s);
   d = DevCtx();
 }
@@ -683,6 +768,14 @@
     out[1] = (p.scan_in_kernel ? 1u : 0u) | (p.rows_in_kernel ? 2u : 0u) | (p.overlap ? 4u : 0u);
     out[2] = (uint32_t)first, out[3] = (uint32_t)((n + chunk - 1) / chunk);
   }
+  return HKV_OK;
+}
+
+int hkv_debug_rec_parts(hkv_ctx* ctx, int dev, size_t n, uint32_t* part_len, uint32_t* n_parts) {
+  if (!dev_ok(ctx, dev) || n == 0 || n > HKV_MAX_STD_INPUTS || !part_len || !n_parts) return HKV_E_ARG;
+  std::lock_guard<std::mutex> lock(ctx->mu);
+  const hkv::RecPlan p = hkv::plan_records(ctx->devs[(size_t)dev].geo, n);
+  *part_len = p.part_len, *n_parts = p.n_parts;
   return HKV_OK;
 }
 
diff --git a/haskoin-node_amd/csrc/hkv_internal.h b/haskoin-node_amd/csrc/hkv_internal.h
--- a/haskoin-node_amd/csrc/hkv_internal.h
+++ b/haskoin-node_amd/csrc/hkv_internal.h
@@ -80,6 +80,7 @@
 struct StdOps;
 hipError_t launch_prologue(const RecPlan& p, const RecOps& r, hipStream_t st);
 hipError_t launch_ecmult(const RecPlan& p, const RecOps& r, const StdOps* std_pro, hipStream_t st);
+hipError_t launch_table_chain(const RecPlan& p, const RecOps& r, uint32_t k, hipStream_t st);
 hipError_t launch_gtable(uint32_t* gtab, hipStream_t st);
 struct MsScan {
   uint32_t* desc;
@@ -130,7 +131,7 @@
 };
 hipError_t launch_std_verify_split(const StdPlan& p, const StdOps& o, const RecOps& r, const MsScan* ms,
                                    const uint32_t* tx_off, hipStream_t st);
-hipError_t launch_finish(const RecPlan& p, const RecOps& r, uint32_t* rare_ctr, const void* late_recs,
+hipError_t launch_finish(const RecPlan& p, const RecOps& r, RecChunk w, uint32_t* rare_ctr, const void* late_recs,
                          hipStream_t st);
 hipError_t launch_gen_pool(uint64_t seed, uint32_t npool, uint32_t* pool, hipStream_t st);
 hipError_t launch_gen_records(uint64_t seed, uint64_t index0, uint32_t n, const uint32_t* pool, uint32_t npool,
diff --git a/haskoin-node_amd/csrc/hkv_kernels.hip b/haskoin-node_amd/csrc/hkv_kernels.hip
--- a/haskoin-node_amd/csrc/hkv_kernels.hip
+++ b/haskoin-node_amd/csrc/hkv_kernels.hip
@@ -1551,7 +1551,7 @@
 
 template <bool ILP, bool LATE>
 HKV_DEV void finish_lane(uint32_t* __restrict__ im, uint32_t n, uint32_t n_pad, const uint32_t* __restrict__ gtab,
-                         uint32_t* __restrict__ rare_ctr, uint32_t i, uint32_t flags,
+                         uint32_t* __restrict__ rare_ctr, uint32_t i0, uint32_t cn, uint32_t i, uint32_t flags,
                          const uint32_t* __restrict__ recs) {
   if constexpr (LATE) {
     if (i < n) flags = late_u1_lane(recs, i, SoAView{im, n_pad}, flags);
@@ -1651,7 +1651,7 @@
     base = __shfl(base, lead);
     const uint32_t rank = __builtin_amdgcn_mbcnt_hi((uint32_t)(rmask >> 32),
                                                     __builtin_amdgcn_mbcnt_lo((uint32_t)rmask, 0u));
-    if (rare && base + rank < n_pad) SoAView{im, n_pad}.put(IM_RARE_LIST, (size_t)base + rank, i);
+    if (rare && base + rank < cn) SoAView{im, n_pad}.put(IM_RARE_LIST, (size_t)i0 + base + rank, i);
   }
   if (rare) {
     fo |= FLAG_RARE | (ainf ? FLAG_AINF : 0u);
@@ -1674,21 +1674,23 @@
 
 template <bool ILP, bool LATE>
 __global__ void __launch_bounds__(WG, ILP ? 2 : HKV_FINISH_WAVES) hkv_finish_kernel(uint32_t* __restrict__ im, uint32_t n,
-                                                                                 uint32_t n_pad,
+                                                                                 uint32_t n_pad, uint32_t i0,
+                                                                                 uint32_t cn,
                                                                                  const uint32_t* __restrict__ gtab,
                                                                                  uint32_t* __restrict__ rare_ctr,
                                                                                  const uint32_t* __restrict__ recs) {
-  const uint32_t i = blockIdx.x * WG + threadIdx.x;
-  if (i >= n_pad) return;
-  finish_lane<ILP, LATE>(im, n, n_pad, gtab, rare_ctr, i, SoAView{im, n_pad}.get(IM_FLAGS, i), recs);
-}
-
-__global__ void __launch_bounds__(WG) hkv_rare_kernel(uint32_t* __restrict__ im, uint32_t n_pad,
-                                                      const uint32_t* __restrict__ rare_ctr) {
+  const uint32_t s = blockIdx.x * WG + threadIdx.x;
+  if (s >= cn) return;
+  const uint32_t i = i0 + s;
+  finish_lane<ILP, LATE>(im, n, n_pad, gtab, rare_ctr, i0, cn, i, SoAView{im, n_pad}.get(IM_FLAGS, i), recs);
+}
+
+__global__ void __launch_bounds__(WG) hkv_rare_kernel(uint32_t* __restrict__ im, uint32_t n_pad, uint32_t i0,
+                                                      uint32_t cn, const uint32_t* __restrict__ rare_ctr) {
   const uint32_t k = blockIdx.x * WG + threadIdx.x;
-  if (k >= min(*rare_ctr, n_pad)) return;
+  if (k >= min(*rare_ctr, cn)) return;
   const SoAView iv = {im, n_pad};
-  const uint32_t i = iv.get(IM_RARE_LIST, k);
+  const uint32_t i = iv.get(IM_RARE_LIST, (size_t)i0 + k);
   const uint32_t flags = iv.get(IM_FLAGS, i);
   const bool rare = true;
   gej A, B;
@@ -1721,27 +1723,29 @@
   if (rare) iv.put(IM_FLAGS, i, flags | FLAG_DECIDED | (acc_ok ? FLAG_ACCEPT : 0u));
 }
 
-__global__ void __launch_bounds__(WG) hkv_yverdict_kernel(uint32_t* __restrict__ im, uint32_t n_pad, uint32_t stride,
-                                                          uint32_t* __restrict__ bits, uint32_t n_words,
-                                                          uint32_t* __restrict__ rare_ctr) {
+__global__ void __launch_bounds__(WG) hkv_yverdict_kernel(uint32_t* __restrict__ im, uint32_t n_pad, uint32_t i0,
+                                                          uint32_t cn, uint32_t stride, uint32_t* __restrict__ bits,
+                                                          uint32_t n_words, uint32_t* __restrict__ rare_ctr) {
   const uint32_t t = blockIdx.x * WG + threadIdx.x;
   if (t == 0) *rare_ctr = 0;
+  const uint32_t first = i0 + t;
   fe c;
   fe_set_u32(c, 1);
   int kn = 0;
   {
     fe d;
-    SoACView::ld8(im, n_pad, IM_DEN.off, t, d.v);
-    uint32_t fl = im[(size_t)IM_FLAGS.off * n_pad + t];
+    SoACView::ld8(im, n_pad, IM_DEN.off, first, d.v);
+    uint32_t fl = im[(size_t)IM_FLAGS.off * n_pad + first];
 #pragma unroll 1
     for (int k = 0; k < VERDICT_BATCH; ++k) {
-      const uint32_t i = t + (uint32_t)k * stride;
-      if (i >= n_pad) break;
+      const uint32_t s = t + (uint32_t)k * stride;
+      if (s >= cn) break;
+      const uint32_t i = i0 + s;
       kn = k + 1;
       const uint32_t inext = i + stride;
       fe dn;
       uint32_t fn = 0;
-      if (k + 1 < VERDICT_BATCH && inext < n_pad) {
+      if (k + 1 < VERDICT_BATCH && s + stride < cn) {
         SoACView::ld8(im, n_pad, IM_DEN.off, inext, dn.v);
         fn = im[(size_t)IM_FLAGS.off * n_pad + inext];
       }
@@ -1761,7 +1765,7 @@
     uint32_t r[8];
   };
   auto load_ops = [&](Ops& o, int k) {
-    const uint32_t i = t + (uint32_t)k * stride;
+    const uint32_t i = first + (uint32_t)k * stride;
     o.f = im[(size_t)IM_FLAGS.off * n_pad + i];
     if (k > 0) SoACView::ld8(im, n_pad, IM_C.off, i - stride, o.prev.v);
     SoACView::ld8(im, n_pad, IM_DEN.off, i, o.d.v);
@@ -1773,7 +1777,7 @@
   if (kn > 0) load_ops(cur, kn - 1);
 #pragma unroll 1
   for (int k = kn - 1; k >= 0; --k) {
-    const uint32_t i = t + (uint32_t)k * stride;
+    const uint32_t i = first + (uint32_t)k * stride;
     Ops nxt;
     if (k > 0) load_ops(nxt, k - 1);
     const uint32_t f = cur.f;
@@ -2453,20 +2457,17 @@
   hipLaunchKernelGGL(hkv_glv_kernel, dim3(ceil_div(p.n_pad, WG)), dim3(WG), 0, st, p.n_pad, r.im);
   return hipGetLastError();
 }
-static hipError_t launch_table_chain(const RecPlan& p, const RecOps& r, hipStream_t st) {
-  if (p.chunk_len < (uint32_t)WG || p.chunk_len % WG != 0) return hipErrorInvalidValue;
-  for (uint32_t k = 0; k < p.n_chunks; ++k) {
-    const uint32_t i0 = p.chunk(k).i0, cn = p.chunk(k).cn;
-    hipLaunchKernelGGL(hkv_qtable_kernel, dim3(cn / WG), dim3(WG), 0, st, (const uint32_t*)r.im, r.n, p.n_pad, i0, cn,
-                       r.qs);
-    hipError_t e = hipGetLastError();
-    if (e != hipSuccess) return e;
-    hipLaunchKernelGGL(hkv_chain_kernel, dim3(cn / WG), dim3(WG), 0, st, r.im, r.n, p.n_pad, i0, cn,
-                       (const uint32_t*)r.qs, i0 == 0 ? r.clk : nullptr);
-    e = hipGetLastError();
-    if (e != hipSuccess) return e;
-  }
-  return hipSuccess;
+hipError_t launch_table_chain(const RecPlan& p, const RecOps& r, uint32_t k, hipStream_t st) {
+  if (p.shape != Shape::TableChain || k >= p.n_parts) return hipErrorInvalidValue;
+  const uint32_t i0 = p.part(k).i0, cn = p.part(k).cn, slot = p.qs_slots == 2 ? RecPlan::part_slot(k) : 0u;
+  if (cn < (uint32_t)WG || cn % WG != 0) return hipErrorInvalidValue;
+  uint32_t* qs = r.qs + p.slot_quads(slot) * 4;
+  hipLaunchKernelGGL(hkv_qtable_kernel, dim3(cn / WG), dim3(WG), 0, st, (const uint32_t*)r.im, r.n, p.n_pad, i0, cn, qs);
+  const hipError_t e = hipGetLastError();
+  if (e != hipSuccess) return e;
+  hipLaunchKernelGGL(hkv_chain_kernel, dim3(cn / WG), dim3(WG), 0, st, r.im, r.n, p.n_pad, i0, cn, (const uint32_t*)qs,
+                     i0 == 0 ? r.clk : nullptr);
+  return hipGetLastError();
 }
 static StdArgs std_args(const StdOps& o) {
   return StdArgs{o.txs, o.n_tx, o.txt, o.scripts, o.scripts_len, o.jobs, o.forkid, nullptr, nullptr, nullptr, nullptr};
@@ -2489,7 +2490,6 @@
       hipLaunchKernelGGL((hkv_ecmult_kernel<true, false>), dim3(p.grid), dim3(WG), 0, st, r.im, r.n, p.n_pad, r.qs,
                          r.clk, StdArgs{});
       break;
-    case Shape::TableChain: return launch_table_chain(p, r, st);
     default: return hipErrorInvalidValue;
   }
   return hipGetLastError();
@@ -2533,27 +2533,30 @@
                      std_args(o));
   return hipGetLastError();
 }
-hipError_t launch_finish(const RecPlan& p, const RecOps& r, uint32_t* rare_ctr, const void* late_recs,
+hipError_t launch_finish(const RecPlan& p, const RecOps& r, RecChunk w, uint32_t* rare_ctr, const void* late_recs,
                          hipStream_t st) {
   if (p.shape != Shape::Mid && p.shape != Shape::TableChain) return hipErrorInvalidValue;
+  const uint32_t i0 = w.i0, cn = w.cn;
+  if (cn < (uint32_t)WG || cn % WG != 0 || i0 % WG != 0 || (uint64_t)i0 + cn > p.n_pad) return hipErrorInvalidValue;
   const bool paired = p.shape == Shape::Mid;
   const uint32_t* lr = static_cast<const uint32_t*>(late_recs);
-  const dim3 g(p.n_pad / WG), b(WG);
+  const dim3 g(cn / WG), b(WG);
   if (paired && lr)
-    hipLaunchKernelGGL((hkv_finish_kernel<true, true>), g, b, 0, st, r.im, r.n, p.n_pad, r.gtab, rare_ctr, lr);
+    hipLaunchKernelGGL((hkv_finish_kernel<true, true>), g, b, 0, st, r.im, r.n, p.n_pad, i0, cn, r.gtab, rare_ctr, lr);
   else if (paired)
-    hipLaunchKernelGGL((hkv_finish_kernel<true, false>), g, b, 0, st, r.im, r.n, p.n_pad, r.gtab, rare_ctr, lr);
+    hipLaunchKernelGGL((hkv_finish_kernel<true, false>), g, b, 0, st, r.im, r.n, p.n_pad, i0, cn, r.gtab, rare_ctr, lr);
   else if (lr)
-    hipLaunchKernelGGL((hkv_finish_kernel<false, true>), g, b, 0, st, r.im, r.n, p.n_pad, r.gtab, rare_ctr, lr);
+    hipLaunchKernelGGL((hkv_finish_kernel<false, true>), g, b, 0, st, r.im, r.n, p.n_pad, i0, cn, r.gtab, rare_ctr, lr);
   else
-    hipLaunchKernelGGL((hkv_finish_kernel<false, false>), g, b, 0, st, r.im, r.n, p.n_pad, r.gtab, rare_ctr, lr);
+    hipLaunchKernelGGL((hkv_finish_kernel<false, false>), g, b, 0, st, r.im, r.n, p.n_pad, i0, cn, r.gtab, rare_ctr, lr);
   hipError_t e = hipGetLastError();
   if (e != hipSuccess) return e;
-  hipLaunchKernelGGL(hkv_rare_kernel, dim3(p.n_pad / WG), dim3(WG), 0, st, r.im, p.n_pad, (const uint32_t*)rare_ctr);
+  hipLaunchKernelGGL(hkv_rare_kernel, g, b, 0, st, r.im, p.n_pad, i0, cn, (const uint32_t*)rare_ctr);
   e = hipGetLastError();
   if (e != hipSuccess) return e;
-  hipLaunchKernelGGL(hkv_yverdict_kernel, dim3(p.verdict_stride / WG), dim3(WG), 0, st, r.im, p.n_pad,
-                     p.verdict_stride, r.bits, r.n_words, rare_ctr);
+  const uint32_t stride = verdict_stride_of(cn);
+  hipLaunchKernelGGL(hkv_yverdict_kernel, dim3(stride / WG), b, 0, st, r.im, p.n_pad, i0, cn, stride, r.bits,
+                     r.n_words, rare_ctr);
   return hipGetLastError();
 }
 hipError_t launch_gen_pool(uint64_t seed, uint32_t npool, uint32_t* pool, hipStream_t st) {
diff --git a/haskoin-node_amd/csrc/hkv_launch_plan.h b/haskoin-node_amd/csrc/hkv_launch_plan.h
--- a/haskoin-node_amd/csrc/hkv_launch_plan.h
+++ b/haskoin-node_amd/csrc/hkv_launch_plan.h
@@ -11,7 +11,12 @@
   uint32_t grid_max = 0;
   size_t rec_chunk = 0;
   size_t std_chunk = 0;
+  size_t rec_part = 0;
 };
+
+constexpr size_t PART_ALIGN = (size_t)VERDICT_BATCH * 32 % WG == 0 ? (size_t)VERDICT_BATCH * 32
+                                                                   : (size_t)VERDICT_BATCH * 32 * WG;
+static_assert(PART_ALIGN % WG == 0 && PART_ALIGN % ((size_t)VERDICT_BATCH * 32) == 0, "part alignment");
 
 constexpr size_t SPLIT_DIV = 8;
 constexpr uint32_t MIN_INV_LANES = 65536;
@@ -41,6 +46,15 @@
     const uint64_t left = n_pad - i0;
     return RecChunk{(uint32_t)i0, (uint32_t)(left < chunk_len ? left : chunk_len)};
   }
+  uint32_t part_len, n_parts, qs_slots;
+  RecChunk part(uint32_t k) const {
+    const uint64_t i0 = (uint64_t)k * part_len;
+    const uint64_t left = n_pad - i0;
+    return RecChunk{(uint32_t)i0, (uint32_t)(left < part_len ? left : part_len)};
+  }
+  static constexpr uint32_t part_stream(uint32_t k) { return k & 1u; }
+  static constexpr uint32_t part_slot(uint32_t k) { return k & 1u; }
+  size_t slot_quads(uint32_t slot) const { return (size_t)slot * part_len * (QTAB_QUADS + QTAB_ZG_QUADS); }
 };
 
 namespace plan_detail {
@@ -51,6 +65,12 @@
   if (n_pad > grid_lanes(g) / SPLIT_DIV) return Shape::Mid;
   return n_pad <= (size_t)BLK_SIGS * g.n_cu ? Shape::Block : Shape::Pair;
 }
+}
+
+inline uint32_t verdict_stride_of(size_t cn) {
+  const size_t min_lanes = cn < MIN_INV_LANES ? cn : MIN_INV_LANES;
+  const size_t ver = plan_detail::round_up((cn + VERDICT_BATCH - 1) / VERDICT_BATCH, WG);
+  return (uint32_t)(ver < min_lanes ? min_lanes : ver);
 }
 
 inline RecPlan plan_records(const Geometry& g, size_t n) {
@@ -72,8 +92,7 @@
   const size_t min_lanes = n_pad < MIN_INV_LANES ? n_pad : MIN_INV_LANES;
   const size_t inv = (n_pad + BATCH_INV - 1) / BATCH_INV;
   p.inv_stride = (uint32_t)(inv > MIN_INV_LANES ? inv : min_lanes);
-  const size_t ver = round_up((n_pad + VERDICT_BATCH - 1) / VERDICT_BATCH, WG);
-  p.verdict_stride = (uint32_t)(ver < min_lanes ? min_lanes : ver);
+  p.verdict_stride = verdict_stride_of(n_pad);
   p.qs_quads = grid_lanes(g) * QTAB_QUADS;
   p.chunk_len = p.n_pad;
   p.n_chunks = 1;
@@ -83,6 +102,17 @@
     if (quads > p.qs_quads) p.qs_quads = quads;
     p.chunk_len = (uint32_t)chunk;
     p.n_chunks = (uint32_t)((n_pad + chunk - 1) / chunk);
+  }
+  p.part_len = p.chunk_len;
+  p.n_parts = p.n_chunks;
+  p.qs_slots = 1;
+  if (p.shape == Shape::TableChain && g.rec_part != 0) {
+    const size_t part = round_up(g.rec_part, PART_ALIGN);
+    if (part < n_pad && part <= p.chunk_len && 2 * part * (QTAB_QUADS + QTAB_ZG_QUADS) <= p.qs_quads) {
+      p.part_len = (uint32_t)part;
+      p.n_parts = (uint32_t)((n_pad + part - 1) / part);
+      p.qs_slots = 2;
+    }
   }
   return p;
 }
diff --git a/haskoin-node_amd/csrc/hkv_layout.h b/haskoin-node_amd/csrc/hkv_layout.h
--- a/haskoin-node_amd/csrc/hkv_layout.h
+++ b/haskoin-node_amd/csrc/hkv_layout.h
@@ -123,6 +123,9 @@
 #ifndef HKV_REC_CHUNK
 #define HKV_REC_CHUNK (1u << 20)
 #endif
+#ifndef HKV_REC_PART
+#define HKV_REC_PART (1u << 19)
+#endif
 constexpr int QTAB_ZG_QUADS = 2;
 
 constexpr int WG = 256;
diff --git a/haskoin-node_amd/hkv/lib.py b/haskoin-node_amd/hkv/lib.py
--- a/haskoin-node_amd/hkv/lib.py
+++ b/haskoin-node_amd/hkv/lib.py
@@ -77,6 +77,7 @@
     "hkv_debug_ms_scratch": (c_int, [c_void_p, c_int, POINTER(c_size_t)]),
     "hkv_debug_q_scratch": (c_int, [c_void_p, c_int, POINTER(c_size_t), POINTER(c_size_t)]),
     "hkv_debug_launch_shape": (c_int, [c_void_p, c_int, c_uint32, c_size_t, POINTER(c_uint32)]),
+    "hkv_debug_rec_parts": (c_int, [c_void_p, c_int, c_size_t, POINTER(c_uint32), POINTER(c_uint32)]),
     "hkv_debug_ms_tail_counts": (c_int, [c_void_p, c_int, POINTER(c_uint64)]),
     "hkv_batch_alloc": (c_int, [c_void_p, c_size_t, POINTER(c_void_p)]),
     "hkv_batch_free": (None, [c_void_p]),
@@ -158,7 +159,7 @@
     "hkv_version": (c_uint32, []),
 }
 
-MEASUREMENT_ONLY = {"hkv_profile_group_stamps", "hkv_debug_q_scratch", "hkv_debug_launch_shape"}
+MEASUREMENT_ONLY = {"hkv_profile_group_stamps", "hkv_debug_q_scratch", "hkv_debug_launch_shape", "hkv_debug_rec_parts"}
 
 _LIB = None
 
diff --git a/include/hkv.h b/include/hkv.h
--- a/include/hkv.h
+++ b/include/hkv.h
@@ -44,6 +44,7 @@
 int hkv_debug_ms_scratch(hkv_ctx* ctx, int dev, size_t* bytes);
 int hkv_debug_q_scratch(hkv_ctx* ctx, int dev, size_t* bytes, size_t* chunk);
 int hkv_debug_launch_shape(hkv_ctx* ctx, int dev, uint32_t kind, size_t n, uint32_t out[4]);
+int hkv_debug_rec_parts(hkv_ctx* ctx, int dev, size_t n, uint32_t* part_len, uint32_t* n_parts);
 int hkv_debug_ms_tail_counts(hkv_ctx* ctx, int dev, uint64_t out[3]);
 
 int hkv_batch_alloc(hkv_ctx* ctx, size_t max_n, hkv_batch** out);
```

Result: faster. 128.0 million, median of 6 (+2.6%).
